# anilkeshwani/speech-integration

Measured on AMD Instinct MI355X. Metric: train_tokens_per_sec, higher is better.
Workload: dtype bf16; 1 GPU; Llama-3.2-1B +5000 DSUs (V=133258), SFT step fwd+bwd+AdamW, seq_len=2048, batch=8/GPU, grad_accum=1, 16 layers, random-init weights, MLS-shaped synthetic DSU sequences; global_batch=8, seq_len=2048, parallelism=dp1

## Files before the change

### include/ssi_hip.h

```cpp
#ifndef SSI_HIP_H
#define SSI_HIP_H

#include <stdint.h>

#ifdef __cplusplus
extern "C" {
#endif

#define SSI_ABI_VERSION 9

enum { SSI_F32 = 0, SSI_BF16 = 1 };
enum { SSI_OK = 0, SSI_ERR_ARG = 1, SSI_ERR_UNSUPPORTED = 2, SSI_ERR_WORKSPACE = 3, SSI_ERR_HIP = 1000  };
enum { SSI_GEMM_NT = 0, SSI_GEMM_NN = 1, SSI_GEMM_TN = 2 };
enum { SSI_TILES_STATIC = 0, SSI_TILES_DYNAMIC = 1 };
int ssi_set_gemm_tile_order(int mode);

enum { SSI_IMPL_AUTO = 0, SSI_IMPL_GENERIC = 1, SSI_IMPL_MFMA = 2,
       SSI_IMPL_MFMA_WG8 = 3  };

int ssi_abi_version(void);
const char* ssi_last_error(void);
int ssi_set_impl(int impl);

int ssi_embed_fwd(const int64_t* tokens, const void* table, void* out, int64_t n_tok, int64_t dim, int64_t vocab,
                  int dtype, void* stream);
int64_t ssi_embed_bwd_workspace_bytes(int64_t vocab);
int ssi_embed_bwd(const int64_t* tokens, const void* dout, void* dtable, int64_t n_tok, int64_t dim, int64_t vocab,
                  int dtype, void* workspace, int64_t workspace_bytes, void* stream);

int ssi_rmsnorm_fwd(const void* x, const void* scale, void* y, float* rstd, int64_t rows, int64_t dim, float eps,
                    int dtype, void* stream);
int64_t ssi_rmsnorm_bwd_workspace_bytes(int64_t rows, int64_t dim);
int ssi_rmsnorm_bwd(const void* dy, const void* x, const void* scale, const float* rstd, const void* dres, void* dx,
                    void* dscale, int accumulate_dscale, int64_t rows, int64_t dim, int dtype, void* workspace,
                    int64_t workspace_bytes, void* stream);

int ssi_rope_inplace(void* x, int64_t ld, int64_t rows, int64_t seq_len, int n_heads_rot, int head_dim,
                     const float* table, int64_t table_len, const int32_t* positions, int inverse, int dtype,
                     void* stream);

int ssi_gemm_rope(int64_t M, int64_t N, int64_t K, const void* A, int64_t lda, const void* B, int64_t ldb, void* C, int64_t ldc,
                  int64_t seq_len, int n_heads_rot, int head_dim, const float* rope_table, int64_t table_len,
                  const int32_t* positions, int dtype, void* stream);

int ssi_attn_fwd(const void* qkv, int64_t ld, void* out, float* lse, int64_t batch, int64_t seq, int n_heads,
                 int n_kv, int head_dim, int dtype, void* stream);
int ssi_attn_bwd(const void* qkv, int64_t ld, const void* out, const void* dout, const float* lse, void* dqkv,
                 float* delta, int64_t batch, int64_t seq, int n_heads, int n_kv, int head_dim, int dtype,
                 void* stream);

int ssi_attn_varlen_fwd(const void* qkv, int64_t ld, void* out, float* lse, const int32_t* doc_start, const int32_t* doc_end,
                        int64_t batch, int64_t seq, int n_heads, int n_kv, int head_dim, int dtype, void* stream);
int ssi_attn_varlen_bwd(const void* qkv, int64_t ld, const void* out, const void* dout, const float* lse, void* dqkv,
                        float* delta, const int32_t* doc_start, const int32_t* doc_end, int64_t batch, int64_t seq,
                        int n_heads, int n_kv, int head_dim, int dtype, void* stream);

int ssi_doc_ranges(const int64_t* input_pos, int64_t batch, int64_t seq, int64_t max_pos, int32_t* positions, int32_t* doc_start,
                   int32_t* doc_end, int32_t* n_clamped, void* stream);

int ssi_attn_varlen_bwd_rope(const void* qkv, int64_t ld, const void* out, const void* dout, const float* lse, void* dqkv,
                             float* delta, const int32_t* doc_start, const int32_t* doc_end, const float* rope_table,
                             int64_t table_len, const int32_t* positions, int64_t batch, int64_t seq, int n_heads, int n_kv,
                             int head_dim, int dtype, void* stream);

int64_t ssi_attn_bwd_workspace_bytes(int64_t batch, int64_t seq, int n_heads, int n_kv, int head_dim, int dtype);
int ssi_attn_varlen_bwd_ws(const void* qkv, int64_t ld, const void* out, const void* dout, const float* lse, void* dqkv,
                           float* delta, const int32_t* doc_start, const int32_t* doc_end, const float* rope_table,
                           int64_t table_len, const int32_t* positions, int64_t batch, int64_t seq, int n_heads, int n_kv,
                           int head_dim, int dtype, void* workspace, int64_t workspace_bytes, void* stream);

enum { SSI_ATTN_KERNEL_DQ = 0, SSI_ATTN_KERNEL_DKV = 1 };
enum { SSI_ATTN_MODE_AUTO = 0, SSI_ATTN_MODE_OLD = 1, SSI_ATTN_MODE_NEW = 2, SSI_ATTN_MODE_NO_HEAD_SPLIT = 3 };
int ssi_set_attn_impl(int which, int mode);
enum { SSI_ATTN_USED_DQ2 = 1, SSI_ATTN_USED_DKV2 = 2, SSI_ATTN_USED_HEAD_SPLIT = 4, SSI_ATTN_USED_PLAN = 8 };
int ssi_attn_last_dispatch(void);

enum { SSI_ATTN_PLAN_HEADER = 16, SSI_ATTN_PLAN_FORCE = 1, SSI_ATTN_PLAN_SPLIT_ALL = 2  };
int64_t ssi_attn_plan_words(int64_t batch, int64_t seq, int64_t n_docs);
int64_t ssi_attn_plan_workspace_bytes(const int32_t* host_plan_header);
int64_t ssi_attn_plan_build(const int32_t* host_doc_row, const int32_t* host_doc_start, const int32_t* host_doc_end, int64_t n_docs,
                            int64_t batch, int64_t seq, int n_heads, int n_kv, int flags, int32_t* host_plan, int64_t plan_words);
int ssi_attn_varlen_bwd_plan(const void* qkv, int64_t ld, const void* out, const void* dout, const float* lse, void* dqkv,
                             float* delta, const int32_t* doc_start, const int32_t* doc_end, const float* rope_table,
                             int64_t table_len, const int32_t* positions, int64_t batch, int64_t seq, int n_heads, int n_kv,
                             int head_dim, int dtype, void* workspace, int64_t workspace_bytes, const int32_t* plan,
                             const int32_t* host_plan_header, void* stream);

int ssi_swiglu_fwd(const void* gu, void* act, int64_t rows, int64_t inter, int dtype, void* stream);
int ssi_swiglu_bwd(const void* dact, const void* gu, void* dgu, int64_t rows, int64_t inter, int dtype, void* stream);

int ssi_gemm(int layout, int64_t M, int64_t N, int64_t K, const void* A, int64_t lda, const void* B, int64_t ldb,
             void* C, int64_t ldc, const void* R, float alpha, const float* alpha_dev, int accumulate, int dtype,
             void* stream);

int64_t ssi_gemm_splitk_workspace_bytes(int64_t M, int64_t N, int splits);
int ssi_gemm_splitk(int layout, int64_t M, int64_t N, int64_t K, const void* A, int64_t lda, const void* B, int64_t ldb,
                    void* C, int64_t ldc, const void* R, float alpha, const float* alpha_dev, int accumulate, int dtype,
                    int splits, void* workspace, int64_t workspace_bytes, void* stream);

int ssi_gemm_batched(int layout, int batch, int64_t M, int64_t N, int64_t K, const void* A, int64_t lda, int64_t strideA, const void* B,
                     int64_t ldb, int64_t strideB, void* C, int64_t ldc, int64_t strideC, float alpha, const float* alpha_dev,
                     int accumulate, int dtype, void* stream);

int ssi_gemm_swiglu_fwd(int64_t M, int64_t inter, int64_t K, const void* X, int64_t ldx, const void* W13, int64_t ldw, void* GU,
                        int64_t ldgu, void* ACT, int64_t ldact, int dtype, void* stream);
int ssi_gemm_swiglu_bwd(int layout, int64_t M, int64_t inter, int64_t K, const void* DY, int64_t lddy, const void* W2, int64_t ldw,
                        const void* GU, int64_t ldgu, void* DGU, int64_t lddgu, void* dact_ws, int dtype, void* stream);

int ssi_transpose(const void* src, int64_t ld_src, void* dst, int64_t ld_dst, int64_t rows, int64_t cols, int dtype,
                  void* stream);

int ssi_ce_fwd(void* logits, int64_t ld, const int64_t* labels, int64_t rows, int64_t vocab, int64_t ignore_index,
               float* row_loss, float* row_lse, int write_grad, int dtype, void* stream);
int ssi_ce_reduce(const float* row_loss, const int64_t* labels, int64_t rows, int64_t vocab, int64_t ignore_index, float* out,
                  void* stream);
int ssi_ce_fwd_weighted(void* logits, int64_t ld, const int64_t* labels, const float* row_weight, int64_t rows, int64_t vocab,
                        int64_t ignore_index, float* row_loss, float* row_lse, int write_grad, int dtype, void* stream);

int ssi_lmhead_ce_fwd(const void* hidden, int64_t ldh, const void* table, int64_t ldt, const int64_t* labels, int64_t rows,
                      int64_t dim, int64_t vocab, int64_t vocab_pad, int64_t ignore_index, void* logits_ws, int64_t ldl,
                      float* row_loss, float* stats, int write_grad, int dtype, void* stream);
int ssi_lmhead_ce_bwd(const void* dlogits, int64_t ldl, const void* hidden, int64_t ldh, const void* table, int64_t ldt,
                      const float* alpha_dev, int64_t rows, int64_t dim, int64_t vocab_pad, void* d_hidden, int64_t lddh,
                      void* d_table, int64_t lddt, int accumulate_d_table, int dtype, void* stream);

int ssi_count_tokens(const int64_t* tokens, const int64_t* labels, int64_t n, const int64_t* ranges, int n_ranges,
                     int64_t pad_id, int64_t ignore_index, int64_t* out, void* stream);

int ssi_scale_inplace(void* x, int64_t n, float scale, const float* scale_dev, int dtype, void* stream);
int64_t ssi_sumsq_workspace_bytes(int64_t n);
int ssi_sumsq(const void* x, int64_t n, int dtype, float* out, void* workspace, int64_t workspace_bytes, void* stream);
int ssi_adamw_step(void* param, void* grad, void* exp_avg, void* exp_avg_sq, int64_t n, double lr, double beta1,
                   double beta2, double eps, double weight_decay, int64_t step, const float* grad_scale_dev, int zero_grad,
                   int dtype, void* stream);

#ifdef __cplusplus
}
#endif
#endif
```

### speech-integration_amd/csrc/common_hip.h

```cpp
#pragma once
#include <hip/hip_runtime.h>
#include <stdint.h>
#include <stdio.h>
#include "../../include/ssi_hip.h"

typedef __bf16 bf16_t;
typedef __attribute__((ext_vector_type(2))) float f32x2;
typedef __attribute__((ext_vector_type(4))) float f32x4;
typedef __attribute__((ext_vector_type(16))) float f32x16;
typedef __attribute__((ext_vector_type(4))) __bf16 bf16x4;
typedef __attribute__((ext_vector_type(8))) __bf16 bf16x8;
typedef __attribute__((ext_vector_type(4))) short s16x4;
typedef __attribute__((ext_vector_type(4))) unsigned int u32x4;
typedef __attribute__((ext_vector_type(2))) unsigned int u32x2;

#define SSI_WAVE 64

void ssi_set_error(const char* fmt, ...);

#define SSI_CHECK_ARG(cond)                                                                  \
    do {                                                                                     \
        if (!(cond)) {                                                                       \
            ssi_set_error("%s:%d: argument check failed: %s", __FILE__, __LINE__, #cond);    \
            return SSI_ERR_ARG;                                                              \
// ... 48 lines not shown
    f32x4 v;
    __device__ __forceinline__ float get(int i) const { return v[i]; }
    __device__ __forceinline__ void set(int i, float x) { v[i] = x; }
};
template <> struct Vec16<bf16_t> {
    static constexpr int N = 8;
    bf16x8 v;
    __device__ __forceinline__ float get(int i) const { return (float)v[i]; }
    __device__ __forceinline__ void set(int i, float x) { v[i] = (bf16_t)x; }
};
template <typename T> __device__ __forceinline__ Vec16<T> load16(const T* p) {
    Vec16<T> r;
    r.v = *reinterpret_cast<const decltype(r.v)*>(p);
    return r;
}
template <typename T> __device__ __forceinline__ void store16(T* p, const Vec16<T>& r) {
    *reinterpret_cast<decltype(r.v)*>(p) = r.v;
}

template <typename T> __device__ __forceinline__ Vec16<T> load16_nt(const T* p) {
    Vec16<T> r;
    r.v = __builtin_nontemporal_load(reinterpret_cast<const decltype(r.v)*>(p));
    return r;
}
template <typename T> __device__ __forceinline__ void store16_nt(T* p, const Vec16<T>& r) {
    __builtin_nontemporal_store(r.v, reinterpret_cast<decltype(r.v)*>(p));
}

__device__ __forceinline__ float wave_sum(float v) {
#pragma unroll
    for (int o = 32; o > 0; o >>= 1) v += __shfl_xor(v, o, 64);
    return v;
}
__device__ __forceinline__ float wave_max(float v) {
#pragma unroll
    for (int o = 32; o > 0; o >>= 1) v = fmaxf(v, __shfl_xor(v, o, 64));
    return v;
}
__device__ __forceinline__ float block_sum(float v, float* red) {
    v = wave_sum(v);
    const int w = threadIdx.x >> 6, l = threadIdx.x & 63, nw = (blockDim.x + 63) >> 6;
    __syncthreads();
    if (l == 0) red[w] = v;
    __syncthreads();
    float t = (l < nw) ? red[l] : 0.f;
    t = wave_sum(t);
    return t;
}
__device__ __forceinline__ float block_max(float v, float* red) {
    v = wave_max(v);
    const int w = threadIdx.x >> 6, l = threadIdx.x & 63, nw = (blockDim.x + 63) >> 6;
    __syncthreads();
    if (l == 0) red[w] = v;
    __syncthreads();
    float t = (l < nw) ? red[l] : -INFINITY;
    t = wave_max(t);
    return t;
}

template <bool ENABLED, int N, bool FENCED = false> struct PhaseStamps {
    unsigned long long begin = __builtin_readcyclecounter(), last = begin, total[N] = {};
    __device__ __forceinline__ void reset() {
        if (FENCED) __builtin_amdgcn_sched_barrier(0);
        last = __builtin_readcyclecounter();
        if (FENCED) __builtin_amdgcn_sched_barrier(0);
    }
    __device__ __forceinline__ void tick(int i) {
        const unsigned long long prev = last;
        reset();
        total[i] += last - prev;
    }
};
template <int N, bool FENCED> struct PhaseStamps<false, N, FENCED> {
    __device__ __forceinline__ void reset() {}
    __device__ __forceinline__ void tick(int) {}
};

int ssi_get_impl();

bool ssi_gemm_mfma_supported(int layout, int64_t M, int64_t N, int64_t K, const void* A, int64_t lda, const void* B,
                             int64_t ldb, const void* C, int64_t ldc, const void* R);
int ssi_gemm_mfma_bf16(int layout, int64_t M, int64_t N, int64_t K, const void* A, int64_t lda, const void* B,
                       int64_t ldb, void* C, int64_t ldc, const void* R, float alpha, const float* alpha_dev,
                       int accumulate, void* stream);
int ssi_gemm_mfma_bf16_splitk(int layout, int64_t M, int64_t N, int64_t K, const void* A, int64_t lda, const void* B,
                              int64_t ldb, void* C, int64_t ldc, const void* R, float alpha, const float* alpha_dev,
                              int accumulate, int splits, float* slabs, void* stream);
bool ssi_gemm_mfma_bf16_batched(int layout, int batch, int64_t M, int64_t N, int64_t K, const void* A, int64_t lda, int64_t bsA, const void* B,
                                int64_t ldb, int64_t bsB, void* C, int64_t ldc, int64_t bsC, float alpha, const float* alpha_dev, int accumulate,
                                void* stream, int* rc);
void ssi_gemm_mfma_set_dynamic_tiles(int on);
bool ssi_gemm_rope_mfma(int64_t M, int64_t N, int64_t K, const void* A, int64_t lda, const void* B, int64_t ldb, void* C, int64_t ldc,
                        const float* rope, const int32_t* positions, int64_t seq, int64_t rot_cols, void* stream, int* rc);
bool ssi_gemm_swiglu_supported(int64_t M, int64_t inter, int64_t K, const void* p0, const void* p1, const void* p2, const void* p3,
                               int64_t ld0, int64_t ld1, int64_t ld2, int64_t ld3);
int ssi_gemm_swiglu_fwd_mfma(int64_t M, int64_t inter, int64_t K, const void* X, int64_t ldx, const void* W13, int64_t ldw,
                             void* GU, int64_t ldgu, void* ACT, int64_t ldact, void* stream);
int ssi_gemm_swiglu_bwd_mfma(int layout, int64_t M, int64_t inter, int64_t K, const void* DY, int64_t lddy, const void* W2, int64_t ldw,
                             const void* GU, int64_t ldgu, void* DGU, int64_t lddgu, void* stream);
bool ssi_gemm_swiglu_bwd_nn_supported(int64_t K, int64_t lddy, int64_t ldw);

bool ssi_gemm_f32_mfma_supported(int layout, int64_t M, int64_t N, int64_t K, const void* A, int64_t lda, const void* B,
                                 int64_t ldb, const void* C, int64_t ldc, const void* R);
int ssi_gemm_f32_mfma(int layout, int64_t M, int64_t N, int64_t K, const void* A, int64_t lda, const void* B, int64_t ldb,
                      void* C, int64_t ldc, const void* R, float alpha, const float* alpha_dev, int accumulate,
                      void* stream);

bool ssi_attn_mfma_supported(int64_t ld, int64_t batch, int64_t seq, int n_heads, int n_kv, int head_dim, int dtype);
void ssi_attn_note_dispatch(int v);
int ssi_attn_bwd_mfma(const void* qkv, int64_t ld, const void* out, const void* dout, const float* lse, void* dqkv,
                      float* delta, const int32_t* doc_start, const int32_t* doc_end, const float* rope, int64_t table_len,
                      const int32_t* positions, int64_t batch, int64_t seq, int n_heads, int n_kv, void* workspace, int64_t workspace_bytes,
                      const int32_t* plan_dev, const int32_t* host_plan_header, void* stream);
int ssi_attn_fwd_mfma(const void* qkv, int64_t ld, void* out, float* lse, const int32_t* doc_start, int64_t batch, int64_t seq,
                      int n_heads, int n_kv, void* stream);
int64_t ssi_attn_mfma_bwd_workspace_bytes(int64_t batch, int64_t seq, int n_heads, int n_kv);

#define SSI_DISPATCH_DTYPE(dtype, ...)                           \
    do {                                                         \
        if ((dtype) == SSI_F32) {                                \
            using T = float;                                     \
            __VA_ARGS__;                                         \
        } else if ((dtype) == SSI_BF16) {                        \
            using T = bf16_t;                                    \
            __VA_ARGS__;                                         \
        } else {                                                 \
            ssi_set_error("unsupported dtype %d", (int)(dtype)); \
            return SSI_ERR_ARG;                                  \
        }                                                        \
    } while (0)
```

### speech-integration_amd/csrc/gemm_generic.hip

```cpp
#include "common_hip.h"
#include <atomic>

static std::atomic<int> g_impl{SSI_IMPL_AUTO};
extern "C" int ssi_set_impl(int impl) {
    if (impl >= SSI_IMPL_AUTO && impl <= SSI_IMPL_MFMA_WG8) return g_impl.exchange(impl, std::memory_order_relaxed);
    return g_impl.load(std::memory_order_relaxed);
}
int ssi_get_impl() { return g_impl.load(std::memory_order_relaxed); }

extern "C" int ssi_set_gemm_tile_order(int mode) {
    if (mode != SSI_TILES_STATIC && mode != SSI_TILES_DYNAMIC) { ssi_set_error("ssi_set_gemm_tile_order: mode %d", mode); return SSI_ERR_ARG; }
    ssi_gemm_mfma_set_dynamic_tiles(mode == SSI_TILES_DYNAMIC);
    return SSI_OK;
}

template <typename T>
__global__ __launch_bounds__(256) void gemm_generic_kernel(int64_t M, int64_t N, int64_t K, const T* __restrict__ A,
                                                           int64_t sam, int64_t sak, const T* __restrict__ B, int64_t sbk,
                                                           int64_t sbn, T* __restrict__ C, int64_t ldc,
                                                           const T* __restrict__ R, float alpha,
                                                           const float* __restrict__ alpha_dev, int accumulate) {
    constexpr int BM = 64, BN = 64, BK = 16;
    __shared__ float As[BK][BM + 4];
    __shared__ float Bs[BK][BN + 4];
    const int tid = threadIdx.x;
    const int tx = tid & 15, ty = tid >> 4;
    const int64_t m0 = (int64_t)blockIdx.y * BM, n0 = (int64_t)blockIdx.x * BN;
    float acc[4][4];
#pragma unroll
    for (int i = 0; i < 4; ++i)
#pragma unroll
        for (int j = 0; j < 4; ++j) acc[i][j] = 0.f;

    const bool a_k_contig = (sak == 1);
    const bool b_n_contig = (sbn == 1);
    for (int64_t k0 = 0; k0 < K; k0 += BK) {
#pragma unroll
        for (int it = 0; it < 4; ++it) {
            const int e = tid + it * 256;
            int mm, kk;
            if (a_k_contig) { kk = e & 15; mm = e >> 4; } else { mm = e & 63; kk = e >> 6; }
            const int64_t gm = m0 + mm, gk = k0 + kk;
            As[kk][mm] = (gm < M && gk < K) ? to_f32<T>(A[gm * sam + gk * sak]) : 0.f;
            int nn, kb;
            if (b_n_contig) { nn = e & 63; kb = e >> 6; } else { kb = e & 15; nn = e >> 4; }
            const int64_t gn = n0 + nn, gkb = k0 + kb;
            Bs[kb][nn] = (gn < N && gkb < K) ? to_f32<T>(B[gkb * sbk + gn * sbn]) : 0.f;
        }
        __syncthreads();
#pragma unroll
        for (int kk = 0; kk < BK; ++kk) {
            float a[4], b[4];
#pragma unroll
            for (int i = 0; i < 4; ++i) a[i] = As[kk][ty * 4 + i];
#pragma unroll
            for (int j = 0; j < 4; ++j) b[j] = Bs[kk][tx * 4 + j];
#pragma unroll
            for (int i = 0; i < 4; ++i)
#pragma unroll
                for (int j = 0; j < 4; ++j) acc[i][j] = fmaf(a[i], b[j], acc[i][j]);
        }
        __syncthreads();
    }
    const float al = alpha * (alpha_dev ? *alpha_dev : 1.f);
#pragma unroll
    for (int i = 0; i < 4; ++i) {
        const int64_t gm = m0 + ty * 4 + i;
        if (gm >= M) continue;
#pragma unroll
        for (int j = 0; j < 4; ++j) {
            const int64_t gn = n0 + tx * 4 + j;
            if (gn >= N) continue;
            float v = al * acc[i][j];
            if (accumulate) v += to_f32<T>(C[gm * ldc + gn]);
            if (R) v += to_f32<T>(R[gm * ldc + gn]);
            C[gm * ldc + gn] = from_f32<T>(v);
        }
    }
}

extern "C" int ssi_gemm(int layout, int64_t M, int64_t N, int64_t K, const void* A, int64_t lda, const void* B,
                        int64_t ldb, void* C, int64_t ldc, const void* R, float alpha, const float* alpha_dev,
                        int accumulate, int dtype, void* stream) {
    SSI_CHECK_ARG(A && B && C && M >= 0 && N >= 0 && K >= 0 && ldc >= N);
    SSI_CHECK_ARG(layout == SSI_GEMM_NT || layout == SSI_GEMM_NN || layout == SSI_GEMM_TN);
    if (M == 0 || N == 0) return SSI_OK;
    int64_t sam, sak, sbk, sbn;
    if (layout == SSI_GEMM_NT)      { SSI_CHECK_ARG(lda >= K && ldb >= K); sam = lda; sak = 1;   sbk = 1;   sbn = ldb; }
    else if (layout == SSI_GEMM_NN) { SSI_CHECK_ARG(lda >= K && ldb >= N); sam = lda; sak = 1;   sbk = ldb; sbn = 1; }
    else                            { SSI_CHECK_ARG(lda >= M && ldb >= N); sam = 1;   sak = lda; sbk = ldb; sbn = 1; }

    const bool f32_ok = dtype == SSI_F32 && ssi_gemm_f32_mfma_supported(layout, M, N, K, A, lda, B, ldb, C, ldc, R);
    const bool mfma_ok = f32_ok || (dtype == SSI_BF16 && ssi_gemm_mfma_supported(layout, M, N, K, A, lda, B, ldb, C, ldc, R));
    if ((g_impl == SSI_IMPL_MFMA || g_impl == SSI_IMPL_MFMA_WG8) && !mfma_ok) {
        ssi_set_error("ssi_gemm: MFMA path forced but shape/dtype unsupported (M=%lld N=%lld K=%lld dtype=%d)",
                      (long long)M, (long long)N, (long long)K, dtype);
        return SSI_ERR_UNSUPPORTED;
    }
    if (f32_ok && g_impl != SSI_IMPL_GENERIC)
        return ssi_gemm_f32_mfma(layout, M, N, K, A, lda, B, ldb, C, ldc, R, alpha, alpha_dev, accumulate, stream);
    if (mfma_ok && g_impl != SSI_IMPL_GENERIC)
        return ssi_gemm_mfma_bf16(layout, M, N, K, A, lda, B, ldb, C, ldc, R, alpha, alpha_dev, accumulate, stream);

    SSI_CHECK_ARG(ssi_cdiv(M, 64) <= 65535);
    dim3 grid((unsigned)ssi_cdiv(N, 64), (unsigned)ssi_cdiv(M, 64));
    SSI_DISPATCH_DTYPE(dtype, hipLaunchKernelGGL(gemm_generic_kernel<T>, grid, dim3(256), 0, (hipStream_t)stream, M, N, K,
                                                 (const T*)A, sam, sak, (const T*)B, sbk, sbn, (T*)C, ldc, (const T*)R,
                                                 alpha, alpha_dev, accumulate));
    SSI_LAUNCH_CHECK();
    return SSI_OK;
}

extern "C" int ssi_gemm_batched(int layout, int batch, int64_t M, int64_t N, int64_t K, const void* A, int64_t lda, int64_t strideA,
                                const void* B, int64_t ldb, int64_t strideB, void* C, int64_t ldc, int64_t strideC, float alpha,
                                const float* alpha_dev, int accumulate, int dtype, void* stream) {
    SSI_CHECK_ARG(batch >= 0 && strideA >= 0 && strideB >= 0 && strideC >= 0);
    SSI_CHECK_ARG(dtype == SSI_BF16 || dtype == SSI_F32);
    if (batch == 0) return SSI_OK;
    SSI_CHECK_ARG(A && B && C);
    const int64_t es = dtype == SSI_BF16 ? 2 : 4;
    auto off = [&](const void* p, int64_t b, int64_t stride) { return (const void*)((const char*)p + b * stride * es); };
    bool mfma_ok = dtype == SSI_BF16 && batch > 1 && g_impl != SSI_IMPL_GENERIC && g_impl != SSI_IMPL_MFMA_WG8;
    for (int b = 0; b < batch && mfma_ok; ++b)
        mfma_ok = ssi_gemm_mfma_supported(layout, M, N, K, off(A, b, strideA), lda, off(B, b, strideB), ldb, off(C, b, strideC), ldc, nullptr);
    if (mfma_ok) {
        SSI_CHECK_ARG(layout == SSI_GEMM_NT || layout == SSI_GEMM_NN || layout == SSI_GEMM_TN);
        int rc = SSI_OK;
        if (ssi_gemm_mfma_bf16_batched(layout, batch, M, N, K, A, lda, strideA, B, ldb, strideB, C, ldc, strideC, alpha, alpha_dev, accumulate,
                                       stream, &rc))
            return rc;
    }
    for (int b = 0; b < batch; ++b)
        if (int rc = ssi_gemm(layout, M, N, K, off(A, b, strideA), lda, off(B, b, strideB), ldb, (void*)off(C, b, strideC), ldc, nullptr, alpha,
                              alpha_dev, accumulate, dtype, stream))
            return rc;
    return SSI_OK;
}

extern "C" int64_t ssi_gemm_splitk_workspace_bytes(int64_t M, int64_t N, int splits) {
    return splits <= 1 ? 0 : (int64_t)splits * M * N * (int64_t)sizeof(float);
}

extern "C" int ssi_gemm_splitk(int layout, int64_t M, int64_t N, int64_t K, const void* A, int64_t lda, const void* B,
                               int64_t ldb, void* C, int64_t ldc, const void* R, float alpha, const float* alpha_dev,
                               int accumulate, int dtype, int splits, void* workspace, int64_t workspace_bytes, void* stream) {
    const bool mfma_ok = dtype == SSI_BF16 && ssi_gemm_mfma_supported(layout, M, N, K, A, lda, B, ldb, C, ldc, R);
    if (splits <= 1 || !mfma_ok || g_impl == SSI_IMPL_GENERIC || K / 64 < splits)
        return ssi_gemm(layout, M, N, K, A, lda, B, ldb, C, ldc, R, alpha, alpha_dev, accumulate, dtype, stream);
    SSI_CHECK_ARG(layout == SSI_GEMM_NT || layout == SSI_GEMM_NN || layout == SSI_GEMM_TN);
    SSI_CHECK_ARG(splits <= 64 && ((uintptr_t)workspace % 16) == 0);
    if (!workspace || workspace_bytes < ssi_gemm_splitk_workspace_bytes(M, N, splits)) { ssi_set_error("ssi_gemm_splitk: workspace too small"); return SSI_ERR_WORKSPACE; }
    return ssi_gemm_mfma_bf16_splitk(layout, M, N, K, A, lda, B, ldb, C, ldc, R, alpha, alpha_dev, accumulate, splits,
                                     (float*)workspace, stream);
}

extern "C" int ssi_gemm_rope(int64_t M, int64_t N, int64_t K, const void* A, int64_t lda, const void* B, int64_t ldb, void* C, int64_t ldc,
                             int64_t seq_len, int n_heads_rot, int head_dim, const float* rope_table, int64_t table_len,
                             const int32_t* positions, int dtype, void* stream) {
    SSI_CHECK_ARG(A && B && C && rope_table && M >= 0 && N > 0 && K > 0 && seq_len > 0 && n_heads_rot > 0 && head_dim > 0);
    SSI_CHECK_ARG((int64_t)n_heads_rot * head_dim <= N && (positions != nullptr || table_len >= seq_len));
    if (M == 0) return SSI_OK;
    int rc = SSI_OK;
    if (dtype == SSI_BF16 && head_dim == 64 && g_impl != SSI_IMPL_GENERIC &&
        ssi_gemm_rope_mfma(M, N, K, A, lda, B, ldb, C, ldc, rope_table, positions, seq_len, (int64_t)n_heads_rot * head_dim, stream, &rc))
        return rc;
    if ((rc = ssi_gemm(SSI_GEMM_NT, M, N, K, A, lda, B, ldb, C, ldc, nullptr, 1.f, nullptr, 0, dtype, stream))) return rc;
    return ssi_rope_inplace(C, ldc, M, seq_len, n_heads_rot, head_dim, rope_table, table_len, positions, 0, dtype, stream);
}

extern "C" int ssi_gemm_swiglu_fwd(int64_t M, int64_t inter, int64_t K, const void* X, int64_t ldx, const void* W13, int64_t ldw,
                                   void* GU, int64_t ldgu, void* ACT, int64_t ldact, int dtype, void* stream) {
    SSI_CHECK_ARG(X && W13 && GU && ACT && M >= 0 && inter > 0 && K > 0 && ldgu >= 2 * inter && ldact >= inter);
    if (dtype == SSI_BF16 && g_impl != SSI_IMPL_GENERIC && ssi_gemm_swiglu_supported(M, inter, K, X, W13, GU, ACT, ldx, ldw, ldgu, ldact))
        return ssi_gemm_swiglu_fwd_mfma(M, inter, K, X, ldx, W13, ldw, GU, ldgu, ACT, ldact, stream);
    if (int rc = ssi_gemm(SSI_GEMM_NT, M, 2 * inter, K, X, ldx, W13, ldw, GU, ldgu, nullptr, 1.f, nullptr, 0, dtype, stream)) return rc;
    SSI_CHECK_ARG(ldgu == 2 * inter && ldact == inter);
    return ssi_swiglu_fwd(GU, ACT, M, inter, dtype, stream);
}

extern "C" int ssi_gemm_swiglu_bwd(int layout, int64_t M, int64_t inter, int64_t K, const void* DY, int64_t lddy, const void* W2,
                                   int64_t ldw, const void* GU, int64_t ldgu, void* DGU, int64_t lddgu, void* dact_ws, int dtype,
                                   void* stream) {
    SSI_CHECK_ARG(DY && W2 && GU && DGU && M >= 0 && inter > 0 && K > 0 && ldgu >= 2 * inter && lddgu >= 2 * inter);
    SSI_CHECK_ARG(layout == SSI_GEMM_NT || layout == SSI_GEMM_NN);
    if (dtype == SSI_BF16 && g_impl != SSI_IMPL_GENERIC && ssi_gemm_swiglu_supported(M, inter, K, DY, W2, GU, DGU, lddy, ldw, ldgu, lddgu) &&
        (layout == SSI_GEMM_NT || ssi_gemm_swiglu_bwd_nn_supported(K, lddy, ldw)))
        return ssi_gemm_swiglu_bwd_mfma(layout, M, inter, K, DY, lddy, W2, ldw, GU, ldgu, DGU, lddgu, stream);
    SSI_CHECK_ARG(dact_ws != nullptr && ldgu == 2 * inter && lddgu == 2 * inter);
    if (int rc = ssi_gemm(layout, M, inter, K, DY, lddy, W2, ldw, dact_ws, inter, nullptr, 1.f, nullptr, 0, dtype, stream)) return rc;
    return ssi_swiglu_bwd(dact_ws, GU, DGU, M, inter, dtype, stream);
}
```

### speech-integration_amd/csrc/gemm_mfma.hip

```cpp
#include "common_hip.h"
#include <atomic>
#include <type_traits>

namespace {

constexpr int BM = 256, BN = 256, BK = 64;
constexpr int NTHREADS = 512;
constexpr int WAVES_N = 4;
constexpr int WM = 128, WN = 64;
constexpr int MT = WM / 16, NT = WN / 16;
constexpr int TILE_BYTES = BM * BK * 2;
constexpr int PIPE_BYTES = 2 * 2 * TILE_BYTES;
constexpr int EPI_ROW_BYTES = WN * 2 + 16;
constexpr int EPI_WAVE_BYTES = WM * EPI_ROW_BYTES;
constexpr int LDS_BYTES = 8 * EPI_WAVE_BYTES > PIPE_BYTES ? 8 * EPI_WAVE_BYTES : PIPE_BYTES;

typedef __attribute__((address_space(3))) void lds_void;
typedef __attribute__((address_space(1))) const void gbl_void;

__device__ __forceinline__ int col_swz(int krow) { return ((krow & 3) | (((krow >> 3) & 1) << 2)) << 1; }

__device__ __forceinline__ void stage_col_load(const bf16_t* __restrict__ g, int64_t ld, int64_t r0, int64_t k0, int tid,
                                               u32x4 (&regs)[4]) {
#pragma unroll
    for (int p = 0; p < 4; ++p) {
        const int krow = p * 16 + (tid >> 5);
        const int chunk = (tid & 31) ^ col_swz(krow);
        regs[p] = *reinterpret_cast<const u32x4*>(g + (k0 + krow) * ld + r0 + chunk * 8);
    }
}
__device__ __forceinline__ void stage_col_write(char* lds_tile, int tid, const u32x4 (&regs)[4]) {
#pragma unroll
    for (int p = 0; p < 4; ++p) *reinterpret_cast<u32x4*>(lds_tile + p * 8192 + tid * 16) = regs[p];
}

template <bool COL>
__device__ __forceinline__ void stage_tile(const bf16_t* __restrict__ g, int64_t ld, int64_t r0, int64_t k0, char* lds_tile,
                                           int tid, int64_t split_rows = 0) {
#pragma unroll
    for (int p = 0; p < 4; ++p) {
        const bf16_t* src;
        if (!COL) {
            const int row = p * 64 + (tid >> 3);
            const int chunk = (tid & 7) ^ ((row >> 1) & 7);
            const int64_t grow = split_rows ? (row < 128 ? (r0 >> 1) + row : split_rows + (r0 >> 1) + row - 128) : r0 + row;
            src = g + grow * ld + k0 + chunk * 8;
        } else {
            const int krow = p * 16 + (tid >> 5);
            const int chunk = (tid & 31) ^ col_swz(krow);
            src = g + (k0 + krow) * ld + r0 + chunk * 8;
        }
        const int wave_base = __builtin_amdgcn_readfirstlane(p * 8192 + (tid >> 6) * 1024);
        __builtin_amdgcn_global_load_lds((gbl_void*)src, (lds_void*)(lds_tile + wave_base), 16, 0, 0);
    }
}

template <bool COL>
__device__ __forceinline__ bf16x8 read_frag(const char* lds_tile, int outer_base, int kh, int lane) {
    if (!COL) {
        const int row = outer_base + (lane & 15);
        const int chunk = (kh * 4 + (lane >> 4)) ^ ((row >> 1) & 7);
        return *reinterpret_cast<const bf16x8*>(lds_tile + row * 128 + chunk * 16);
    } else {
        const int i = lane & 15, q = i >> 2, p = i & 3;
        const int kbase = kh * 32 + 8 * (lane >> 4);
        const int chunk = (outer_base >> 3) + (p >> 1);
        const int k0 = kbase + q, k1 = kbase + 4 + q;
        const char* a0 = lds_tile + k0 * 512 + ((chunk ^ col_swz(k0)) * 16) + 8 * (p & 1);
        const char* a1 = lds_tile + k1 * 512 + ((chunk ^ col_swz(k1)) * 16) + 8 * (p & 1);
        s16x4 lo = __builtin_amdgcn_ds_read_tr16_b64_v4i16((__attribute__((address_space(3))) s16x4*)a0);
        s16x4 hi = __builtin_amdgcn_ds_read_tr16_b64_v4i16((__attribute__((address_space(3))) s16x4*)a1);
        typedef __attribute__((ext_vector_type(8))) short s16x8;
        s16x8 r = __builtin_shufflevector(lo, hi, 0, 1, 2, 3, 4, 5, 6, 7);
        return __builtin_bit_cast(bf16x8, r);
    }
}

__device__ __forceinline__ void tile_coords(int bid, int tiles_m, int tiles_n, int& tm, int& tn) {
    const int nwg = tiles_m * tiles_n;
    const int xcd = bid & 7, q = nwg >> 3, r = nwg & 7;
    const int t = (xcd < r ? xcd * (q + 1) : r * (q + 1) + (xcd - r) * q) + (bid >> 3);
    constexpr int GM = 4;
    const int per_group = GM * tiles_n;
    const int group = t / per_group, in_group = t % per_group;
    const int gm = (tiles_m - group * GM) < GM ? (tiles_m - group * GM) : GM;
    tm = group * GM + in_group % gm;
    tn = in_group / gm;
}

__device__ __forceinline__ void tile_from_t(int t, int tiles_m, int tiles_n, int& tm, int& tn) {
    constexpr int GM = 4;
    const int per_group = GM * tiles_n;
    const int group = t / per_group, in_group = t % per_group;
    const int gm = (tiles_m - group * GM) < GM ? (tiles_m - group * GM) : GM;
    tm = group * GM + in_group % gm;
    tn = in_group / gm;
}

__device__ int g_nt4_sched[16][16];

enum { EPI_PLAIN = 0, EPI_SWIGLU_FWD = 1, EPI_SWIGLU_BWD = 2, EPI_ROPE = 3 };
struct EpiArgs {
    bf16_t* out2;
    int64_t ld_out2;
    const bf16_t* in2;
    int64_t ld_in2;
    int64_t inter;
    const float* rope = nullptr;
    const int32_t* pos = nullptr;
    int64_t seq = 1;
    int64_t rot_cols = 0;
    int batch = 1;
    int64_t bsA = 0, bsB = 0, bsC = 0;
};

template <bool A_COL, bool B_COL, bool SPLITK, int EPI = EPI_PLAIN>
__global__ __launch_bounds__(NTHREADS, 2) void gemm_mfma_kernel(int tiles_m, int tiles_n, int64_t K,
                                                               const bf16_t* __restrict__ A, int64_t lda,
                                                               const bf16_t* __restrict__ B, int64_t ldb,
                                                               bf16_t* __restrict__ C, int64_t ldc,
                                                               const bf16_t* __restrict__ R, float alpha,
                                                               const float* __restrict__ alpha_dev, int accumulate,
                                                               float* __restrict__ slabs, EpiArgs ea) {
    extern __shared__ __attribute__((aligned(16))) char smem[];
    const int tid = threadIdx.x, lane = tid & 63;
    const int wave = __builtin_amdgcn_readfirstlane(tid >> 6);
    const int wm = wave / WAVES_N, wn = wave % WAVES_N;
    int tm, tn;
    tile_coords(blockIdx.x, tiles_m, tiles_n, tm, tn);
    const int64_t m0 = (int64_t)tm * BM, n0 = (int64_t)tn * BN;

    f32x4 acc[NT][MT];
#pragma unroll
    for (int i = 0; i < NT; ++i)
#pragma unroll
        for (int j = 0; j < MT; ++j) acc[i][j] = f32x4{0.f, 0.f, 0.f, 0.f};

    const int nk_total = (int)(K / BK);
    const int kt_begin = SPLITK ? (int)((int64_t)blockIdx.y * nk_total / gridDim.y) : 0;
    const int kt_end = SPLITK ? (int)((int64_t)(blockIdx.y + 1) * nk_total / gridDim.y) : nk_total;
    const int nk = kt_end - kt_begin;
    const int64_t kofs = (int64_t)kt_begin * BK;
    auto tileA = [&](int buf) { return smem + buf * 2 * TILE_BYTES; };
    auto tileB = [&](int buf) { return smem + buf * 2 * TILE_BYTES + TILE_BYTES; };
    auto stage = [&](int kt, int buf) {
        stage_tile<A_COL>(A, lda, m0, kofs + (int64_t)kt * BK, tileA(buf), tid);
        stage_tile<B_COL>(B, ldb, n0, kofs + (int64_t)kt * BK, tileB(buf), tid, EPI == EPI_SWIGLU_FWD ? ea.inter : 0);
    };
    if constexpr (A_COL && B_COL) {
        u32x4 ra[4], rb[4];
        stage_col_load(A, lda, m0, kofs, tid, ra);
        stage_col_load(B, ldb, n0, kofs, tid, rb);
        stage_col_write(tileA(0), tid, ra);
        stage_col_write(tileB(0), tid, rb);
        for (int kt = 0; kt < nk; ++kt) {
            const int cur = kt & 1;
            __syncthreads();
            if (kt + 1 < nk) {
                stage_col_load(A, lda, m0, kofs + (int64_t)(kt + 1) * BK, tid, ra);
                stage_col_load(B, ldb, n0, kofs + (int64_t)(kt + 1) * BK, tid, rb);
            }
            const char* la = tileA(cur);
            const char* lb = tileB(cur);
#pragma unroll
            for (int kh = 0; kh < 2; ++kh) {
                bf16x8 bfr[NT], afr[MT];
#pragma unroll
                for (int j = 0; j < NT; ++j) bfr[j] = read_frag<true>(lb, wn * WN + j * 16, kh, lane);
#pragma unroll
                for (int i = 0; i < MT; ++i) afr[i] = read_frag<true>(la, wm * WM + i * 16, kh, lane);
                __builtin_amdgcn_s_setprio(1);
#pragma unroll
                for (int i = 0; i < MT; ++i)
#pragma unroll
                    for (int j = 0; j < NT; ++j)
                        acc[j][i] = __builtin_amdgcn_mfma_f32_16x16x32_bf16(bfr[j], afr[i], acc[j][i], 0, 0, 0);
                __builtin_amdgcn_s_setprio(0);
            }
            if (kt + 1 < nk) {
// ... 180 lines not shown
#pragma unroll
    for (int e = 0; e < 8; ++e) f[e] = 0.f;
    for (int s = 0; s < splits; ++s) {
        const float* p = slabs + (int64_t)s * M * N + row * N + col;
        const f32x4 a = *reinterpret_cast<const f32x4*>(p), b = *reinterpret_cast<const f32x4*>(p + 4);
#pragma unroll
        for (int e = 0; e < 4; ++e) { f[e] += a[e]; f[4 + e] += b[e]; }
    }
    bf16x8 o;
#pragma unroll
    for (int e = 0; e < 8; ++e) o[e] = (bf16_t)(f[e] * al);
    const int64_t off = row * ldc + col;
    if (accumulate || R) {
#pragma unroll
        for (int e = 0; e < 8; ++e) f[e] = (float)o[e];
        if (accumulate) {
            const bf16x8 c = *reinterpret_cast<const bf16x8*>(C + off);
#pragma unroll
            for (int e = 0; e < 8; ++e) f[e] += (float)c[e];
        }
        if (R) {
            const bf16x8 c = *reinterpret_cast<const bf16x8*>(R + off);
#pragma unroll
            for (int e = 0; e < 8; ++e) f[e] += (float)c[e];
        }
#pragma unroll
        for (int e = 0; e < 8; ++e) o[e] = (bf16_t)f[e];
    }
    *reinterpret_cast<bf16x8*>(C + off) = o;
}

template <bool A_COL, bool B_COL, bool SPLITK, int EPI = EPI_PLAIN>
int launch(int tiles_m, int tiles_n, int64_t K, const void* A, int64_t lda, const void* B, int64_t ldb, void* C,
           int64_t ldc, const void* R, float alpha, const float* alpha_dev, int accumulate, hipStream_t st,
           int splits = 1, float* slabs = nullptr, EpiArgs ea = EpiArgs{nullptr, 0, nullptr, 0, 0}) {
    auto kern = gemm_mfma_kernel<A_COL, B_COL, SPLITK, EPI>;
    static const hipError_t attr_rc = hipFuncSetAttribute((const void*)kern, hipFuncAttributeMaxDynamicSharedMemorySize, LDS_BYTES);
    if (attr_rc != hipSuccess) { ssi_set_error("gemm_mfma: cannot reserve %d B of LDS: %s", LDS_BYTES, hipGetErrorString(attr_rc)); return SSI_ERR_HIP + (int)attr_rc; }
    hipLaunchKernelGGL(kern, dim3((unsigned)(tiles_m * tiles_n), (unsigned)splits), dim3(NTHREADS), LDS_BYTES, st, tiles_m,
                       tiles_n, K, (const bf16_t*)A, lda, (const bf16_t*)B, ldb, (bf16_t*)C, ldc, (const bf16_t*)R, alpha,
                       alpha_dev, accumulate, slabs, ea);
    SSI_LAUNCH_CHECK();
    if (SPLITK) {
        const int64_t M = (int64_t)tiles_m * BM, N = (int64_t)tiles_n * BN;
        hipLaunchKernelGGL(splitk_reduce_kernel, dim3((unsigned)ssi_cdiv(M * N / 8, 256)), dim3(256), 0, st, slabs, splits, M, N,
                           (bf16_t*)C, ldc, (const bf16_t*)R, alpha, alpha_dev, accumulate);
        SSI_LAUNCH_CHECK();
    }
    return SSI_OK;
}

#ifndef NT4_ST_AUX
#define NT4_ST_AUX 0
#endif
#ifndef NT4_ST_AUX_BIG
#define NT4_ST_AUX_BIG 2
#endif
#ifndef NT4_RS
#define NT4_RS 2
#define NT4_BAR 40
#define NT4_A0 44
#define NT4_SA 6
#define NT4_NA 4
#endif
constexpr int NT4_THREADS = 256;
constexpr int NT4_LDS_BYTES = PIPE_BYTES + 16;
std::atomic<int> g_nt4_dynamic{0};
inline unsigned nt4_next_slot() {
    static std::atomic<unsigned> n{0};
    return n.fetch_add(1, std::memory_order_relaxed);
}
constexpr int NT4_WM = 128, NT4_WN = 128;
constexpr unsigned BUF_RSRC_DW3 = 0x00020000u;

__device__ __forceinline__ __amdgpu_buffer_rsrc_t make_rsrc(const void* p) {
    return __builtin_amdgcn_make_buffer_rsrc(const_cast<void*>(p), 0, 0x7fffffff, BUF_RSRC_DW3);
}

template <bool A_COL, bool B_COL, int EPI, int PREV, bool SPLITK, bool BATCHED>
__device__ __forceinline__ void nt4_body(char* smem, int tiles_m, int tiles_n, int64_t K, const bf16_t* __restrict__ A,
                                         int64_t lda, const bf16_t* __restrict__ B, int64_t ldb,
                                         bf16_t* __restrict__ C, int64_t ldc, const bf16_t* __restrict__ R,
                                         float alpha, const float* __restrict__ alpha_dev, EpiArgs ea, int slot,
                                         int splits, float* __restrict__ slabs) {
    const int tid = threadIdx.x, lane = tid & 63;
    const int wave = __builtin_amdgcn_readfirstlane(tid >> 6);
    const int wm = wave >> 1, wn = wave & 1;
    const int per_prob = tiles_m * tiles_n;
    const int ntiles_out = BATCHED ? per_prob * ea.batch : per_prob;
    const int ntiles = SPLITK ? ntiles_out * splits : ntiles_out;
    auto locate = [&](int t, int& tm, int& tn) {
        int tt = SPLITK ? t % ntiles_out : t, pb = 0;
        if constexpr (BATCHED) { pb = tt / per_prob; tt -= pb * per_prob; }
        tile_from_t(tt, tiles_m, tiles_n, tm, tn);
        return pb;
    };
    const int G = (int)gridDim.x;
    const int nk_total = (int)(K / BK);
    auto k_lo = [&](int t) { return SPLITK ? (int)(((int64_t)nk_total * (t / ntiles_out) / splits) & ~1LL) : 0; };
    auto k_hi = [&](int t) { return SPLITK ? ((t / ntiles_out) + 1 == splits ? nk_total : (int)(((int64_t)nk_total * (t / ntiles_out + 1) / splits) & ~1LL)) : nk_total; };

    int* sched = g_nt4_sched[slot < 0 ? 0 : slot];
    volatile int* lds_next = reinterpret_cast<volatile int*>(smem + PIPE_BYTES);
    const int xcd = (int)blockIdx.x & 7, span_q = ntiles >> 3, span_r = ntiles & 7;
    auto span_len = [&](int x) { return span_q + (x < span_r ? 1 : 0); };
    auto span_lo = [&](int x) { return x < span_r ? x * (span_q + 1) : span_r * (span_q + 1) + (x - span_r) * span_q; };
    auto span_wgs = [&](int x) { return (G - x + 7) >> 3; };
    auto span_fixed = [&](int x) { const int n = 2 * span_wgs(x); return n < span_len(x) ? n : span_len(x); };
    const bool dynamic = slot >= 0;
    int my_idx = (int)blockIdx.x >> 3;
    int pending = 0;
    auto request_tile = [&]() {
        if (dynamic && tid == 0) pending = atomicAdd(&sched[xcd], 1);
    };
    auto receive_tile = [&]() -> int {
        if (!dynamic) {
            my_idx += G >> 3;
            return ((G & 7) == 0 && my_idx < span_len(xcd)) ? span_lo(xcd) + my_idx : -1;
        }
        asm volatile("s_waitcnt lgkmcnt(0)\n\ts_barrier" ::: "memory");
        if (tid == 0) {
            int t = -1;
            const int i = pending + span_fixed(xcd);
            if (i < span_len(xcd)) t = span_lo(xcd) + i;
            if (t < 0) {
                int seen[8];
#pragma unroll
                for (int x = 0; x < 8; ++x) seen[x] = __hip_atomic_load(&sched[x], __ATOMIC_RELAXED, __HIP_MEMORY_SCOPE_AGENT);
                for (int k = 1; k < 8 && t < 0; ++k) {
                    const int x = (xcd + k) & 7;
                    if (seen[x] + span_fixed(x) >= span_len(x)) continue;
                    const int j = atomicAdd(&sched[x], 1) + span_fixed(x);
                    if (j < span_len(x)) t = span_lo(x) + j;
                }
            }
            *lds_next = t;
        }
        asm volatile("s_waitcnt lgkmcnt(0)\n\ts_barrier" ::: "memory");
        return __builtin_amdgcn_readfirstlane(*lds_next);
    };
    int cur = ((int)blockIdx.x >> 3) < span_len(xcd) ? span_lo(xcd) + ((int)blockIdx.x >> 3) : -1;
    int nxt = -1;
    if (dynamic) {
        const int second = ((int)blockIdx.x >> 3) + span_wgs(xcd);
        nxt = (cur >= 0 && second < span_len(xcd)) ? span_lo(xcd) + second : -1;
    }

    f32x4 acc[8][8];
    auto tileA = [&](int buf) { return smem + buf * TILE_BYTES; };
    auto tileB = [&](int buf) { return smem + 2 * TILE_BYTES + buf * TILE_BYTES; };

    int lkt = 0, lnk = nk_total;
    const bf16_t* baseA = A;
    const bf16_t* baseB = B;
    const int64_t kstepA_ = A_COL ? BK * lda : BK, kstepB_ = B_COL ? BK * ldb : BK;
    auto set_load_tile = [&](int t) {
        int tm, tn;
        const int pb = locate(t, tm, tn);
        const bf16_t* Ap = BATCHED ? A + pb * ea.bsA : A;
        const bf16_t* Bp = BATCHED ? B + pb * ea.bsB : B;
        baseA = (A_COL ? Ap + (int64_t)tm * BM : Ap + (int64_t)tm * BM * lda) + k_lo(t) * kstepA_;
        baseB = (B_COL ? Bp + (int64_t)tn * BN : Bp + (int64_t)tn * (EPI == EPI_SWIGLU_FWD ? BN / 2 : BN) * ldb) + k_lo(t) * kstepB_;
        lnk = k_hi(t) - k_lo(t);
    };
    auto advance = [&]() {
        if (++lkt == lnk) {
            lkt = 0;
            if (nxt >= 0) set_load_tile(nxt);
        }
    };
    auto lane_off = [&](bool col, int64_t ld, int odd) {
        if (col) return (int)(((tid >> 5) * ld + (((tid & 31) ^ col_swz(odd * 8 + (tid >> 5))) * 8)) * 2);
        return (int)(((tid >> 3) * ld + (tid & 7) * 8) * 2);
    };
    const int offA0 = lane_off(A_COL, lda, 0), offA1 = A_COL ? lane_off(true, lda, 1) : offA0;
    const int offB0 = lane_off(B_COL, ldb, 0), offB1 = B_COL ? lane_off(true, ldb, 1) : offB0;
    const int64_t kstepA = kstepA_, kstepB = kstepB_;
    auto pieceA = [&](int p) { return A_COL ? (int)(p * 8 * lda * 2) : (int)(p * 32 * lda * 2); };
    auto pieceB = [&](int p) {
        if (B_COL) return (int)(p * 8 * ldb * 2);
        if (EPI == EPI_SWIGLU_FWD) {
            const int blk64 = p >> 1;
            return (int)((((blk64 & 1) ? ea.inter : 0) + (blk64 >> 1) * 64 + (p & 1) * 32) * ldb * 2);
        }
        return (int)(p * 32 * ldb * 2);
    };
    int trA = 0, trB = 0;
    if (A_COL || B_COL) {
        const int i16 = lane & 15, q = i16 >> 2, pp = i16 & 3, k0l = 8 * (lane >> 4) + q;
        const int common = k0l * 512 + (pp >> 1) * 16 + 8 * (pp & 1) + (col_swz(k0l) << 4);
        trA = common + wm * 256;
        trB = common + wn * 256;
    }
    auto rd_tr = [&](const char* tile, int base, int t8, int kh) {
        typedef __attribute__((address_space(3))) s16x4 lds_s16x4;
        const char* a0 = tile + (base ^ (t8 << 5)) + kh * 16384;
        const s16x4 lo = __builtin_amdgcn_ds_read_tr16_b64_v4i16((lds_s16x4*)a0);
        const s16x4 hi = __builtin_amdgcn_ds_read_tr16_b64_v4i16((lds_s16x4*)(a0 + 2048));
        typedef __attribute__((ext_vector_type(8))) short s16x8;
        const s16x8 r = __builtin_shufflevector(lo, hi, 0, 1, 2, 3, 4, 5, 6, 7);
        return __builtin_bit_cast(bf16x8, r);
    };
    using F_ = std::false_type;
    bf16x8 F0A[8], F0B[8], F1A[8], F1B[8];
    const int dofA = (int)(((tid >> 3) * lda + (((tid & 7) ^ ((tid >> 4) & 7)) * 8)) * 2);
    const int dofB = (int)(((tid >> 3) * ldb + (((tid & 7) ^ ((tid >> 4) & 7)) * 8)) * 2);
    typedef __attribute__((address_space(3))) char lds_c;
    const unsigned lds_wave = __builtin_amdgcn_readfirstlane((unsigned)(uintptr_t)(lds_c*)smem + (unsigned)wave * 1024u);
    auto rsrc_words = [&](const bf16_t* base) {
        const uint64_t a = (uint64_t)(uintptr_t)base;
        u32x4 r;
        r[0] = __builtin_amdgcn_readfirstlane((unsigned)a);
        r[1] = __builtin_amdgcn_readfirstlane((unsigned)(a >> 32) & 0xffffu);
        r[2] = 0x7fffffffu;
        r[3] = BUF_RSRC_DW3;
        return r;
    };
    auto dma_m0 = [&](int buf, int d) {
        const unsigned dst = lds_wave + (unsigned)((d < 8 ? buf * TILE_BYTES : 2 * TILE_BYTES + buf * TILE_BYTES) + (d & 7) * 4096);
        asm volatile("s_mov_b32 m0, %0" ::"s"(dst) : "memory");
    };
    u32x4 rsA, rsB;
    auto dma_src = [&]() { rsA = rsrc_words(baseA + lkt * kstepA); rsB = rsrc_words(baseB + lkt * kstepB); };
    auto dma_go = [&](int d) {
        if (d < 8) asm volatile("buffer_load_dwordx4 %0, %1, %2 offen lds" ::"v"(A_COL ? ((d & 1) ? offA1 : offA0) : dofA), "s"(rsA), "s"(pieceA(d)) : "memory");
        else asm volatile("buffer_load_dwordx4 %0, %1, %2 offen lds" ::"v"(B_COL ? ((d & 1) ? offB1 : offB0) : dofB), "s"(rsB), "s"(pieceB(d - 8)) : "memory");
    };
    auto dma = [&](int buf, int d) {
        dma_m0(buf, d);
        asm volatile("s_nop 1" ::: "memory");
        dma_go(d);
    };
    auto fragA = [&](const char* t, int i, int kh) {
        if constexpr (A_COL) return rd_tr(t, trA, i, kh);
        else return read_frag<false>(t, wm * NT4_WM + i * 16, kh, lane);
    };
    auto fragB = [&](const char* t, int j, int kh) {
        if constexpr (B_COL) return rd_tr(t, trB, j, kh);
        else return read_frag<false>(t, wn * NT4_WN + j * 16, kh, lane);
    };
    auto phase = [&](const bf16x8 (&fa)[8], const bf16x8 (&fb)[8], auto zero_c, auto extra) {
#pragma unroll
        for (int m = 0; m < 64; ++m) {
            const int i = m >> 3, j = m & 7;
            if (decltype(zero_c)::value)
                asm volatile("v_mfma_f32_16x16x32_bf16 %0, %1, %2, 0" : "=a"(acc[j][i]) : "v"(fb[j]), "v"(fa[i]));
            else
                asm volatile("v_mfma_f32_16x16x32_bf16 %0, %1, %2, %0" : "+a"(acc[j][i]) : "v"(fb[j]), "v"(fa[i]));
            extra(m);
            __builtin_amdgcn_sched_barrier(0);
        }
    };
    auto dma_body = [&](auto cur_c, auto first) {
        constexpr int cur = decltype(cur_c)::value;
        if (A_COL) asm volatile("" : "+v"(trA));
        if (B_COL) asm volatile("" : "+v"(trB));
        const char* la = tileA(cur);
        const char* lb = tileB(cur);
        const char* na = tileA(cur ^ 1);
        const char* nb = tileB(cur ^ 1);
        constexpr int RS = NT4_RS, BAR = NT4_BAR, A0 = NT4_A0, SA = NT4_SA, NA = NT4_NA;
        static_assert(15 * RS + 4 <= BAR && BAR + 2 <= A0 - 1 && A0 + (NA - 1) * SA <= 63 && 3 + 5 * (15 - NA) <= 58, "DMA schedule");
        phase(F0A, F0B, first, [&](int m) {
            if (m < 16 * RS && m % RS == 0) {
                const int r = m / RS;
                if (r < 8) F1B[r] = fragB(lb, r, 1); else F1A[r - 8] = fragA(la, r - 8, 1);
            }
            if (m == BAR) {
                asm volatile("s_waitcnt lgkmcnt(0)\n\ts_barrier" ::: "memory");
                dma_src();
            }
            if (m >= A0 - 1 && m < A0 - 1 + NA * SA && (m - (A0 - 1)) % SA == 0) dma_m0(cur, (m - (A0 - 1)) / SA);
            if (m >= A0 && m < A0 + NA * SA && (m - A0) % SA == 0) dma_go((m - A0) / SA);
        });
        advance();
        phase(F1A, F1B, F_{}, [&](int m) {
            if (m >= 2 && m < 2 + 5 * (16 - NA) && (m - 2) % 5 == 0) dma_m0(cur, NA + (m - 2) / 5);
            if (m >= 3 && m < 3 + 5 * (16 - NA) && (m - 3) % 5 == 0) dma_go(NA + (m - 3) / 5);
            if (m == 11) {
                if constexpr (NA == 4) asm volatile("s_waitcnt vmcnt(6)\n\ts_barrier" ::: "memory");
                else if constexpr (NA == 6) asm volatile("s_waitcnt vmcnt(8)\n\ts_barrier" ::: "memory");
                else if constexpr (NA == 7) asm volatile("s_waitcnt vmcnt(9)\n\ts_barrier" ::: "memory");
                else asm volatile("s_waitcnt vmcnt(0)\n\ts_barrier" ::: "memory");
            }
            if (m >= 12 && m <= 50 && !(m & 1) && m % 10 != 8) {
                const int r = (m - 12) / 2 - (m - 8) / 10;
                if (r < 8) F0B[r] = fragB(nb, r, 0); else F0A[r - 8] = fragA(na, r - 8, 0);
            }
        });
    };
    set_load_tile(cur >= 0 ? cur : 0);
    if (nk_total == 0) return;
    dma_src();
#pragma unroll
    for (int d = 0; d < 16; ++d) dma(0, d);
    advance();
    dma_src();
#pragma unroll
    for (int d = 0; d < 16; ++d) dma(1, d);
    advance();
    asm volatile("s_waitcnt vmcnt(16)\n\ts_barrier" ::: "memory");
#pragma unroll
    for (int r = 0; r < 8; ++r) F0B[r] = fragB(tileB(0), r, 0);
#pragma unroll
    for (int r = 0; r < 8; ++r) F0A[r] = fragA(tileA(0), r, 0);
    if (cur >= 0 && !dynamic) nxt = receive_tile();
    const float al = alpha * (alpha_dev ? *alpha_dev : 1.f);
    const int g = lane >> 4;
    while (cur >= 0) {
        int tm, tn;
        const int pb = locate(cur, tm, tn);
        const int nk = k_hi(cur) - k_lo(cur);
        using B0_ = std::integral_constant<int, 0>;
        using B1_ = std::integral_constant<int, 1>;
        if (nxt >= 0) request_tile();
        dma_body(B0_{}, std::true_type{});
        dma_body(B1_{}, F_{});
        for (int kt = 2; kt < nk; kt += 2) {
            dma_body(B0_{}, F_{});
            dma_body(B1_{}, F_{});
        }
        asm volatile("s_nop 15\n\ts_nop 15" ::: "memory");
        auto pair = [&](int i, int ja, int jb, auto scale_c) {
            bf16x4 x, y;
#pragma unroll
            for (int r = 0; r < 4; ++r) {
                float fx, fy;
                asm volatile("v_accvgpr_read_b32 %0, %1" : "=v"(fx) : "a"(acc[ja][i][r]));
                asm volatile("v_accvgpr_read_b32 %0, %1" : "=v"(fy) : "a"(acc[jb][i][r]));
                x[r] = (bf16_t)(decltype(scale_c)::value ? fx * al : fx);
                y[r] = (bf16_t)(decltype(scale_c)::value ? fy * al : fy);
            }
            const u32x2 xu = __builtin_bit_cast(u32x2, x), yu = __builtin_bit_cast(u32x2, y);
            const auto s0 = __builtin_amdgcn_permlane16_swap(xu[0], yu[0], false, false);
            const auto s1 = __builtin_amdgcn_permlane16_swap(xu[1], yu[1], false, false);
            u32x4 o;
            o[0] = s0[0]; o[1] = s1[0]; o[2] = s0[1]; o[3] = s1[1];
            return o;
        };
        auto duo = [&](int i, int j0, auto scale_c, u32x4& lo, u32x4& hi) {
            const u32x4 oa = pair(i, j0, j0 + 1, scale_c), ob = pair(i, j0 + 2, j0 + 3, scale_c);
#pragma unroll
            for (int d = 0; d < 4; ++d) {
                lo[d] = (unsigned)__builtin_amdgcn_update_dpp((int)oa[d], (int)ob[d], 0x118 , 0xF, 0xC, false);
                hi[d] = (unsigned)__builtin_amdgcn_update_dpp((int)ob[d], (int)oa[d], 0x108 , 0xF, 0x3, false);
            }
        };
        if constexpr (SPLITK) {
            const __amdgpu_buffer_rsrc_t rsS = make_rsrc(slabs + ((int64_t)cur * 4 + wave) * (64 * 64 * 4));
#pragma unroll
            for (int i = 0; i < 8; ++i)
#pragma unroll
                for (int j = 0; j < 8; ++j) {
                    u32x4 v;
#pragma unroll
                    for (int r = 0; r < 4; ++r) {
                        float f;
                        asm volatile("v_accvgpr_read_b32 %0, %1" : "=v"(f) : "a"(acc[j][i][r]));
                        v[r] = __builtin_bit_cast(unsigned, f);
                    }
                    __builtin_amdgcn_raw_buffer_store_b128(v, rsS, lane * 16, (i * 8 + j) * 1024, 0);
                    __builtin_amdgcn_sched_barrier(0);
                }
        } else {
        const int64_t row0 = (int64_t)tm * BM + wm * NT4_WM;
        const int lane_row = lane & 7, lane_col = ((lane >> 3) & 1) * 32 + (g & 1) * 16 + (g >> 1) * 8;
        auto epilogue = [&](auto scale_c) {
        if constexpr (EPI == EPI_PLAIN) {
            const int64_t tile_off = (BATCHED ? pb * ea.bsC : 0) + row0 * ldc + (int64_t)tn * BN + wn * NT4_WN;
            const __amdgpu_buffer_rsrc_t rsC = make_rsrc(C + tile_off);
            const __amdgpu_buffer_rsrc_t rsP = make_rsrc(PREV == 2 ? R + tile_off : C + tile_off);
            const int voff = (int)((lane_row * ldc + lane_col) * 2);
            auto soff = [&](int i, int h, int jd) { return (int)(((i * 16 + h * 8) * ldc + jd * 64) * 2); };
            u32x4 pv[2][4];
            auto ldprev = [&](int i) {
#pragma unroll
                for (int q = 0; q < 4; ++q) pv[i & 1][q] = __builtin_amdgcn_raw_buffer_load_b128(rsP, voff, soff(i, q & 1, q >> 1), 0);
            };
            auto add_prev = [&](u32x4& o, const u32x4& p) {
                bf16x8 ob = __builtin_bit_cast(bf16x8, o);
                const bf16x8 c = __builtin_bit_cast(bf16x8, p);
#pragma unroll
                for (int e = 0; e < 8; ++e) ob[e] = (bf16_t)((float)ob[e] + (float)c[e]);
                o = __builtin_bit_cast(u32x4, ob);
            };
            if (PREV) ldprev(0);
#pragma unroll
            for (int i = 0; i < 8; ++i) {
                if (PREV && i + 1 < 8) ldprev(i + 1);
#pragma unroll
                for (int jd = 0; jd < 2; ++jd) {
                    u32x4 lo, hi;
                    duo(i, jd * 4, scale_c, lo, hi);
                    if (PREV) { add_prev(lo, pv[i & 1][jd * 2]); add_prev(hi, pv[i & 1][jd * 2 + 1]); }
                    __builtin_amdgcn_raw_buffer_store_b128(lo, rsC, voff, soff(i, 0, jd), NT4_ST_AUX);
                    __builtin_amdgcn_raw_buffer_store_b128(hi, rsC, voff, soff(i, 1, jd), NT4_ST_AUX);
                    __builtin_amdgcn_sched_barrier(0);
                }
            }
        } else if constexpr (EPI == EPI_ROPE) {
            const int64_t tile_off = row0 * ldc + (int64_t)tn * BN + wn * NT4_WN;
            const __amdgpu_buffer_rsrc_t rsC = make_rsrc(C + tile_off);
            const int voff = (int)((lane_row * ldc + lane_col) * 2);
            auto soff = [&](int i, int hh, int jd) { return (int)(((i * 16 + hh * 8) * ldc + jd * 64) * 2); };
            const bool rot = (int64_t)tn * BN < ea.rot_cols;
            int prow[8][2];
            f32x4 cs[2][2][2];
            if (rot) {
#pragma unroll
                for (int i = 0; i < 8; ++i)
#pragma unroll
                    for (int hh = 0; hh < 2; ++hh) {
                        const int64_t r = row0 + i * 16 + hh * 8 + lane_row;
                        prow[i][hh] = ea.pos ? ea.pos[r] : (int)(r % ea.seq);
                    }
            }
            auto ldcs = [&](int i) {
#pragma unroll
                for (int hh = 0; hh < 2; ++hh) {
                    const float* tb = ea.rope + (int64_t)prow[i][hh] * 64 + (lane_col & 63);
                    cs[i & 1][hh][0] = *reinterpret_cast<const f32x4*>(tb);
                    cs[i & 1][hh][1] = *reinterpret_cast<const f32x4*>(tb + 4);
                }
            };
            auto rotate = [&](u32x4& o, const f32x4& c01, const f32x4& c23) {
                bf16x8 v = __builtin_bit_cast(bf16x8, o);
#pragma unroll
                for (int p = 0; p < 4; ++p) {
                    const f32x4& c = p < 2 ? c01 : c23;
                    float o0, o1;
                    ssi_rope_pair((float)v[2 * p], (float)v[2 * p + 1], c[(p & 1) * 2], c[(p & 1) * 2 + 1], o0, o1);
                    v[2 * p] = (bf16_t)o0;
                    v[2 * p + 1] = (bf16_t)o1;
                }
                o = __builtin_bit_cast(u32x4, v);
            };
            if (rot) ldcs(0);
#pragma unroll
            for (int i = 0; i < 8; ++i) {
                if (rot && i + 1 < 8) ldcs(i + 1);
#pragma unroll
                for (int jd = 0; jd < 2; ++jd) {
                    u32x4 lo, hi;
                    duo(i, jd * 4, scale_c, lo, hi);
                    if (rot) { rotate(lo, cs[i & 1][0][0], cs[i & 1][0][1]); rotate(hi, cs[i & 1][1][0], cs[i & 1][1][1]); }
                    __builtin_amdgcn_raw_buffer_store_b128(lo, rsC, voff, soff(i, 0, jd), NT4_ST_AUX);
                    __builtin_amdgcn_raw_buffer_store_b128(hi, rsC, voff, soff(i, 1, jd), NT4_ST_AUX);
// ... 18 lines not shown
            };
#pragma unroll
            for (int i = 0; i < 8; ++i) {
                u32x4 glo, ghi, ulo, uhi;
                duo(i, 0, scale_c, glo, ghi);
                duo(i, 4, scale_c, ulo, uhi);
#pragma unroll
                for (int h = 0; h < 2; ++h) {
                    const u32x4& gq = h ? ghi : glo;
                    const u32x4& uq = h ? uhi : ulo;
                    const int so = (int)(((i * 16 + h * 8) * ldc) * 2), so2 = (int)(((i * 16 + h * 8) * ea.ld_out2) * 2);
                    __builtin_amdgcn_raw_buffer_store_b128(gq, rsGU, voff, so, NT4_ST_AUX_BIG);
                    __builtin_amdgcn_raw_buffer_store_b128(uq, rsGU, voff, so + up_off, NT4_ST_AUX_BIG);
                    __builtin_amdgcn_raw_buffer_store_b128(act_of(gq, uq), rsACT, voff2, so2, NT4_ST_AUX_BIG);
                }
                __builtin_amdgcn_sched_barrier(0);
            }
        } else {
            const int64_t c0 = (int64_t)tn * BN + wn * NT4_WN;
            const __amdgpu_buffer_rsrc_t rsGU = make_rsrc(ea.in2 + row0 * ea.ld_in2 + c0);
            const __amdgpu_buffer_rsrc_t rsDGU = make_rsrc(ea.out2 + row0 * ea.ld_out2 + c0);
            const int voff = (int)((lane_row * ea.ld_in2 + lane_col) * 2), voff2 = (int)((lane_row * ea.ld_out2 + lane_col) * 2);
            const int up_off = (int)(ea.inter * 2);
            u32x4 pg[2][2], pu[2][2];
            auto ldprev = [&](int u) {
#pragma unroll
                for (int h = 0; h < 2; ++h) {
                    const int so = (int)((((u >> 1) * 16 + h * 8) * ea.ld_in2 + (u & 1) * 64) * 2);
                    pg[u & 1][h] = __builtin_amdgcn_raw_buffer_load_b128(rsGU, voff, so, 0);
                    pu[u & 1][h] = __builtin_amdgcn_raw_buffer_load_b128(rsGU, voff, so + up_off, 0);
                }
            };
            auto grads = [&](const u32x4& dq, const u32x4& gq, const u32x4& uq, u32x4& og_out, u32x4& ou_out) {
                const bf16x8 dv = __builtin_bit_cast(bf16x8, dq), gv = __builtin_bit_cast(bf16x8, gq), uv = __builtin_bit_cast(bf16x8, uq);
                bf16x8 og, ou;
#pragma unroll
                for (int e = 0; e < 8; ++e) {
                    float dg, du;
                    ssi_swiglu_bwd_elem<bf16_t>((float)gv[e], (float)uv[e], (float)dv[e], dg, du);
                    ou[e] = (bf16_t)du;
                    og[e] = (bf16_t)dg;
                }
                og_out = __builtin_bit_cast(u32x4, og);
                ou_out = __builtin_bit_cast(u32x4, ou);
            };
            ldprev(0);
#pragma unroll
            for (int u = 0; u < 16; ++u) {
                if (u + 1 < 16) ldprev(u + 1);
                const int i = u >> 1, jd = u & 1;
                u32x4 lo, hi;
                duo(i, jd * 4, scale_c, lo, hi);
#pragma unroll
                for (int h = 0; h < 2; ++h) {
                    u32x4 og, ou;
                    grads(h ? hi : lo, pg[u & 1][h], pu[u & 1][h], og, ou);
                    const int so2 = (int)(((i * 16 + h * 8) * ea.ld_out2 + jd * 64) * 2);
                    __builtin_amdgcn_raw_buffer_store_b128(og, rsDGU, voff2, so2, NT4_ST_AUX);
                    __builtin_amdgcn_raw_buffer_store_b128(ou, rsDGU, voff2, so2 + up_off, NT4_ST_AUX);
                }
                __builtin_amdgcn_sched_barrier(0);
            }
        }
        };
        if (al == 1.f) epilogue(std::false_type{});
        else epilogue(std::true_type{});
        }
        cur = nxt;
        if (cur >= 0) nxt = receive_tile();
    }
    asm volatile("s_waitcnt vmcnt(0)" ::: "memory");
    if (dynamic && tid == 0 && atomicAdd(&sched[8], 1) == G - 1) {
        volatile int* vs = sched;
#pragma unroll
        for (int i = 0; i < 9; ++i) vs[i] = 0;
    }
}

template <bool A_COL, bool B_COL, int EPI, int PREV, bool SPLITK = false, bool BATCHED = false>
__global__ __launch_bounds__(NT4_THREADS, 1) void gemm_nt4dma_kernel(int tiles_m, int tiles_n, int64_t K, const bf16_t* __restrict__ A,
                                                                     int64_t lda, const bf16_t* __restrict__ B, int64_t ldb,
                                                                     bf16_t* __restrict__ C, int64_t ldc, const bf16_t* __restrict__ R,
                                                                     float alpha, const float* __restrict__ alpha_dev, EpiArgs ea, int slot,
                                                                     int splits, float* __restrict__ slabs) {
    extern __shared__ __attribute__((aligned(16))) char smem[];
    nt4_body<A_COL, B_COL, EPI, PREV, SPLITK, BATCHED>(smem, tiles_m, tiles_n, K, A, lda, B, ldb, C, ldc, R, alpha, alpha_dev, ea, slot, splits, slabs);
}

__global__ __launch_bounds__(256) void nt4_splitk_reduce_kernel(const float* __restrict__ slabs, int splits, int tiles_m, int tiles_n,
                                                                bf16_t* __restrict__ C, int64_t ldc, const bf16_t* __restrict__ R, float alpha,
                                                                const float* __restrict__ alpha_dev, int accumulate) {
    const int lane = threadIdx.x & 63;
    const int64_t u = (int64_t)blockIdx.x * 4 + (threadIdx.x >> 6);
    const int ntiles = tiles_m * tiles_n;
    if (u >= (int64_t)ntiles * 64) return;
    const int jd = (int)(u & 1), i = (int)((u >> 1) & 7), wave = (int)((u >> 4) & 3), t = (int)(u >> 6);
    const int wm = wave >> 1, wn = wave & 1, g = lane >> 4;
    int tm, tn;
    tile_from_t(t, tiles_m, tiles_n, tm, tn);
    const float al = alpha * (alpha_dev ? *alpha_dev : 1.f);
    f32x4 sum[4];
#pragma unroll
    for (int j = 0; j < 4; ++j) sum[j] = f32x4{0.f, 0.f, 0.f, 0.f};
    for (int s = 0; s < splits; ++s) {
        const float* p = slabs + (((int64_t)s * ntiles + t) * 4 + wave) * (64 * 64 * 4) + (int64_t)(i * 8 + jd * 4) * 256 + lane * 4;
#pragma unroll
        for (int j = 0; j < 4; ++j) {
            const f32x4 v = *reinterpret_cast<const f32x4*>(p + j * 256);
#pragma unroll
            for (int r = 0; r < 4; ++r) sum[j][r] += v[r];
        }
    }
    auto pair = [&](const f32x4& a, const f32x4& b) {
        bf16x4 x, y;
#pragma unroll
        for (int r = 0; r < 4; ++r) { x[r] = (bf16_t)(a[r] * al); y[r] = (bf16_t)(b[r] * al); }
        const u32x2 xu = __builtin_bit_cast(u32x2, x), yu = __builtin_bit_cast(u32x2, y);
        const auto s0 = __builtin_amdgcn_permlane16_swap(xu[0], yu[0], false, false);
        const auto s1 = __builtin_amdgcn_permlane16_swap(xu[1], yu[1], false, false);
        u32x4 o;
        o[0] = s0[0]; o[1] = s1[0]; o[2] = s0[1]; o[3] = s1[1];
        return o;
    };
    const u32x4 oa = pair(sum[0], sum[1]), ob = pair(sum[2], sum[3]);
    u32x4 lo, hi;
#pragma unroll
    for (int d = 0; d < 4; ++d) {
        lo[d] = (unsigned)__builtin_amdgcn_update_dpp((int)oa[d], (int)ob[d], 0x118 , 0xF, 0xC, false);
        hi[d] = (unsigned)__builtin_amdgcn_update_dpp((int)ob[d], (int)oa[d], 0x108 , 0xF, 0x3, false);
    }
    const int lane_row = lane & 7, lane_col = ((lane >> 3) & 1) * 32 + (g & 1) * 16 + (g >> 1) * 8;
    bf16_t* base = C + ((int64_t)tm * BM + wm * NT4_WM + i * 16 + lane_row) * ldc + (int64_t)tn * BN + wn * NT4_WN + jd * 64 + lane_col;
    const int64_t r_off = R ? (R - C) : 0;
    auto finish = [&](u32x4 o, bf16_t* dst) {
        if (accumulate || R) {
            bf16x8 ob8 = __builtin_bit_cast(bf16x8, o);
            const bf16x8 c = *reinterpret_cast<const bf16x8*>(dst + r_off);
#pragma unroll
            for (int e = 0; e < 8; ++e) ob8[e] = (bf16_t)((float)ob8[e] + (float)c[e]);
            o = __builtin_bit_cast(u32x4, ob8);
        }
        *reinterpret_cast<u32x4*>(dst) = o;
    };
    finish(lo, base);
    finish(hi, base + 8 * ldc);
}

template <bool A_COL, bool B_COL, int EPI, int PREV, bool SPLITK = false, bool BATCHED = false>
int launch_nt4(int tiles_m, int tiles_n, int64_t K, const void* A, int64_t lda, const void* B, int64_t ldb, void* C, int64_t ldc,
               const void* R, float alpha, const float* alpha_dev, hipStream_t st, EpiArgs ea = EpiArgs{nullptr, 0, nullptr, 0, 0},
               int splits = 1, float* slabs = nullptr) {
    static_assert(!BATCHED || (!SPLITK && EPI == EPI_PLAIN), "batched form: plain epilogue, no split-K");
    auto kern = gemm_nt4dma_kernel<A_COL, B_COL, EPI, PREV, SPLITK, BATCHED>;
    static const hipError_t attr_rc = hipFuncSetAttribute((const void*)kern, hipFuncAttributeMaxDynamicSharedMemorySize, NT4_LDS_BYTES);
    if (attr_rc != hipSuccess) { ssi_set_error("gemm_nt4: cannot reserve %d B of LDS: %s", NT4_LDS_BYTES, hipGetErrorString(attr_rc)); return SSI_ERR_HIP + (int)attr_rc; }
    static const int num_cu = [] {
        int dev = 0, cus = 0;
        if (hipGetDevice(&dev) != hipSuccess || hipDeviceGetAttribute(&cus, hipDeviceAttributeMultiprocessorCount, dev) != hipSuccess || cus <= 0) cus = 256;
        return cus;
    }();
    const int ntiles = tiles_m * tiles_n * (SPLITK ? splits : 1) * (BATCHED ? ea.batch : 1);
    int grid = ntiles < num_cu ? ntiles : num_cu;
    const int slot = g_nt4_dynamic.load(std::memory_order_relaxed) ? (int)(nt4_next_slot() & 15) : -1;
    hipLaunchKernelGGL(kern, dim3((unsigned)grid), dim3(NT4_THREADS), NT4_LDS_BYTES, st, tiles_m, tiles_n, K, (const bf16_t*)A, lda,
                       (const bf16_t*)B, ldb, (bf16_t*)C, ldc, (const bf16_t*)R, alpha, alpha_dev, ea, slot, splits, slabs);
    SSI_LAUNCH_CHECK();
    return SSI_OK;
}

bool nt4_ok(int64_t K) { return K % (2 * BK) == 0 && K >= 4 * BK && ssi_get_impl() != SSI_IMPL_MFMA_WG8; }
bool nt4_ld_ok(int64_t lda, int64_t ldb) { return 256 * lda * 2 < (1LL << 31) && 256 * ldb * 2 < (1LL << 31); }

template <bool A_COL, bool B_COL>
int gemm_form(int tm, int tn, int64_t K, const void* A, int64_t lda, const void* B, int64_t ldb, void* C, int64_t ldc, const void* R,
              float alpha, const float* alpha_dev, int accumulate, hipStream_t st) {
    if (nt4_ok(K) && nt4_ld_ok(lda, ldb) && !(accumulate && R)) {
        if (accumulate) return launch_nt4<A_COL, B_COL, EPI_PLAIN, 1>(tm, tn, K, A, lda, B, ldb, C, ldc, R, alpha, alpha_dev, st);
        if (R) return launch_nt4<A_COL, B_COL, EPI_PLAIN, 2>(tm, tn, K, A, lda, B, ldb, C, ldc, R, alpha, alpha_dev, st);
        return launch_nt4<A_COL, B_COL, EPI_PLAIN, 0>(tm, tn, K, A, lda, B, ldb, C, ldc, R, alpha, alpha_dev, st);
    }
    return launch<A_COL, B_COL, false>(tm, tn, K, A, lda, B, ldb, C, ldc, R, alpha, alpha_dev, accumulate, st);
}

}

void ssi_gemm_mfma_set_dynamic_tiles(int on) { g_nt4_dynamic.store(on ? 1 : 0, std::memory_order_relaxed); }

bool ssi_gemm_mfma_supported(int layout, int64_t M, int64_t N, int64_t K, const void* A, int64_t lda, const void* B,
                             int64_t ldb, const void* C, int64_t ldc, const void* R) {
    if (M <= 0 || N <= 0 || K <= 0) return false;
    if (M % BM || N % BN || K % BK) return false;
    if (lda % 8 || ldb % 8 || ldc % 8) return false;
    if (((uintptr_t)A | (uintptr_t)B | (uintptr_t)C | (uintptr_t)R) & 15) return false;
    if ((M / BM) * (N / BN) > (1LL << 30)) return false;
    (void)layout;
    return true;
}

int ssi_gemm_mfma_bf16(int layout, int64_t M, int64_t N, int64_t K, const void* A, int64_t lda, const void* B,
                       int64_t ldb, void* C, int64_t ldc, const void* R, float alpha, const float* alpha_dev,
                       int accumulate, void* stream) {
    const int tm = (int)(M / BM), tn = (int)(N / BN);
    auto st = (hipStream_t)stream;
#define GO(AC, BC) return gemm_form<AC, BC>(tm, tn, K, A, lda, B, ldb, C, ldc, R, alpha, alpha_dev, accumulate, st)
    switch (layout) {
        case SSI_GEMM_NT: GO(false, false);
        case SSI_GEMM_NN: GO(false, true);
        case SSI_GEMM_TN: GO(true, true);
    }
#undef GO
    return SSI_ERR_ARG;
}

bool ssi_gemm_mfma_bf16_batched(int layout, int batch, int64_t M, int64_t N, int64_t K, const void* A, int64_t lda, int64_t bsA, const void* B,
                                int64_t ldb, int64_t bsB, void* C, int64_t ldc, int64_t bsC, float alpha, const float* alpha_dev, int accumulate,
                                void* stream, int* rc) {
    if (layout != SSI_GEMM_TN || !nt4_ok(K) || !nt4_ld_ok(lda, ldb) || (bsA | bsB | bsC) % 8 || (M / BM) * (N / BN) * batch > (1LL << 30))
        return false;
    const int tm = (int)(M / BM), tn = (int)(N / BN);
    auto st = (hipStream_t)stream;
    EpiArgs ea{nullptr, 0, nullptr, 0, 0};
    ea.batch = batch; ea.bsA = bsA; ea.bsB = bsB; ea.bsC = bsC;
    *rc = accumulate ? launch_nt4<true, true, EPI_PLAIN, 1, false, true>(tm, tn, K, A, lda, B, ldb, C, ldc, nullptr, alpha, alpha_dev, st, ea)
                     : launch_nt4<true, true, EPI_PLAIN, 0, false, true>(tm, tn, K, A, lda, B, ldb, C, ldc, nullptr, alpha, alpha_dev, st, ea);
    return true;
}

int ssi_gemm_mfma_bf16_splitk(int layout, int64_t M, int64_t N, int64_t K, const void* A, int64_t lda, const void* B,
                              int64_t ldb, void* C, int64_t ldc, const void* R, float alpha, const float* alpha_dev,
                              int accumulate, int splits, float* slabs, void* stream) {
    const int tm = (int)(M / BM), tn = (int)(N / BN);
    auto st = (hipStream_t)stream;
    if (nt4_ok(K) && nt4_ld_ok(lda, ldb) && !(R && accumulate) && K / BK / splits >= 6 && ldc % 8 == 0) {
        const EpiArgs none{nullptr, 0, nullptr, 0, 0};
        int rc = SSI_ERR_ARG;
        if (layout == SSI_GEMM_TN) rc = launch_nt4<true, true, EPI_PLAIN, 0, true>(tm, tn, K, A, lda, B, ldb, C, ldc, nullptr, 1.f, nullptr, st, none, splits, slabs);
        else if (layout == SSI_GEMM_NT) rc = launch_nt4<false, false, EPI_PLAIN, 0, true>(tm, tn, K, A, lda, B, ldb, C, ldc, nullptr, 1.f, nullptr, st, none, splits, slabs);
        else if (layout == SSI_GEMM_NN) rc = launch_nt4<false, true, EPI_PLAIN, 0, true>(tm, tn, K, A, lda, B, ldb, C, ldc, nullptr, 1.f, nullptr, st, none, splits, slabs);
        if (rc) return rc;
        hipLaunchKernelGGL(nt4_splitk_reduce_kernel, dim3((unsigned)ssi_cdiv((int64_t)tm * tn * 64, 4)), dim3(256), 0, st, slabs, splits, tm, tn,
                           (bf16_t*)C, ldc, (const bf16_t*)R, alpha, alpha_dev, accumulate);
        SSI_LAUNCH_CHECK();
        return SSI_OK;
    }
#define GO(AC, BC) return launch<AC, BC, true>(tm, tn, K, A, lda, B, ldb, C, ldc, R, alpha, alpha_dev, accumulate, st, splits, slabs)
    switch (layout) {
        case SSI_GEMM_NT: GO(false, false);
        case SSI_GEMM_NN: GO(false, true);
        case SSI_GEMM_TN: GO(true, true);
    }
#undef GO
    return SSI_ERR_ARG;
}

bool ssi_gemm_rope_mfma(int64_t M, int64_t N, int64_t K, const void* A, int64_t lda, const void* B, int64_t ldb, void* C, int64_t ldc,
                        const float* rope, const int32_t* positions, int64_t seq, int64_t rot_cols, void* stream, int* rc) {
    if (!nt4_ok(K) || !nt4_ld_ok(lda, ldb) || M % BM || N % BN || rot_cols % BN || rot_cols > N || lda % 8 || ldb % 8 || ldc % 8) return false;
    if (((uintptr_t)A | (uintptr_t)B | (uintptr_t)C) & 15) return false;
    EpiArgs ea{nullptr, 0, nullptr, 0, 0};
    ea.rope = rope; ea.pos = positions; ea.seq = seq; ea.rot_cols = rot_cols;
    *rc = launch_nt4<false, false, EPI_ROPE, 0, false>((int)(M / BM), (int)(N / BN), K, A, lda, B, ldb, C, ldc, nullptr, 1.f, nullptr,
                                                (hipStream_t)stream, ea);
    return true;
}

bool ssi_gemm_swiglu_supported(int64_t M, int64_t inter, int64_t K, const void* p0, const void* p1, const void* p2, const void* p3,
                               int64_t ld0, int64_t ld1, int64_t ld2, int64_t ld3) {
    if (M <= 0 || M % BM || inter % BN || K % BK) return false;
    if ((ld0 | ld1 | ld2 | ld3) % 8) return false;
    if (((uintptr_t)p0 | (uintptr_t)p1 | (uintptr_t)p2 | (uintptr_t)p3) & 15) return false;
    return true;
}

int ssi_gemm_swiglu_fwd_mfma(int64_t M, int64_t inter, int64_t K, const void* X, int64_t ldx, const void* W13, int64_t ldw,
                             void* GU, int64_t ldgu, void* ACT, int64_t ldact, void* stream) {
    EpiArgs ea{(bf16_t*)ACT, ldact, nullptr, 0, inter};
    if (nt4_ok(K))
        return launch_nt4<false, false, EPI_SWIGLU_FWD, 0, false>((int)(M / BM), (int)(2 * inter / BN), K, X, ldx, W13, ldw, GU, ldgu, nullptr, 1.f, nullptr,
                                             (hipStream_t)stream, ea);
    return launch<false, false, false, EPI_SWIGLU_FWD>((int)(M / BM), (int)(2 * inter / BN), K, X, ldx, W13, ldw, GU, ldgu, nullptr, 1.f,
                                                       nullptr, 0, (hipStream_t)stream, 1, nullptr, ea);
}

int ssi_gemm_swiglu_bwd_mfma(int layout, int64_t M, int64_t inter, int64_t K, const void* DY, int64_t lddy, const void* W2, int64_t ldw,
                             const void* GU, int64_t ldgu, void* DGU, int64_t lddgu, void* stream) {
    EpiArgs ea{(bf16_t*)DGU, lddgu, (const bf16_t*)GU, ldgu, inter};
    const int tm = (int)(M / BM), tn = (int)(inter / BN);
    if (layout == SSI_GEMM_NN) {
        if (nt4_ok(K) && nt4_ld_ok(lddy, ldw))
            return launch_nt4<false, true, EPI_SWIGLU_BWD, 0, false>(tm, tn, K, DY, lddy, W2, ldw, DGU, lddgu, nullptr, 1.f, nullptr, (hipStream_t)stream, ea);
        return SSI_ERR_UNSUPPORTED;
    }
    if (nt4_ok(K) && nt4_ld_ok(lddy, ldw))
        return launch_nt4<false, false, EPI_SWIGLU_BWD, 0, false>(tm, tn, K, DY, lddy, W2, ldw, DGU, lddgu, nullptr, 1.f, nullptr, (hipStream_t)stream, ea);
    return launch<false, false, false, EPI_SWIGLU_BWD>(tm, tn, K, DY, lddy, W2, ldw, DGU, lddgu, nullptr, 1.f, nullptr, 0, (hipStream_t)stream, 1,
                                                       nullptr, ea);
}

bool ssi_gemm_swiglu_bwd_nn_supported(int64_t K, int64_t lddy, int64_t ldw) { return nt4_ok(K) && nt4_ld_ok(lddy, ldw); }
```

### speech-integration_amd/ssi/_lib.py

```python

from __future__ import annotations

import ctypes
import os
from ctypes import POINTER, c_char_p, c_double, c_float, c_int, c_int32, c_int64, c_void_p

import torch

_HERE = os.path.dirname(os.path.abspath(__file__))
LIB_PATH = os.environ.get("SSI_HIP_LIB") or os.path.join(os.path.dirname(_HERE), "libssi_hip.so")

SSI_F32, SSI_BF16 = 0, 1
GEMM_NT, GEMM_NN, GEMM_TN = 0, 1, 2
IMPL_AUTO, IMPL_GENERIC, IMPL_MFMA, IMPL_MFMA_WG8 = 0, 1, 2, 3
TILES_STATIC, TILES_DYNAMIC = 0, 1
ABI_VERSION = 9
ATTN_KERNEL_DQ, ATTN_KERNEL_DKV = 0, 1
ATTN_MODE_AUTO, ATTN_MODE_OLD, ATTN_MODE_NEW, ATTN_MODE_NO_HEAD_SPLIT = 0, 1, 2, 3
ATTN_USED_DQ2, ATTN_USED_DKV2, ATTN_USED_HEAD_SPLIT, ATTN_USED_PLAN = 1, 2, 4, 8
ATTN_PLAN_HEADER, ATTN_PLAN_FORCE, ATTN_PLAN_SPLIT_ALL = 16, 1, 2

_P = c_void_p
PROTOTYPES = {
    "ssi_abi_version": (c_int, []),
    "ssi_last_error": (c_char_p, []),
    "ssi_set_impl": (c_int, [c_int]),
    "ssi_set_attn_impl": (c_int, [c_int, c_int]),
    "ssi_attn_last_dispatch": (c_int, []),
    "ssi_embed_fwd": (c_int, [_P, _P, _P, c_int64, c_int64, c_int64, c_int, _P]),
    "ssi_embed_bwd_workspace_bytes": (c_int64, [c_int64]),
    "ssi_embed_bwd": (c_int, [_P, _P, _P, c_int64, c_int64, c_int64, c_int, _P, c_int64, _P]),
    "ssi_rmsnorm_fwd": (c_int, [_P, _P, _P, _P, c_int64, c_int64, c_float, c_int, _P]),
    "ssi_rmsnorm_bwd_workspace_bytes": (c_int64, [c_int64, c_int64]),
    "ssi_rmsnorm_bwd": (c_int, [_P, _P, _P, _P, _P, _P, _P, c_int, c_int64, c_int64, c_int, _P, c_int64, _P]),
    "ssi_rope_inplace": (c_int, [_P, c_int64, c_int64, c_int64, c_int, c_int, _P, c_int64, _P, c_int, c_int, _P]),
    "ssi_gemm_rope": (c_int, [c_int64, c_int64, c_int64, _P, c_int64, _P, c_int64, _P, c_int64, c_int64, c_int, c_int, _P, c_int64, _P,
                              c_int, _P]),
    "ssi_attn_fwd": (c_int, [_P, c_int64, _P, _P, c_int64, c_int64, c_int, c_int, c_int, c_int, _P]),
    "ssi_attn_bwd": (c_int, [_P, c_int64, _P, _P, _P, _P, _P, c_int64, c_int64, c_int, c_int, c_int, c_int, _P]),
    "ssi_set_gemm_tile_order": (c_int, [c_int]),
    "ssi_attn_varlen_fwd": (c_int, [_P, c_int64, _P, _P, _P, _P, c_int64, c_int64, c_int, c_int, c_int, c_int, _P]),
    "ssi_attn_varlen_bwd": (c_int, [_P, c_int64, _P, _P, _P, _P, _P, _P, _P, c_int64, c_int64, c_int, c_int, c_int, c_int, _P]),
    "ssi_attn_varlen_bwd_rope": (c_int, [_P, c_int64, _P, _P, _P, _P, _P, _P, _P, _P, c_int64, _P, c_int64, c_int64, c_int, c_int, c_int,
                                         c_int, _P]),
    "ssi_attn_bwd_workspace_bytes": (c_int64, [c_int64, c_int64, c_int, c_int, c_int, c_int]),
    "ssi_attn_varlen_bwd_ws": (c_int, [_P, c_int64, _P, _P, _P, _P, _P, _P, _P, _P, c_int64, _P, c_int64, c_int64, c_int, c_int, c_int,
                                       c_int, _P, c_int64, _P]),
    "ssi_attn_plan_words": (c_int64, [c_int64, c_int64, c_int64]),
    "ssi_attn_plan_workspace_bytes": (c_int64, [_P]),
    "ssi_attn_plan_build": (c_int64, [_P, _P, _P, c_int64, c_int64, c_int64, c_int, c_int, c_int, _P, c_int64]),
    "ssi_attn_varlen_bwd_plan": (c_int, [_P, c_int64, _P, _P, _P, _P, _P, _P, _P, _P, c_int64, _P, c_int64, c_int64, c_int, c_int, c_int,
                                         c_int, _P, c_int64, _P, _P, _P]),
    "ssi_doc_ranges": (c_int, [_P, c_int64, c_int64, c_int64, _P, _P, _P, _P, _P]),
    "ssi_swiglu_fwd": (c_int, [_P, _P, c_int64, c_int64, c_int, _P]),
    "ssi_swiglu_bwd": (c_int, [_P, _P, _P, c_int64, c_int64, c_int, _P]),
    "ssi_gemm": (c_int, [c_int, c_int64, c_int64, c_int64, _P, c_int64, _P, c_int64, _P, c_int64, _P, c_float, _P,
                         c_int, c_int, _P]),
    "ssi_gemm_splitk_workspace_bytes": (c_int64, [c_int64, c_int64, c_int]),
    "ssi_gemm_splitk": (c_int, [c_int, c_int64, c_int64, c_int64, _P, c_int64, _P, c_int64, _P, c_int64, _P, c_float, _P,
                                c_int, c_int, c_int, _P, c_int64, _P]),
    "ssi_gemm_batched": (c_int, [c_int, c_int, c_int64, c_int64, c_int64, _P, c_int64, c_int64, _P, c_int64, c_int64, _P, c_int64, c_int64,
                                 c_float, _P, c_int, c_int, _P]),
    "ssi_gemm_swiglu_fwd": (c_int, [c_int64, c_int64, c_int64, _P, c_int64, _P, c_int64, _P, c_int64, _P, c_int64, c_int, _P]),
    "ssi_gemm_swiglu_bwd": (c_int, [c_int, c_int64, c_int64, c_int64, _P, c_int64, _P, c_int64, _P, c_int64, _P, c_int64, _P, c_int,
                                    _P]),
    "ssi_transpose": (c_int, [_P, c_int64, _P, c_int64, c_int64, c_int64, c_int, _P]),
    "ssi_ce_fwd": (c_int, [_P, c_int64, _P, c_int64, c_int64, c_int64, _P, _P, c_int, c_int, _P]),
    "ssi_ce_fwd_weighted": (c_int, [_P, c_int64, _P, _P, c_int64, c_int64, c_int64, _P, _P, c_int, c_int, _P]),
    "ssi_ce_reduce": (c_int, [_P, _P, c_int64, c_int64, c_int64, _P, _P]),
    "ssi_lmhead_ce_fwd": (c_int, [_P, c_int64, _P, c_int64, _P, c_int64, c_int64, c_int64, c_int64, c_int64, _P, c_int64, _P, _P, c_int, c_int, _P]),
    "ssi_lmhead_ce_bwd": (c_int, [_P, c_int64, _P, c_int64, _P, c_int64, _P, c_int64, c_int64, c_int64, _P, c_int64, _P, c_int64, c_int, c_int, _P]),
    "ssi_count_tokens": (c_int, [_P, _P, c_int64, _P, c_int, c_int64, c_int64, _P, _P]),
    "ssi_scale_inplace": (c_int, [_P, c_int64, c_float, _P, c_int, _P]),
    "ssi_sumsq_workspace_bytes": (c_int64, [c_int64]),
    "ssi_sumsq": (c_int, [_P, c_int64, c_int, _P, _P, c_int64, _P]),
    "ssi_adamw_step": (c_int, [_P, _P, _P, _P, c_int64, c_double, c_double, c_double, c_double, c_double, c_int64, _P, c_int,
                               c_int, _P]),
}

_lib = None


class HipLibraryError(RuntimeError):
    pass


def load() -> ctypes.CDLL:
    global _lib
    if _lib is not None:
        return _lib
    if not os.path.exists(LIB_PATH):
        raise HipLibraryError(
            f"{LIB_PATH} not found: the HIP extension is required (no CPU fallback). Build it with "
            f"`make -C {os.path.join(os.path.dirname(_HERE), 'csrc')}` or `__graft_entry__.build()`.")
    lib = ctypes.CDLL(LIB_PATH)
    for name, (res, args) in PROTOTYPES.items():
        try:
            fn = getattr(lib, name)
        except AttributeError as e:
            raise HipLibraryError(f"{LIB_PATH} does not export {name}") from e
        fn.restype, fn.argtypes = res, args
    v = lib.ssi_abi_version()
    if v != ABI_VERSION:
        raise HipLibraryError(f"libssi_hip ABI version {v} != expected {ABI_VERSION}")
    _lib = lib
    return lib


def check(rc: int, what: str) -> None:
    if rc != 0:
        msg = load().ssi_last_error()
        raise RuntimeError(f"{what} failed with code {rc}: {msg.decode() if msg else ''}")


def dtype_code(dtype: torch.dtype) -> int:
    if dtype == torch.float32:
        return SSI_F32
    if dtype == torch.bfloat16:
        return SSI_BF16
    raise TypeError(f"unsupported dtype {dtype}; supported: torch.float32, torch.bfloat16")


def ptr(t: torch.Tensor | None) -> int | None:
    if t is None:
        return None
    if not t.is_cuda:
        raise HipLibraryError("libssi_hip kernels need GPU tensors (there is no CPU fallback in the product path)")
    return t.data_ptr()


_RAW_STREAM = getattr(torch._C, "_cuda_getCurrentRawStream", None)
_CURRENT_DEVICE = getattr(torch._C, "_cuda_getDevice", None)


def stream_ptr() -> int:
    if _RAW_STREAM is not None and _CURRENT_DEVICE is not None:
        return _RAW_STREAM(_CURRENT_DEVICE())
    return torch.cuda.current_stream().cuda_stream
```

### speech-integration_amd/ssi/model.py

```python

from __future__ import annotations

import os

import logging
import math
from typing import Any, Optional

import torch
from torch import Tensor, nn

from . import _lib, ops
from .constants import CROSS_ENTROPY_IGNORE_IDX, PRECISION_STR_TO_DTYPE
from .llama_configs import ConfigLlama3_2
from .ops import GEMM_NN, GEMM_NT, GEMM_TN

LOGGER = logging.getLogger(__name__)

VOCAB_ALIGN = 256


def _align(n: int, a: int) -> int:
    return (n + a - 1) // a * a

# ... 208 lines not shown

    def zero_grad(self, set_to_none: bool = True) -> None:
        if set_to_none:
            self._grads_stale = self._grads_stale or self._grads_dirty
            for p, _, _ in self._param_src:
                p.grad = None
        elif self._grads_dirty or self._grads_stale:
            self._flat_grad.zero_()
            self._grads_stale = False
        self._grads_dirty = False
        self._emb_grad_written = False
        self.pending_grad_scale = None

    def _window_accumulates(self) -> bool:
        if not self._grads_dirty:
            return False
        dropped = [(p, name, rows) for p, name, rows in self._param_src if p.grad is None]
        if not dropped:
            return True
        if len(dropped) == len(self._param_src):
            self._grads_dirty, self._grads_stale, self._emb_grad_written = False, True, False
            self.pending_grad_scale = None
            return False
        for p, name, rows in dropped:
            p.grad = self._view(name, rows, self._flat_grad).zero_()
        return True

    def _finish_pending_exchange(self) -> None:
        sync = self.grad_sync
        if sync is not None and hasattr(sync, "finish_deferred"):
            sync.finish_deferred()

    def activation_bytes(self) -> int:
        return self._arena.bytes()

    def _mfma_shapes(self) -> bool:
        D, I = self.embed_dim, self.intermediate_dim
        return (self.dtype == torch.bfloat16 and D % 256 == 0 and self.qkv_dim % 256 == 0 and (2 * I) % 256 == 0
                and I % 64 == 0 and (self.num_heads * self.head_dim) % 64 == 0)

    def padded_seq_len(self, batch: int, seq: int) -> int:
        if not self._mfma_shapes():
            return seq
        g = 256 // math.gcd(batch, 256)
        g = max(g, 128)
        return _align(seq, g)

    @staticmethod
    def _document_ranges(input_pos: Tensor, max_pos: Optional[int] = None) -> tuple[Tensor, Tensor, Tensor]:
        B, S = input_pos.shape
        idx = torch.arange(S, device=input_pos.device, dtype=torch.int64).expand(B, S)
        is_start = input_pos == 0
        is_start[:, 0] = True
        doc_start = torch.where(is_start, idx, torch.zeros_like(idx)).cummax(dim=1).values
        nxt = torch.where(is_start, idx, torch.full_like(idx, S))
        nxt = torch.cat([nxt[:, 1:], torch.full_like(nxt[:, :1], S)], dim=1)
        doc_end = nxt.flip(1).cummin(dim=1).values.flip(1)
        as32 = lambda t: t.to(torch.int32).reshape(-1).contiguous()
        return as32(input_pos if max_pos is None else input_pos.clamp(max=max_pos)), as32(doc_start), as32(doc_end)

    split_small_grids = os.environ.get("SSI_SPLITK_NT", "1") != "0"

    split_tail_only = os.environ.get("SSI_TAIL_SPLIT", "1") != "0"

    def _gemm(self, layout: int, a: Tensor, b: Tensor, c: Tensor, residual: Optional[Tensor] = None) -> None:
        M, N = c.shape
        K = a.shape[1]
        mfma = self.split_small_grids and self.dtype == torch.bfloat16 and self._mfma_shapes() and M % 256 == 0 and N % 256 == 0
        if mfma and self.split_tail_only and layout in (GEMM_NT, GEMM_NN):
            tm, tn = M // 256, N // 256
            rounds = (tm * tn) // 256
            m_main = (rounds * 256) // tn
            if rounds >= 1 and 0 < m_main < tm and (tm - m_main) * tn <= 192:
                rows = m_main * 256
                ops.gemm(layout, a[:rows], b, c[:rows], residual=None if residual is None else residual[:rows])
                self._gemm(layout, a[rows:], b, c[rows:], None if residual is None else residual[rows:])
                return
        splits = ops.splitk_choice(M, N, K) if mfma else 1
        if splits > 1:
            wsk = self._arena.get("ws.splitk.nt", (splits * M * N,), torch.float32)
            ops.gemm_splitk(layout, a, b, c, splits, wsk, residual=residual)
        else:
            ops.gemm(layout, a, b, c, residual=residual)

    def build_attn_plan(self, input_pos: Tensor, force: bool = False):
        from . import attn_plan
        if input_pos is None or input_pos.is_cuda or input_pos.dim() != 2 or not self._mfma_shapes() or self.head_dim != 64:
            return None
        B, S = input_pos.shape
        if self.num_heads != 4 * self.num_kv_heads or self.padded_seq_len(B, S) != S or S % 128:
            return None
        return attn_plan.plan_from_input_pos(input_pos, self.num_heads, self.num_kv_heads, force=force)

    def _forward_hidden(self, tokens: Tensor, save: bool, input_pos: Optional[Tensor] = None, attn_plan=None) -> Tensor:
        B, S = tokens.shape
        pos = ds = de = None
        self.position_errors = None
        plan = None
        if input_pos is not None and save:
            if attn_plan is None and not input_pos.is_cuda:
                attn_plan = self.build_attn_plan(input_pos)
            if attn_plan is not None and attn_plan.matches(B, S, self.num_heads, self.num_kv_heads) and self._mfma_shapes():
                plan = attn_plan.to_device(tokens.device)
        if input_pos is not None:
            if input_pos.shape != tokens.shape:
                raise ValueError("input_pos must have the shape of tokens")
            if not input_pos.is_cuda and int(input_pos.max()) >= self._rope.shape[0]:
                raise ValueError("input_pos exceeds the RoPE cache")
            self.position_errors = torch.zeros(1, dtype=torch.int32, device=tokens.device)
            pos, ds, de = ops.doc_ranges(input_pos.to(tokens.device), self._rope.shape[0] - 1, self.position_errors)
        T, D, I = B * S, self.embed_dim, self.intermediate_dim
        H, KV, hd, dt, A = self.num_heads, self.num_kv_heads, self.head_dim, self.dtype, self._arena
        if pos is None and S > self._rope.shape[0]:
            raise ValueError(f"sequence length {S} exceeds the RoPE cache ({self._rope.shape[0]})")
        tok = tokens.reshape(-1).contiguous()
        L = self.num_layers
        h = A.get("h0" if save else "h0.x", (T, D), dt)
        ops.embed_fwd(tok, self._view("emb"), h, self.vocab_size)
        for l in range(L):
            sfx = f"{l}" if save else "x"
            xn1 = A.get("xn1.all", (L, T, D), dt)[l] if save else A.get("xn1.x", (T, D), dt)
            rstd1 = A.get(f"rstd1.{sfx}", (T,), torch.float32)
            ops.rmsnorm_fwd(h, self._view(f"L{l}.sa_norm"), xn1, rstd1, self.norm_eps)
            qkv = A.get(f"qkv.{sfx}", (T, self.qkv_dim), dt)
            ops.gemm_rope(xn1, self._view(f"L{l}.wqkv"), qkv, S, H + KV, hd, self._rope, positions=pos)
            att = A.get("att.all", (L, T, H * hd), dt)[l] if save else A.get("att.x", (T, H * hd), dt)
            lse = A.get(f"lse.{sfx}", (B * H * S,), torch.float32)
            ops.attn_fwd(qkv, att, lse, B, S, H, KV, hd, ds, de)
            hmid = A.get(f"hmid.{sfx}", (T, D), dt)
            self._gemm(GEMM_NT, att, self._view(f"L{l}.wo"), hmid, residual=h)
            xn2 = A.get(f"xn2.{sfx}", (T, D), dt)
            rstd2 = A.get(f"rstd2.{sfx}", (T,), torch.float32)
            ops.rmsnorm_fwd(hmid, self._view(f"L{l}.mlp_norm"), xn2, rstd2, self.norm_eps)
            gu = A.get(f"gu.{sfx}", (T, 2 * I), dt)
            act = A.get(f"act.{sfx}", (T, I), dt)
            ops.gemm_swiglu_fwd(xn2, self._view(f"L{l}.w13"), gu, act)
            hn_name = f"h{l + 1}" if save else f"hx{l & 1}"
            hnext = A.get(hn_name, (T, D), dt)
            self._gemm(GEMM_NT, act, self._view(f"L{l}.w2"), hnext, residual=hmid)
            h = hnext
        hn = A.get("hn" if save else "hn.x", (T, D), dt)
        rstdf = A.get("rstdf" if save else "rstdf.x", (T,), torch.float32)
        ops.rmsnorm_fwd(h, self.norm.scale, hn, rstdf, self.norm_eps)
        if save:
            self._fwd_generation += 1
            self._saved = {"tok": tok, "B": B, "S": S, "gen": self._fwd_generation, "pos": pos, "ds": ds, "de": de, "plan": plan}
        return hn

    def _backward_hidden(self, d_hn: Tensor, gen: int) -> None:
        sv = self._saved
        if sv is None or sv["gen"] != gen:
            raise RuntimeError("HipLlamaDecoder: backward called for a forward whose activations were overwritten; "
                               "run backward before the next training forward")
        B, S, tok = sv["B"], sv["S"], sv["tok"]
        pos, ds, de, plan = sv["pos"], sv["ds"], sv["de"], sv.get("plan")
        T, D, I = B * S, self.embed_dim, self.intermediate_dim
        H, KV, hd, dt, A = self.num_heads, self.num_kv_heads, self.head_dim, self.dtype, self._arena
        L = self.num_layers
        G = self._flat_grad
        self._finish_pending_exchange()
        acc = self._window_accumulates()
        gv = lambda name: self._view(name, None, G)
        ws = A.get("ws.rms", (max(ops.rmsnorm_bwd_workspace_bytes(T, D), 16),), torch.uint8)

        def wgrad(dy: Tensor, x: Tensor, name: str) -> None:
            g = gv(name)
            splits = ops.splitk_choice(g.shape[0], g.shape[1], T) if (dt == torch.bfloat16 and T % 64 == 0) else 1
            if splits > 1:
                wsk = A.get("ws.splitk", (splits * g.shape[0] * g.shape[1],), torch.float32)
                ops.gemm_splitk(GEMM_TN, dy, x, g, splits, wsk, accumulate=acc)
            else:
                ops.gemm(GEMM_TN, dy, x, g, accumulate=acc)

        sync = self.grad_sync if (self.grad_sync is not None and self.sync_this_backward) else None
        listener, self.bucket_listener = (self.bucket_listener if self.sync_this_backward else None), None

        def announce(name: str) -> None:
            if sync:
                sync.bucket_ready(*self._bucket_by_name[name])
            if listener is not None:
                listener(*self._bucket_by_name[name])

        Gp = self.wgrad_group
        if sync and Gp != self._bucket_group:
            raise RuntimeError("wgrad_group was changed after construction: the data-parallel buckets were laid out for the old grouping")
        defer = (Gp > 1 and dt == torch.bfloat16 and self._mfma_shapes() and T % 128 == 0 and T >= 256
                 and ops.splitk_choice(D, H * hd, T) > 1 and ops.splitk_choice(self.qkv_dim, D, T) > 1)
        xn1_all, att_all = A.get("xn1.all", (L, T, D), dt), A.get("att.all", (L, T, H * hd), dt)
        if defer:
            dhmid_all, dqkv_all = A.get("dh.b.all", (Gp, T, D), dt), A.get("dqkv.all", (Gp, T, self.qkv_dim), dt)
            lstride = (self._slices["L1.wqkv"][0] - self._slices["L0.wqkv"][0]) if L > 1 else 0

        def flush_attention_wgrads(l_lo: int) -> None:
            n = min(Gp, L - l_lo)
            g_o = torch.as_strided(G, (n, D, H * hd), (lstride, H * hd, 1), self._slices[f"L{l_lo}.wo"][0])
            g_qkv = torch.as_strided(G, (n, self.qkv_dim, D), (lstride, D, 1), self._slices[f"L{l_lo}.wqkv"][0])
            ops.gemm_batched(GEMM_TN, dhmid_all[:n], att_all[l_lo:l_lo + n], g_o, accumulate=acc)
            ops.gemm_batched(GEMM_TN, dqkv_all[:n], xn1_all[l_lo:l_lo + n], g_qkv, accumulate=acc)

        def dgrad(dy: Tensor, name: str, dx: Tensor) -> None:
            self._gemm(GEMM_NN, dy, self._view(name), dx)

        ws_bytes = ops.attn_bwd_workspace_bytes(B, S, H, KV, hd, dt) if T > 0 else 0
        if plan is not None:
            ws_bytes = max(ws_bytes, plan.workspace_bytes)
        attn_ws = A.get("ws.attn", (ws_bytes,), torch.uint8) if ws_bytes else None
        dh = A.get("dh.a", (T, D), dt)
        ops.rmsnorm_bwd(d_hn, A.get(f"h{L}", (T, D), dt), self.norm.scale, A.get("rstdf", (T,), torch.float32), None, dh,
                        gv("norm"), ws, accumulate=acc)
        announce("norm")
        for l in reversed(range(L)):
            xn1, xn2 = xn1_all[l], A.get(f"xn2.{l}", (T, D), dt)
            qkv, att = A.get(f"qkv.{l}", (T, self.qkv_dim), dt), att_all[l]
            hmid, gu, act = A.get(f"hmid.{l}", (T, D), dt), A.get(f"gu.{l}", (T, 2 * I), dt), A.get(f"act.{l}", (T, I), dt)
            h_in = A.get(f"h{l}", (T, D), dt)
            wgrad(dh, act, f"L{l}.w2")
            dgu = A.get("dgu", (T, 2 * I), dt)
            ops.gemm_swiglu_bwd(GEMM_NN, dh, self._view(f"L{l}.w2"), gu, dgu, A.get("dact", (T, I), dt))
            dxn = A.get("dxn", (T, D), dt)
            dgrad(dgu, f"L{l}.w13", dxn)
            wgrad(dgu, xn2, f"L{l}.w13")
            dhmid = dhmid_all[l % Gp] if defer else A.get("dh.b", (T, D), dt)
            ops.rmsnorm_bwd(dxn, hmid, self._view(f"L{l}.mlp_norm"), A.get(f"rstd2.{l}", (T,), torch.float32), dh, dhmid,
                            gv(f"L{l}.mlp_norm"), ws, accumulate=acc)
            datt = A.get("datt", (T, H * hd), dt)
            dgrad(dhmid, f"L{l}.wo", datt)
            if not defer:
                wgrad(dhmid, att, f"L{l}.wo")
            dqkv = dqkv_all[l % Gp] if defer else A.get("dqkv", (T, self.qkv_dim), dt)
            delta = A.get("delta", (B * H * S,), torch.float32)
            ops.attn_bwd(qkv, att, datt, A.get(f"lse.{l}", (B * H * S,), torch.float32), dqkv, delta, B, S, H, KV, hd, ds, de,
                         rope_table=self._rope, positions=pos, workspace=attn_ws, plan=plan)
            dgrad(dqkv, f"L{l}.wqkv", dxn)
            if not defer:
                wgrad(dqkv, xn1, f"L{l}.wqkv")
            ops.rmsnorm_bwd(dxn, h_in, self._view(f"L{l}.sa_norm"), A.get(f"rstd1.{l}", (T,), torch.float32), dhmid, dh,
                            gv(f"L{l}.sa_norm"), ws, accumulate=acc)
            announce(f"L{l}.mlp")
            if defer and l % Gp == 0:
                flush_attention_wgrads(l)
            if l % self._bucket_group == 0:
                announce(f"attn.{l}")
        ws_e = A.get("ws.emb", (max(_lib.load().ssi_embed_bwd_workspace_bytes(self.vocab_size), 16),), torch.uint8)
        if not acc and not self._emb_grad_written:
            gv("emb").zero_()
        ops.embed_bwd(tok, dh, gv("emb"), self.vocab_size, ws_e)
        self._grads_dirty, self._grads_stale, self._emb_grad_written = True, False, False
        announce("emb")
        self._saved = None
        self.attach_grads()

    def _head_logits(self, hn: Tensor, arena_name: Optional[str] = None) -> Tensor:
        T = hn.shape[0]
        if arena_name is None:
            logits = torch.empty((T, self.vocab_pad), dtype=self.dtype, device=self.device)
        else:
            logits = self._arena.get(arena_name, (T, self.vocab_pad), self.dtype)
        ops.gemm(GEMM_NT, hn, self._view("emb"), logits)
        return logits

    def _head_backward(self, dlogits: Tensor, hn: Tensor, alpha_dev: Optional[Tensor]) -> Tensor:
        T, D = hn.shape
        self._finish_pending_exchange()
        acc = self._window_accumulates()
        d_hn = self._arena.get("d_hn", (T, D), self.dtype)
        ops.gemm(GEMM_NN, dlogits, self._view("emb"), d_hn, alpha_dev=alpha_dev)
        g_emb = self._view("emb", None, self._flat_grad)
        rows_main = self._head_wgrad_main_rows(T)
        if rows_main:
            Vp = self.vocab_pad
            ops.gemm(GEMM_TN, dlogits[:, :rows_main], hn, g_emb[:rows_main], alpha_dev=alpha_dev, accumulate=acc)
            tail, splits = Vp - rows_main, self._head_wgrad_tail_splits
            wsk = self._arena.get("ws.splitk.head", (splits * tail * D,), torch.float32)
            ops.gemm_splitk(GEMM_TN, dlogits[:, rows_main:], hn, g_emb[rows_main:], splits, wsk, alpha_dev=alpha_dev, accumulate=acc)
        else:
            ops.gemm(GEMM_TN, dlogits, hn, g_emb, alpha_dev=alpha_dev, accumulate=acc)
        self._emb_grad_written = True
        return d_hn

    _head_wgrad_tail_splits = 3

    def _head_wgrad_main_rows(self, T: int, n_cu: int = 256) -> int:
        if os.environ.get("SSI_HEAD_WGRAD_TAIL", "1") == "0" or self.dtype != torch.bfloat16 or not self._mfma_shapes() or T % 128 or T < 64 * 6 * self._head_wgrad_tail_splits:
            return 0
        tm, tn = self.vocab_pad // 256, self.embed_dim // 256
        full_rounds = (tm * tn) // n_cu
        if full_rounds == 0 or (full_rounds * n_cu) % tn:
            return 0
        tail_tiles = tm * tn - full_rounds * n_cu
        if tail_tiles == 0 or 2 * tail_tiles >= n_cu or tail_tiles * self._head_wgrad_tail_splits > n_cu:
            return 0
        return full_rounds * n_cu // tn * 256

    def _check_inputs(self, tokens: Tensor, mask, encoder_input, encoder_mask, input_pos) -> Tensor:
        if encoder_input is not None or encoder_mask is not None:
            raise NotImplementedError("no encoder inputs: the reference's model is decoder-only (ssi/model.py:34)")
        if mask is not None and input_pos is None:
            raise NotImplementedError("a dense attention mask is never materialised: packed batches pass input_pos, from which "
                                      "the block-causal mask follows (ssi/data/packed.py)")
        if tokens.dim() != 2 or tokens.dtype != torch.int64:
            raise ValueError("tokens must be an int64 tensor of shape [batch, seq]")
# ... 172 lines not shown
```

### speech-integration_amd/ssi/ops.py

```python

from __future__ import annotations

import torch
from typing import Optional
from torch import Tensor

from . import _lib
from ._lib import GEMM_NN, GEMM_NT, GEMM_TN, check, dtype_code, ptr, stream_ptr

__all__ = ["lmhead_ce_fwd", "lmhead_ce_bwd", "doc_ranges", "embed_fwd", "embed_bwd", "rmsnorm_fwd", "rmsnorm_bwd", "rope_", "attn_fwd", "attn_bwd", "attn_bwd_workspace_bytes", "swiglu_fwd",
           "swiglu_bwd", "gemm", "gemm_splitk", "splitk_choice", "gemm_swiglu_fwd", "gemm_swiglu_bwd", "transpose", "ce_fwd", "ce_reduce", "count_tokens", "scale_", "sumsq", "adamw_step", "set_impl", "set_attn_impl", "attn_last_dispatch",
           "GEMM_NT", "GEMM_NN", "GEMM_TN"]


def set_impl(impl: int) -> int:
    return _lib.load().ssi_set_impl(impl)


def set_attn_impl(which: int, mode: int) -> int:
    return _lib.load().ssi_set_attn_impl(which, mode)


def attn_last_dispatch() -> int:
    return _lib.load().ssi_attn_last_dispatch()


def _byte_ws(nbytes: int, like: Tensor) -> Tensor:
    return torch.empty(max(int(nbytes), 16), dtype=torch.uint8, device=like.device)


def embed_fwd(tokens: Tensor, table: Tensor, out: Tensor, vocab: int) -> None:
    n, dim = tokens.numel(), table.shape[1]
    assert tokens.dtype == torch.int64 and tokens.is_contiguous() and out.is_contiguous() and table.stride(1) == 1
    assert table.stride(0) == dim and out.shape[-1] == dim and out.numel() == n * dim and out.dtype == table.dtype
    check(_lib.load().ssi_embed_fwd(ptr(tokens), ptr(table), ptr(out), n, dim, vocab, dtype_code(table.dtype),
                                    stream_ptr()), "ssi_embed_fwd")


def embed_bwd(tokens: Tensor, dout: Tensor, dtable: Tensor, vocab: int, workspace: Tensor | None = None) -> None:
    lib = _lib.load()
    n, dim = tokens.numel(), dtable.shape[1]
    assert tokens.dtype == torch.int64 and tokens.is_contiguous() and dout.is_contiguous() and dtable.stride(0) == dim
    need = lib.ssi_embed_bwd_workspace_bytes(vocab)
    if workspace is None or workspace.numel() * workspace.element_size() < need:
        workspace = _byte_ws(need, dout)
    check(lib.ssi_embed_bwd(ptr(tokens), ptr(dout), ptr(dtable), n, dim, vocab, dtype_code(dtable.dtype), ptr(workspace),
                            workspace.numel() * workspace.element_size(), stream_ptr()), "ssi_embed_bwd")


def rmsnorm_fwd(x: Tensor, scale: Tensor, y: Tensor, rstd: Tensor | None, eps: float) -> None:
    dim = x.shape[-1]
    rows = x.numel() // dim
    assert x.is_contiguous() and y.is_contiguous() and scale.is_contiguous() and scale.numel() == dim
    assert rstd is None or (rstd.dtype == torch.float32 and rstd.numel() >= rows)
    check(_lib.load().ssi_rmsnorm_fwd(ptr(x), ptr(scale), ptr(y), ptr(rstd), rows, dim, eps, dtype_code(x.dtype),
                                      stream_ptr()), "ssi_rmsnorm_fwd")


def rmsnorm_bwd_workspace_bytes(rows: int, dim: int) -> int:
    return _lib.load().ssi_rmsnorm_bwd_workspace_bytes(rows, dim)


def rmsnorm_bwd(dy: Tensor, x: Tensor, scale: Tensor, rstd: Tensor, dres: Tensor | None, dx: Tensor, dscale: Tensor,
                workspace: Tensor | None = None, accumulate: bool = True) -> None:
    lib = _lib.load()
    dim = x.shape[-1]
    rows = x.numel() // dim
    assert dy.is_contiguous() and x.is_contiguous() and dx.is_contiguous() and dscale.is_contiguous()
    assert dres is None or dres.is_contiguous()
    need = lib.ssi_rmsnorm_bwd_workspace_bytes(rows, dim)
    if workspace is None or workspace.numel() * workspace.element_size() < need:
        workspace = _byte_ws(need, dy)
    check(lib.ssi_rmsnorm_bwd(ptr(dy), ptr(x), ptr(scale), ptr(rstd), ptr(dres), ptr(dx), ptr(dscale), int(accumulate), rows, dim,
                              dtype_code(x.dtype), ptr(workspace), workspace.numel() * workspace.element_size(),
                              stream_ptr()), "ssi_rmsnorm_bwd")


def rope_(x: Tensor, seq_len: int, n_heads_rot: int, head_dim: int, table: Tensor, inverse: bool = False,
          positions: Tensor | None = None) -> None:
    assert x.dim() == 2 and x.stride(1) == 1 and table.dtype == torch.float32 and table.is_contiguous()
    assert positions is None or (positions.dtype == torch.int32 and positions.numel() == x.shape[0])
    check(_lib.load().ssi_rope_inplace(ptr(x), x.stride(0), x.shape[0], seq_len, n_heads_rot, head_dim, ptr(table),
                                       table.shape[0], ptr(positions), int(inverse), dtype_code(x.dtype), stream_ptr()),
          "ssi_rope_inplace")


def gemm_rope(a: Tensor, b: Tensor, c: Tensor, seq_len: int, n_heads_rot: int, head_dim: int, table: Tensor,
              positions: Tensor | None = None) -> None:
    assert a.dim() == 2 and b.dim() == 2 and c.dim() == 2 and a.stride(1) == 1 and b.stride(1) == 1 and c.stride(1) == 1
    M, K = a.shape
    N = b.shape[0]
    assert b.shape[1] == K and c.shape == (M, N) and a.dtype == b.dtype == c.dtype
    assert table.dtype == torch.float32 and table.is_contiguous() and table.shape[1] * 2 == head_dim
    assert positions is None or (positions.dtype == torch.int32 and positions.numel() == M)
    check(_lib.load().ssi_gemm_rope(M, N, K, ptr(a), a.stride(0), ptr(b), b.stride(0), ptr(c), c.stride(0), seq_len, n_heads_rot, head_dim,
                                    ptr(table), table.shape[0], ptr(positions), dtype_code(a.dtype), stream_ptr()), "ssi_gemm_rope")


def _doc_ptrs(doc_start: Optional[Tensor], doc_end: Optional[Tensor], rows: int):
    if doc_start is None and doc_end is None:
        return None, None
    assert doc_start is not None and doc_end is not None, "doc_start and doc_end go together"
    for t in (doc_start, doc_end):
        assert t.dtype == torch.int32 and t.is_contiguous() and t.numel() == rows
    return ptr(doc_start), ptr(doc_end)


def doc_ranges(input_pos: Tensor, max_pos: int, n_clamped: Tensor | None = None) -> tuple[Tensor, Tensor, Tensor]:
    assert input_pos.dim() == 2 and input_pos.dtype == torch.int64
    assert n_clamped is None or (n_clamped.dtype == torch.int32 and n_clamped.numel() == 1)
    ip = input_pos.contiguous()
    B, S = ip.shape
    out = torch.empty(3, B * S, dtype=torch.int32, device=ip.device)
    check(_lib.load().ssi_doc_ranges(ptr(ip), B, S, int(max_pos), ptr(out[0]), ptr(out[1]), ptr(out[2]), ptr(n_clamped), stream_ptr()),
          "ssi_doc_ranges")
    return out[0], out[1], out[2]


def set_gemm_tile_order(dynamic: bool) -> None:
    check(_lib.load().ssi_set_gemm_tile_order(_lib.TILES_DYNAMIC if dynamic else _lib.TILES_STATIC), "ssi_set_gemm_tile_order")


def attn_fwd(qkv: Tensor, out: Tensor, lse: Tensor, batch: int, seq: int, n_heads: int, n_kv: int, head_dim: int,
             doc_start: Optional[Tensor] = None, doc_end: Optional[Tensor] = None) -> None:
    assert qkv.dim() == 2 and qkv.stride(1) == 1 and out.is_contiguous() and lse.dtype == torch.float32
    assert qkv.shape[0] == batch * seq and out.numel() == batch * seq * n_heads * head_dim
    assert lse.numel() >= batch * n_heads * seq
    ds, de = _doc_ptrs(doc_start, doc_end, batch * seq)
    check(_lib.load().ssi_attn_varlen_fwd(ptr(qkv), qkv.stride(0), ptr(out), ptr(lse), ds, de, batch, seq, n_heads, n_kv, head_dim,
                                          dtype_code(qkv.dtype), stream_ptr()), "ssi_attn_varlen_fwd")


def attn_bwd_workspace_bytes(batch: int, seq: int, n_heads: int, n_kv: int, head_dim: int, dtype: torch.dtype) -> int:
    return int(_lib.load().ssi_attn_bwd_workspace_bytes(batch, seq, n_heads, n_kv, head_dim, dtype_code(dtype)))


def attn_bwd(qkv: Tensor, out: Tensor, dout: Tensor, lse: Tensor, dqkv: Tensor, delta: Tensor, batch: int, seq: int,
             n_heads: int, n_kv: int, head_dim: int, doc_start: Optional[Tensor] = None, doc_end: Optional[Tensor] = None,
             rope_table: Optional[Tensor] = None, positions: Optional[Tensor] = None, workspace: Optional[Tensor] = None, plan=None) -> None:
    assert qkv.stride(1) == 1 and dqkv.stride() == qkv.stride() and out.is_contiguous() and dout.is_contiguous()
    assert delta.dtype == torch.float32 and delta.numel() >= batch * n_heads * seq
    assert workspace is None or (workspace.is_contiguous() and workspace.dtype == torch.uint8)
    assert rope_table is None or (rope_table.dtype == torch.float32 and rope_table.is_contiguous() and rope_table.shape[1] * 2 == head_dim)
    assert positions is None or (positions.dtype == torch.int32 and positions.numel() == batch * seq)
    ds, de = _doc_ptrs(doc_start, doc_end, batch * seq)
    ws_bytes = workspace.numel() if workspace is not None else 0
    table_len = rope_table.shape[0] if rope_table is not None else 0
    plan_dev = plan_header = None
    if plan is not None:
        assert plan.dev is not None and plan.dev.device == qkv.device and plan.matches(batch, seq, n_heads, n_kv)
        assert ds is not None or (positions is None and plan.n_docs == batch), "a plan for plain rows has one document per row"
        if ws_bytes < plan.workspace_bytes:
            workspace = _byte_ws(plan.workspace_bytes, qkv)
            ws_bytes = workspace.numel()
        plan_dev, plan_header = ptr(plan.dev), plan.host.data_ptr()
    check(_lib.load().ssi_attn_varlen_bwd_plan(ptr(qkv), qkv.stride(0), ptr(out), ptr(dout), ptr(lse), ptr(dqkv), ptr(delta), ds, de,
                                               ptr(rope_table), table_len, ptr(positions), batch, seq, n_heads, n_kv, head_dim,
                                               dtype_code(qkv.dtype), ptr(workspace), ws_bytes, plan_dev, plan_header, stream_ptr()),
          "ssi_attn_varlen_bwd_plan")


def swiglu_fwd(gu: Tensor, act: Tensor) -> None:
    inter = act.shape[-1]
    rows = act.numel() // inter
    assert gu.is_contiguous() and act.is_contiguous() and gu.shape[-1] == 2 * inter
    check(_lib.load().ssi_swiglu_fwd(ptr(gu), ptr(act), rows, inter, dtype_code(gu.dtype), stream_ptr()), "ssi_swiglu_fwd")


def swiglu_bwd(dact: Tensor, gu: Tensor, dgu: Tensor) -> None:
    inter = dact.shape[-1]
    rows = dact.numel() // inter
    assert gu.is_contiguous() and dact.is_contiguous() and dgu.is_contiguous() and gu.shape[-1] == 2 * inter
    check(_lib.load().ssi_swiglu_bwd(ptr(dact), ptr(gu), ptr(dgu), rows, inter, dtype_code(gu.dtype), stream_ptr()),
          "ssi_swiglu_bwd")


def gemm(layout: int, a: Tensor, b: Tensor, c: Tensor, *, residual: Tensor | None = None, alpha: float = 1.0,
         alpha_dev: Tensor | None = None, accumulate: bool = False) -> None:
    assert a.dim() == 2 and b.dim() == 2 and c.dim() == 2 and a.stride(1) == 1 and b.stride(1) == 1 and c.stride(1) == 1
    assert a.dtype == b.dtype == c.dtype
    M, N = c.shape
    if layout == GEMM_NT:
        K = a.shape[1]
        assert a.shape[0] == M and b.shape == (N, K)
    elif layout == GEMM_NN:
        K = a.shape[1]
        assert a.shape[0] == M and b.shape == (K, N)
    else:
        K = a.shape[0]
        assert a.shape[1] == M and b.shape == (K, N)
    if residual is not None:
        assert residual.shape == c.shape and residual.stride() == c.stride() and residual.dtype == c.dtype
    if alpha_dev is not None:
        assert alpha_dev.dtype == torch.float32 and alpha_dev.numel() == 1
    check(_lib.load().ssi_gemm(layout, M, N, K, ptr(a), a.stride(0), ptr(b), b.stride(0), ptr(c), c.stride(0),
                               ptr(residual), alpha, ptr(alpha_dev), int(accumulate), dtype_code(c.dtype), stream_ptr()),
          "ssi_gemm")


def splitk_choice(M: int, N: int, K: int, n_cu: int = 256) -> int:
    if M % 256 or N % 256 or K % 64:
        return 1
    tiles, nk = (M // 256) * (N // 256), K // 64
    if tiles >= 4 * n_cu or tiles % n_cu == 0:
        return 1
    best, best_t = 1, None
    for s in (1, 2, 3, 4, 6, 8, 12, 16):
        if s > nk:
            break
        waves = -(-tiles * s // n_cu)
        t = waves * -(-nk // s) * 1.8e-6 + ((s + 1) * M * N * 4 / 4.0e12 if s > 1 else 0.0)
        if best_t is None or t < best_t * 0.97:
            best, best_t = s, t
    return best


def gemm_splitk(layout: int, a: Tensor, b: Tensor, c: Tensor, splits: int, workspace: Tensor, *, alpha: float = 1.0,
                alpha_dev: Tensor | None = None, accumulate: bool = False, residual: Tensor | None = None) -> None:
    if splits <= 1:
        return gemm(layout, a, b, c, alpha=alpha, alpha_dev=alpha_dev, accumulate=accumulate, residual=residual)
    M, N = c.shape
    K = a.shape[1] if layout in (GEMM_NT, GEMM_NN) else a.shape[0]
    assert a.stride(1) == 1 and b.stride(1) == 1 and c.stride(1) == 1 and a.dtype == b.dtype == c.dtype
    if residual is not None:
        assert residual.shape == c.shape and residual.stride() == c.stride() and residual.dtype == c.dtype and not accumulate
    check(_lib.load().ssi_gemm_splitk(layout, M, N, K, ptr(a), a.stride(0), ptr(b), b.stride(0), ptr(c), c.stride(0), ptr(residual),
                                      alpha, ptr(alpha_dev), int(accumulate), dtype_code(c.dtype), splits, ptr(workspace),
                                      workspace.numel() * workspace.element_size(), stream_ptr()), "ssi_gemm_splitk")


def gemm_batched(layout: int, a: Tensor, b: Tensor, c: Tensor, *, alpha: float = 1.0, alpha_dev: Tensor | None = None,
                 accumulate: bool = False) -> None:
    assert a.dim() == 3 and b.dim() == 3 and c.dim() == 3 and a.shape[0] == b.shape[0] == c.shape[0]
    assert a.stride(2) == 1 and b.stride(2) == 1 and c.stride(2) == 1 and a.dtype == b.dtype == c.dtype
    n, M, N = c.shape
    if layout == GEMM_NT:
        K = a.shape[2]
        assert a.shape[1] == M and b.shape[1:] == (N, K)
    elif layout == GEMM_NN:
        K = a.shape[2]
        assert a.shape[1] == M and b.shape[1:] == (K, N)
    else:
        K = a.shape[1]
        assert a.shape[2] == M and b.shape[1:] == (K, N)
    if alpha_dev is not None:
        assert alpha_dev.dtype == torch.float32 and alpha_dev.numel() == 1
    check(_lib.load().ssi_gemm_batched(layout, n, M, N, K, ptr(a), a.stride(1), a.stride(0), ptr(b), b.stride(1), b.stride(0), ptr(c),
                                       c.stride(1), c.stride(0), alpha, ptr(alpha_dev), int(accumulate), dtype_code(c.dtype), stream_ptr()),
          "ssi_gemm_batched")


def gemm_swiglu_fwd(x: Tensor, w13: Tensor, gu: Tensor, act: Tensor) -> None:
    M, K = x.shape
    inter = act.shape[1]
    assert w13.shape == (2 * inter, K) and gu.shape == (M, 2 * inter) and act.shape[0] == M
    assert x.stride(1) == 1 and w13.stride(1) == 1 and gu.is_contiguous() and act.is_contiguous()
    check(_lib.load().ssi_gemm_swiglu_fwd(M, inter, K, ptr(x), x.stride(0), ptr(w13), w13.stride(0), ptr(gu), gu.stride(0), ptr(act),
                                          act.stride(0), dtype_code(x.dtype), stream_ptr()), "ssi_gemm_swiglu_fwd")


def gemm_swiglu_bwd(layout: int, dy: Tensor, w2: Tensor, gu: Tensor, dgu: Tensor, dact_ws: Tensor | None) -> None:
    M, K = dy.shape
    inter = gu.shape[1] // 2
    assert w2.shape == ((inter, K) if layout == GEMM_NT else (K, inter)) and dgu.shape == gu.shape and gu.shape[0] == M
    assert dy.stride(1) == 1 and w2.stride(1) == 1 and gu.is_contiguous() and dgu.is_contiguous()
    check(_lib.load().ssi_gemm_swiglu_bwd(layout, M, inter, K, ptr(dy), dy.stride(0), ptr(w2), w2.stride(0), ptr(gu), gu.stride(0),
                                          ptr(dgu), dgu.stride(0), ptr(dact_ws), dtype_code(dy.dtype), stream_ptr()),
          "ssi_gemm_swiglu_bwd")


def transpose(src: Tensor, dst: Tensor) -> None:
    assert src.dim() == 2 and dst.dim() == 2 and src.stride(1) == 1 and dst.stride(1) == 1 and src.dtype == dst.dtype
    assert dst.shape == (src.shape[1], src.shape[0])
    check(_lib.load().ssi_transpose(ptr(src), src.stride(0), ptr(dst), dst.stride(0), src.shape[0], src.shape[1],
                                    dtype_code(src.dtype), stream_ptr()), "ssi_transpose")


def ce_fwd(logits: Tensor, labels: Tensor, vocab: int, ignore_index: int, row_loss: Tensor, row_lse: Tensor | None,
           write_grad: bool, row_weight: Tensor | None = None) -> None:
    assert logits.dim() == 2 and logits.stride(1) == 1 and labels.dtype == torch.int64 and labels.is_contiguous()
    rows = logits.shape[0]
    assert labels.numel() == rows and row_loss.dtype == torch.float32 and row_loss.numel() >= rows
    if row_weight is None:
        check(_lib.load().ssi_ce_fwd(ptr(logits), logits.stride(0), ptr(labels), rows, vocab, ignore_index, ptr(row_loss),
                                     ptr(row_lse), int(write_grad), dtype_code(logits.dtype), stream_ptr()), "ssi_ce_fwd")
        return
    assert row_weight.dtype == torch.float32 and row_weight.is_contiguous() and row_weight.numel() == rows and row_weight.device == logits.device
    check(_lib.load().ssi_ce_fwd_weighted(ptr(logits), logits.stride(0), ptr(labels), ptr(row_weight), rows, vocab, ignore_index, ptr(row_loss),
                                          ptr(row_lse), int(write_grad), dtype_code(logits.dtype), stream_ptr()), "ssi_ce_fwd_weighted")


def ce_reduce(row_loss: Tensor, labels: Tensor, vocab: int, ignore_index: int, out: Tensor) -> None:
    assert out.dtype == torch.float32 and out.numel() >= 4 and labels.is_contiguous()
    check(_lib.load().ssi_ce_reduce(ptr(row_loss), ptr(labels), labels.numel(), vocab, ignore_index, ptr(out), stream_ptr()),
          "ssi_ce_reduce")


def lmhead_ce_fwd(hidden: Tensor, table: Tensor, labels: Tensor, vocab: int, ignore_index: int, logits_ws: Tensor, row_loss: Tensor,
                  stats: Tensor, write_grad: bool) -> None:
    rows, dim = hidden.shape
    vocab_pad = table.shape[0]
    assert table.shape[1] == dim and logits_ws.shape == (rows, vocab_pad) and hidden.stride(1) == 1 and table.stride(1) == 1
    assert labels.dtype == torch.int64 and labels.is_contiguous() and labels.numel() == rows and stats.dtype == torch.float32 and stats.numel() >= 4
    assert row_loss.dtype == torch.float32 and row_loss.numel() >= rows and hidden.dtype == table.dtype == logits_ws.dtype
    check(_lib.load().ssi_lmhead_ce_fwd(ptr(hidden), hidden.stride(0), ptr(table), table.stride(0), ptr(labels), rows, dim, vocab, vocab_pad,
                                        ignore_index, ptr(logits_ws), logits_ws.stride(0), ptr(row_loss), ptr(stats), int(write_grad),
                                        dtype_code(hidden.dtype), stream_ptr()), "ssi_lmhead_ce_fwd")


def lmhead_ce_bwd(dlogits: Tensor, hidden: Tensor, table: Tensor, alpha_dev: Tensor | None, d_hidden: Tensor, d_table: Tensor,
                  accumulate_d_table: bool) -> None:
    rows, dim = hidden.shape
    vocab_pad = table.shape[0]
    assert dlogits.shape == (rows, vocab_pad) and d_hidden.shape == hidden.shape and d_table.shape == table.shape
    assert alpha_dev is None or (alpha_dev.dtype == torch.float32 and alpha_dev.numel() == 1)
    check(_lib.load().ssi_lmhead_ce_bwd(ptr(dlogits), dlogits.stride(0), ptr(hidden), hidden.stride(0), ptr(table), table.stride(0),
                                        ptr(alpha_dev), rows, dim, vocab_pad, ptr(d_hidden), d_hidden.stride(0), ptr(d_table),
                                        d_table.stride(0), int(accumulate_d_table), dtype_code(hidden.dtype), stream_ptr()), "ssi_lmhead_ce_bwd")


def count_tokens(tokens: Tensor, labels: Tensor | None, ranges: Tensor, pad_id: int, ignore_index: int, out: Tensor) -> None:
    n_ranges = ranges.numel() // 2
    assert tokens.dtype == torch.int64 and tokens.is_contiguous() and ranges.dtype == torch.int64 and out.dtype == torch.int64
    assert out.numel() >= n_ranges + 2 and (labels is None or (labels.is_contiguous() and labels.numel() == tokens.numel()))
    check(_lib.load().ssi_count_tokens(ptr(tokens), ptr(labels), tokens.numel(), ptr(ranges), n_ranges, pad_id,
                                       ignore_index, ptr(out), stream_ptr()), "ssi_count_tokens")


def scale_(x: Tensor, scale: float = 1.0, scale_dev: Tensor | None = None) -> None:
    assert x.is_contiguous()
    check(_lib.load().ssi_scale_inplace(ptr(x), x.numel(), scale, ptr(scale_dev), dtype_code(x.dtype), stream_ptr()),
          "ssi_scale_inplace")


def sumsq(x: Tensor, out: Tensor, workspace: Tensor | None = None) -> None:
    lib = _lib.load()
    assert x.is_contiguous() and out.dtype == torch.float32
    need = lib.ssi_sumsq_workspace_bytes(x.numel())
    if workspace is None or workspace.numel() * workspace.element_size() < need:
        workspace = _byte_ws(need, x)
    check(lib.ssi_sumsq(ptr(x), x.numel(), dtype_code(x.dtype), ptr(out), ptr(workspace),
                        workspace.numel() * workspace.element_size(), stream_ptr()), "ssi_sumsq")


def adamw_step(param: Tensor, grad: Tensor, exp_avg: Tensor, exp_avg_sq: Tensor, *, lr: float, beta1: float, beta2: float,
               eps: float, weight_decay: float, step: int, grad_scale_dev: Tensor | None = None,
               zero_grad: bool = False, skip_nonfinite_scale: bool = False) -> None:
    assert param.is_contiguous() and grad.is_contiguous() and exp_avg.is_contiguous() and exp_avg_sq.is_contiguous()
    assert param.numel() == grad.numel() == exp_avg.numel() == exp_avg_sq.numel()
    assert param.dtype == grad.dtype == exp_avg.dtype == exp_avg_sq.dtype
    check(_lib.load().ssi_adamw_step(ptr(param), ptr(grad), ptr(exp_avg), ptr(exp_avg_sq), param.numel(), lr, beta1, beta2,
# ... 3 lines not shown
```

Measured before the change: 156,900 tokens/s.

## Split-K the wave-quantization tail of persistent MFMA GEMMs into K-slice units

```diff
diff --git a/include/ssi_hip.h b/include/ssi_hip.h
--- a/include/ssi_hip.h
+++ b/include/ssi_hip.h
@@ -7,7 +7,7 @@
 extern "C" {
 #endif
 
-#define SSI_ABI_VERSION 9
+#define SSI_ABI_VERSION 10
 
 enum { SSI_F32 = 0, SSI_BF16 = 1 };
 enum { SSI_OK = 0, SSI_ERR_ARG = 1, SSI_ERR_UNSUPPORTED = 2, SSI_ERR_WORKSPACE = 3, SSI_ERR_HIP = 1000  };
@@ -93,6 +93,21 @@
              void* C, int64_t ldc, const void* R, float alpha, const float* alpha_dev, int accumulate, int dtype,
              void* stream);
 
+int ssi_gemm_tail_plan(int64_t M, int64_t N, int64_t K, int cus, int* n_main, int* splits);
+int64_t ssi_gemm_tail_workspace_bytes(int64_t M, int64_t N, int64_t K, int cus);
+int64_t ssi_gemm_tail_units(int64_t M, int64_t N, int64_t K, int cus, int32_t* units, int64_t capacity);
+int ssi_gemm_tail(int layout, int64_t M, int64_t N, int64_t K, const void* A, int64_t lda, const void* B, int64_t ldb,
+                  void* C, int64_t ldc, const void* R, float alpha, const float* alpha_dev, int accumulate, int dtype,
+                  void* workspace, int64_t workspace_bytes, void* stream);
+int ssi_gemm_rope_tail(int64_t M, int64_t N, int64_t K, const void* A, int64_t lda, const void* B, int64_t ldb, void* C, int64_t ldc,
+                       int64_t seq_len, int n_heads_rot, int head_dim, const float* rope_table, int64_t table_len,
+                       const int32_t* positions, int dtype, void* workspace, int64_t workspace_bytes, void* stream);
+int ssi_gemm_swiglu_fwd_tail(int64_t M, int64_t inter, int64_t K, const void* X, int64_t ldx, const void* W13, int64_t ldw, void* GU,
+                             int64_t ldgu, void* ACT, int64_t ldact, int dtype, void* workspace, int64_t workspace_bytes, void* stream);
+int ssi_gemm_swiglu_bwd_tail(int layout, int64_t M, int64_t inter, int64_t K, const void* DY, int64_t lddy, const void* W2, int64_t ldw,
+                             const void* GU, int64_t ldgu, void* DGU, int64_t lddgu, void* dact_ws, int dtype, void* workspace,
+                             int64_t workspace_bytes, void* stream);
+
 int64_t ssi_gemm_splitk_workspace_bytes(int64_t M, int64_t N, int splits);
 int ssi_gemm_splitk(int layout, int64_t M, int64_t N, int64_t K, const void* A, int64_t lda, const void* B, int64_t ldb,
                     void* C, int64_t ldc, const void* R, float alpha, const float* alpha_dev, int accumulate, int dtype,
diff --git a/speech-integration_amd/csrc/common_hip.h b/speech-integration_amd/csrc/common_hip.h
--- a/speech-integration_amd/csrc/common_hip.h
+++ b/speech-integration_amd/csrc/common_hip.h
@@ -154,7 +154,10 @@
                              int64_t ldb, const void* C, int64_t ldc, const void* R);
 int ssi_gemm_mfma_bf16(int layout, int64_t M, int64_t N, int64_t K, const void* A, int64_t lda, const void* B,
                        int64_t ldb, void* C, int64_t ldc, const void* R, float alpha, const float* alpha_dev,
-                       int accumulate, void* stream);
+                       int accumulate, void* stream, void* tail_ws = nullptr, int64_t tail_ws_bytes = 0);
+int ssi_gemm_mfma_tail_plan(int64_t M, int64_t N, int64_t K, int cus, int* n_main, int* splits);
+int64_t ssi_gemm_mfma_tail_units(int64_t M, int64_t N, int64_t K, int cus, int32_t* out, int64_t cap);
+int ssi_gemm_mfma_num_cu();
 int ssi_gemm_mfma_bf16_splitk(int layout, int64_t M, int64_t N, int64_t K, const void* A, int64_t lda, const void* B,
                               int64_t ldb, void* C, int64_t ldc, const void* R, float alpha, const float* alpha_dev,
                               int accumulate, int splits, float* slabs, void* stream);
@@ -163,13 +166,15 @@
                                 void* stream, int* rc);
 void ssi_gemm_mfma_set_dynamic_tiles(int on);
 bool ssi_gemm_rope_mfma(int64_t M, int64_t N, int64_t K, const void* A, int64_t lda, const void* B, int64_t ldb, void* C, int64_t ldc,
-                        const float* rope, const int32_t* positions, int64_t seq, int64_t rot_cols, void* stream, int* rc);
+                        const float* rope, const int32_t* positions, int64_t seq, int64_t rot_cols, void* stream, int* rc,
+                        void* tail_ws = nullptr, int64_t tail_ws_bytes = 0);
 bool ssi_gemm_swiglu_supported(int64_t M, int64_t inter, int64_t K, const void* p0, const void* p1, const void* p2, const void* p3,
                                int64_t ld0, int64_t ld1, int64_t ld2, int64_t ld3);
 int ssi_gemm_swiglu_fwd_mfma(int64_t M, int64_t inter, int64_t K, const void* X, int64_t ldx, const void* W13, int64_t ldw,
-                             void* GU, int64_t ldgu, void* ACT, int64_t ldact, void* stream);
+                             void* GU, int64_t ldgu, void* ACT, int64_t ldact, void* stream, void* tail_ws = nullptr, int64_t tail_ws_bytes = 0);
 int ssi_gemm_swiglu_bwd_mfma(int layout, int64_t M, int64_t inter, int64_t K, const void* DY, int64_t lddy, const void* W2, int64_t ldw,
-                             const void* GU, int64_t ldgu, void* DGU, int64_t lddgu, void* stream);
+                             const void* GU, int64_t ldgu, void* DGU, int64_t lddgu, void* stream, void* tail_ws = nullptr,
+                             int64_t tail_ws_bytes = 0);
 bool ssi_gemm_swiglu_bwd_nn_supported(int64_t K, int64_t lddy, int64_t ldw);
 
 bool ssi_gemm_f32_mfma_supported(int layout, int64_t M, int64_t N, int64_t K, const void* A, int64_t lda, const void* B,
diff --git a/speech-integration_amd/csrc/gemm_generic.hip b/speech-integration_amd/csrc/gemm_generic.hip
--- a/speech-integration_amd/csrc/gemm_generic.hip
+++ b/speech-integration_amd/csrc/gemm_generic.hip
@@ -82,6 +82,31 @@
 extern "C" int ssi_gemm(int layout, int64_t M, int64_t N, int64_t K, const void* A, int64_t lda, const void* B,
                         int64_t ldb, void* C, int64_t ldc, const void* R, float alpha, const float* alpha_dev,
                         int accumulate, int dtype, void* stream) {
+    return ssi_gemm_tail(layout, M, N, K, A, lda, B, ldb, C, ldc, R, alpha, alpha_dev, accumulate, dtype, nullptr, 0, stream);
+}
+
+extern "C" int ssi_gemm_tail_plan(int64_t M, int64_t N, int64_t K, int cus, int* n_main, int* splits) {
+    int nm = 0, sp = 1;
+    const int rc = ssi_gemm_mfma_tail_plan(M, N, K, cus, &nm, &sp);
+    if (n_main) *n_main = nm;
+    if (splits) *splits = sp;
+    return rc;
+}
+
+extern "C" int64_t ssi_gemm_tail_workspace_bytes(int64_t M, int64_t N, int64_t K, int cus) {
+    int nm = 0, sp = 1;
+    if (ssi_gemm_mfma_tail_plan(M, N, K, cus, &nm, &sp) <= 1) return 0;
+    return ((M / 256) * (N / 256) - nm) * sp * (int64_t)(256 * 256 * sizeof(float));
+}
+
+extern "C" int64_t ssi_gemm_tail_units(int64_t M, int64_t N, int64_t K, int cus, int32_t* units, int64_t capacity) {
+    if (!units || capacity < 0) return -1;
+    return ssi_gemm_mfma_tail_units(M, N, K, cus, units, capacity);
+}
+
+extern "C" int ssi_gemm_tail(int layout, int64_t M, int64_t N, int64_t K, const void* A, int64_t lda, const void* B,
+                             int64_t ldb, void* C, int64_t ldc, const void* R, float alpha, const float* alpha_dev,
+                             int accumulate, int dtype, void* workspace, int64_t workspace_bytes, void* stream) {
     SSI_CHECK_ARG(A && B && C && M >= 0 && N >= 0 && K >= 0 && ldc >= N);
     SSI_CHECK_ARG(layout == SSI_GEMM_NT || layout == SSI_GEMM_NN || layout == SSI_GEMM_TN);
     if (M == 0 || N == 0) return SSI_OK;
@@ -100,7 +125,7 @@
     if (f32_ok && g_impl != SSI_IMPL_GENERIC)
         return ssi_gemm_f32_mfma(layout, M, N, K, A, lda, B, ldb, C, ldc, R, alpha, alpha_dev, accumulate, stream);
     if (mfma_ok && g_impl != SSI_IMPL_GENERIC)
-        return ssi_gemm_mfma_bf16(layout, M, N, K, A, lda, B, ldb, C, ldc, R, alpha, alpha_dev, accumulate, stream);
+        return ssi_gemm_mfma_bf16(layout, M, N, K, A, lda, B, ldb, C, ldc, R, alpha, alpha_dev, accumulate, stream, workspace, workspace_bytes);
 
     SSI_CHECK_ARG(ssi_cdiv(M, 64) <= 65535);
     dim3 grid((unsigned)ssi_cdiv(N, 64), (unsigned)ssi_cdiv(M, 64));
@@ -157,12 +182,20 @@
 extern "C" int ssi_gemm_rope(int64_t M, int64_t N, int64_t K, const void* A, int64_t lda, const void* B, int64_t ldb, void* C, int64_t ldc,
                              int64_t seq_len, int n_heads_rot, int head_dim, const float* rope_table, int64_t table_len,
                              const int32_t* positions, int dtype, void* stream) {
+    return ssi_gemm_rope_tail(M, N, K, A, lda, B, ldb, C, ldc, seq_len, n_heads_rot, head_dim, rope_table, table_len, positions, dtype, nullptr, 0,
+                              stream);
+}
+
+extern "C" int ssi_gemm_rope_tail(int64_t M, int64_t N, int64_t K, const void* A, int64_t lda, const void* B, int64_t ldb, void* C, int64_t ldc,
+                                  int64_t seq_len, int n_heads_rot, int head_dim, const float* rope_table, int64_t table_len,
+                                  const int32_t* positions, int dtype, void* workspace, int64_t workspace_bytes, void* stream) {
     SSI_CHECK_ARG(A && B && C && rope_table && M >= 0 && N > 0 && K > 0 && seq_len > 0 && n_heads_rot > 0 && head_dim > 0);
     SSI_CHECK_ARG((int64_t)n_heads_rot * head_dim <= N && (positions != nullptr || table_len >= seq_len));
     if (M == 0) return SSI_OK;
     int rc = SSI_OK;
     if (dtype == SSI_BF16 && head_dim == 64 && g_impl != SSI_IMPL_GENERIC &&
-        ssi_gemm_rope_mfma(M, N, K, A, lda, B, ldb, C, ldc, rope_table, positions, seq_len, (int64_t)n_heads_rot * head_dim, stream, &rc))
+        ssi_gemm_rope_mfma(M, N, K, A, lda, B, ldb, C, ldc, rope_table, positions, seq_len, (int64_t)n_heads_rot * head_dim, stream, &rc,
+                           workspace, workspace_bytes))
         return rc;
     if ((rc = ssi_gemm(SSI_GEMM_NT, M, N, K, A, lda, B, ldb, C, ldc, nullptr, 1.f, nullptr, 0, dtype, stream))) return rc;
     return ssi_rope_inplace(C, ldc, M, seq_len, n_heads_rot, head_dim, rope_table, table_len, positions, 0, dtype, stream);
@@ -170,9 +203,15 @@
 
 extern "C" int ssi_gemm_swiglu_fwd(int64_t M, int64_t inter, int64_t K, const void* X, int64_t ldx, const void* W13, int64_t ldw,
                                    void* GU, int64_t ldgu, void* ACT, int64_t ldact, int dtype, void* stream) {
+    return ssi_gemm_swiglu_fwd_tail(M, inter, K, X, ldx, W13, ldw, GU, ldgu, ACT, ldact, dtype, nullptr, 0, stream);
+}
+
+extern "C" int ssi_gemm_swiglu_fwd_tail(int64_t M, int64_t inter, int64_t K, const void* X, int64_t ldx, const void* W13, int64_t ldw,
+                                        void* GU, int64_t ldgu, void* ACT, int64_t ldact, int dtype, void* workspace, int64_t workspace_bytes,
+                                        void* stream) {
     SSI_CHECK_ARG(X && W13 && GU && ACT && M >= 0 && inter > 0 && K > 0 && ldgu >= 2 * inter && ldact >= inter);
     if (dtype == SSI_BF16 && g_impl != SSI_IMPL_GENERIC && ssi_gemm_swiglu_supported(M, inter, K, X, W13, GU, ACT, ldx, ldw, ldgu, ldact))
-        return ssi_gemm_swiglu_fwd_mfma(M, inter, K, X, ldx, W13, ldw, GU, ldgu, ACT, ldact, stream);
+        return ssi_gemm_swiglu_fwd_mfma(M, inter, K, X, ldx, W13, ldw, GU, ldgu, ACT, ldact, stream, workspace, workspace_bytes);
     if (int rc = ssi_gemm(SSI_GEMM_NT, M, 2 * inter, K, X, ldx, W13, ldw, GU, ldgu, nullptr, 1.f, nullptr, 0, dtype, stream)) return rc;
     SSI_CHECK_ARG(ldgu == 2 * inter && ldact == inter);
     return ssi_swiglu_fwd(GU, ACT, M, inter, dtype, stream);
@@ -181,11 +220,17 @@
 extern "C" int ssi_gemm_swiglu_bwd(int layout, int64_t M, int64_t inter, int64_t K, const void* DY, int64_t lddy, const void* W2,
                                    int64_t ldw, const void* GU, int64_t ldgu, void* DGU, int64_t lddgu, void* dact_ws, int dtype,
                                    void* stream) {
+    return ssi_gemm_swiglu_bwd_tail(layout, M, inter, K, DY, lddy, W2, ldw, GU, ldgu, DGU, lddgu, dact_ws, dtype, nullptr, 0, stream);
+}
+
+extern "C" int ssi_gemm_swiglu_bwd_tail(int layout, int64_t M, int64_t inter, int64_t K, const void* DY, int64_t lddy, const void* W2,
+                                        int64_t ldw, const void* GU, int64_t ldgu, void* DGU, int64_t lddgu, void* dact_ws, int dtype,
+                                        void* workspace, int64_t workspace_bytes, void* stream) {
     SSI_CHECK_ARG(DY && W2 && GU && DGU && M >= 0 && inter > 0 && K > 0 && ldgu >= 2 * inter && lddgu >= 2 * inter);
     SSI_CHECK_ARG(layout == SSI_GEMM_NT || layout == SSI_GEMM_NN);
     if (dtype == SSI_BF16 && g_impl != SSI_IMPL_GENERIC && ssi_gemm_swiglu_supported(M, inter, K, DY, W2, GU, DGU, lddy, ldw, ldgu, lddgu) &&
         (layout == SSI_GEMM_NT || ssi_gemm_swiglu_bwd_nn_supported(K, lddy, ldw)))
-        return ssi_gemm_swiglu_bwd_mfma(layout, M, inter, K, DY, lddy, W2, ldw, GU, ldgu, DGU, lddgu, stream);
+        return ssi_gemm_swiglu_bwd_mfma(layout, M, inter, K, DY, lddy, W2, ldw, GU, ldgu, DGU, lddgu, stream, workspace, workspace_bytes);
     SSI_CHECK_ARG(dact_ws != nullptr && ldgu == 2 * inter && lddgu == 2 * inter);
     if (int rc = ssi_gemm(layout, M, inter, K, DY, lddy, W2, ldw, dact_ws, inter, nullptr, 1.f, nullptr, 0, dtype, stream)) return rc;
     return ssi_swiglu_bwd(dact_ws, GU, DGU, M, inter, dtype, stream);
diff --git a/speech-integration_amd/csrc/gemm_mfma.hip b/speech-integration_amd/csrc/gemm_mfma.hip
--- a/speech-integration_amd/csrc/gemm_mfma.hip
+++ b/speech-integration_amd/csrc/gemm_mfma.hip
@@ -95,6 +95,22 @@
     const int gm = (tiles_m - group * GM) < GM ? (tiles_m - group * GM) : GM;
     tm = group * GM + in_group % gm;
     tn = in_group / gm;
+}
+
+__host__ __device__ inline int nt4_slice_lo(int nk, int s, int splits) { return (int)(((unsigned)nk * (unsigned)s / (unsigned)splits) & ~1u); }
+__host__ __device__ inline int nt4_slice_hi(int nk, int s, int splits) { return s + 1 == splits ? nk : nt4_slice_lo(nk, s + 1, splits); }
+__host__ __device__ inline int nt4_unit_decode(int t, int n_main, int n_tail, int nk, int splits, int& k_lo, int& k_hi) {
+    if (t < n_main) { k_lo = 0; k_hi = nk; return t; }
+    const unsigned r = (unsigned)(t - n_main), s = r / (unsigned)n_tail;
+    k_lo = nt4_slice_lo(nk, (int)s, splits);
+    k_hi = nt4_slice_hi(nk, (int)s, splits);
+    return n_main + (int)(r - s * (unsigned)n_tail);
+}
+__host__ __device__ inline int nt4_part_len(int n, int x) { return (n >> 3) + (x < (n & 7) ? 1 : 0); }
+__host__ __device__ inline int nt4_part_lo(int n, int x) { const int q = n >> 3, r = n & 7; return x < r ? x * (q + 1) : r * (q + 1) + (x - r) * q; }
+__host__ __device__ inline int nt4_unit_at(int x, int p, int n_main, int n_tail_units) {
+    const int ml = nt4_part_len(n_main, x);
+    return p < ml ? nt4_part_lo(n_main, x) + p : n_main + nt4_part_lo(n_tail_units, x) + (p - ml);
 }
 
 __device__ int g_nt4_sched[16][16];
@@ -441,13 +457,16 @@
                                          int64_t lda, const bf16_t* __restrict__ B, int64_t ldb,
                                          bf16_t* __restrict__ C, int64_t ldc, const bf16_t* __restrict__ R,
                                          float alpha, const float* __restrict__ alpha_dev, EpiArgs ea, int slot,
-                                         int splits, float* __restrict__ slabs) {
+                                         int splits, float* __restrict__ slabs, int n_main_arg) {
+    constexpr bool TAIL = !SPLITK && !BATCHED;
     const int tid = threadIdx.x, lane = tid & 63;
     const int wave = __builtin_amdgcn_readfirstlane(tid >> 6);
     const int wm = wave >> 1, wn = wave & 1;
     const int per_prob = tiles_m * tiles_n;
     const int ntiles_out = BATCHED ? per_prob * ea.batch : per_prob;
-    const int ntiles = SPLITK ? ntiles_out * splits : ntiles_out;
+    const int n_main = TAIL ? n_main_arg : ntiles_out, n_tail = ntiles_out - n_main;
+    const int n_tail1 = n_tail > 0 ? n_tail : 1, n_tail_units = TAIL ? n_tail * splits : 0;
+    const int ntiles = SPLITK ? ntiles_out * splits : n_main + n_tail_units;
     auto locate = [&](int t, int& tm, int& tn) {
         int tt = SPLITK ? t % ntiles_out : t, pb = 0;
         if constexpr (BATCHED) { pb = tt / per_prob; tt -= pb * per_prob; }
@@ -458,12 +477,28 @@
     const int nk_total = (int)(K / BK);
     auto k_lo = [&](int t) { return SPLITK ? (int)(((int64_t)nk_total * (t / ntiles_out) / splits) & ~1LL) : 0; };
     auto k_hi = [&](int t) { return SPLITK ? ((t / ntiles_out) + 1 == splits ? nk_total : (int)(((int64_t)nk_total * (t / ntiles_out + 1) / splits) & ~1LL)) : nk_total; };
+    auto locate_k = [&](int t, int& tm, int& tn, int& lo, int& hi) {
+        if constexpr (TAIL) {
+            tile_from_t(nt4_unit_decode(t, n_main, n_tail1, nk_total, splits, lo, hi), tiles_m, tiles_n, tm, tn);
+            return 0;
+        } else {
+            lo = k_lo(t);
+            hi = k_hi(t);
+            return locate(t, tm, tn);
+        }
+    };
 
     int* sched = g_nt4_sched[slot < 0 ? 0 : slot];
     volatile int* lds_next = reinterpret_cast<volatile int*>(smem + PIPE_BYTES);
     const int xcd = (int)blockIdx.x & 7, span_q = ntiles >> 3, span_r = ntiles & 7;
-    auto span_len = [&](int x) { return span_q + (x < span_r ? 1 : 0); };
-    auto span_lo = [&](int x) { return x < span_r ? x * (span_q + 1) : span_r * (span_q + 1) + (x - span_r) * span_q; };
+    auto span_len = [&](int x) {
+        if constexpr (TAIL) return nt4_part_len(n_main, x) + nt4_part_len(n_tail_units, x);
+        return span_q + (x < span_r ? 1 : 0);
+    };
+    auto unit_at = [&](int x, int p) {
+        if constexpr (TAIL) return nt4_unit_at(x, p, n_main, n_tail_units);
+        return (x < span_r ? x * (span_q + 1) : span_r * (span_q + 1) + (x - span_r) * span_q) + p;
+    };
     auto span_wgs = [&](int x) { return (G - x + 7) >> 3; };
     auto span_fixed = [&](int x) { const int n = 2 * span_wgs(x); return n < span_len(x) ? n : span_len(x); };
     const bool dynamic = slot >= 0;
@@ -475,13 +510,13 @@
     auto receive_tile = [&]() -> int {
         if (!dynamic) {
             my_idx += G >> 3;
-            return ((G & 7) == 0 && my_idx < span_len(xcd)) ? span_lo(xcd) + my_idx : -1;
+            return ((G & 7) == 0 && my_idx < span_len(xcd)) ? unit_at(xcd, my_idx) : -1;
         }
         asm volatile("s_waitcnt lgkmcnt(0)\n\ts_barrier" ::: "memory");
         if (tid == 0) {
             int t = -1;
             const int i = pending + span_fixed(xcd);
-            if (i < span_len(xcd)) t = span_lo(xcd) + i;
+            if (i < span_len(xcd)) t = unit_at(xcd, i);
             if (t < 0) {
                 int seen[8];
 #pragma unroll
@@ -490,7 +525,7 @@
                     const int x = (xcd + k) & 7;
                     if (seen[x] + span_fixed(x) >= span_len(x)) continue;
                     const int j = atomicAdd(&sched[x], 1) + span_fixed(x);
-                    if (j < span_len(x)) t = span_lo(x) + j;
+                    if (j < span_len(x)) t = unit_at(x, j);
                 }
             }
             *lds_next = t;
@@ -498,11 +533,11 @@
         asm volatile("s_waitcnt lgkmcnt(0)\n\ts_barrier" ::: "memory");
         return __builtin_amdgcn_readfirstlane(*lds_next);
     };
-    int cur = ((int)blockIdx.x >> 3) < span_len(xcd) ? span_lo(xcd) + ((int)blockIdx.x >> 3) : -1;
+    int cur = ((int)blockIdx.x >> 3) < span_len(xcd) ? unit_at(xcd, (int)blockIdx.x >> 3) : -1;
     int nxt = -1;
     if (dynamic) {
         const int second = ((int)blockIdx.x >> 3) + span_wgs(xcd);
-        nxt = (cur >= 0 && second < span_len(xcd)) ? span_lo(xcd) + second : -1;
+        nxt = (cur >= 0 && second < span_len(xcd)) ? unit_at(xcd, second) : -1;
     }
 
     f32x4 acc[8][8];
@@ -514,13 +549,13 @@
     const bf16_t* baseB = B;
     const int64_t kstepA_ = A_COL ? BK * lda : BK, kstepB_ = B_COL ? BK * ldb : BK;
     auto set_load_tile = [&](int t) {
-        int tm, tn;
-        const int pb = locate(t, tm, tn);
+        int tm, tn, klo, khi;
+        const int pb = locate_k(t, tm, tn, klo, khi);
         const bf16_t* Ap = BATCHED ? A + pb * ea.bsA : A;
         const bf16_t* Bp = BATCHED ? B + pb * ea.bsB : B;
-        baseA = (A_COL ? Ap + (int64_t)tm * BM : Ap + (int64_t)tm * BM * lda) + k_lo(t) * kstepA_;
-        baseB = (B_COL ? Bp + (int64_t)tn * BN : Bp + (int64_t)tn * (EPI == EPI_SWIGLU_FWD ? BN / 2 : BN) * ldb) + k_lo(t) * kstepB_;
-        lnk = k_hi(t) - k_lo(t);
+        baseA = (A_COL ? Ap + (int64_t)tm * BM : Ap + (int64_t)tm * BM * lda) + klo * kstepA_;
+        baseB = (B_COL ? Bp + (int64_t)tn * BN : Bp + (int64_t)tn * (EPI == EPI_SWIGLU_FWD ? BN / 2 : BN) * ldb) + klo * kstepB_;
+        lnk = khi - klo;
     };
     auto advance = [&]() {
         if (++lkt == lnk) {
@@ -667,9 +702,9 @@
     const float al = alpha * (alpha_dev ? *alpha_dev : 1.f);
     const int g = lane >> 4;
     while (cur >= 0) {
-        int tm, tn;
-        const int pb = locate(cur, tm, tn);
-        const int nk = k_hi(cur) - k_lo(cur);
+        int tm, tn, klo_, khi_;
+        const int pb = locate_k(cur, tm, tn, klo_, khi_);
+        const int nk = khi_ - klo_;
         using B0_ = std::integral_constant<int, 0>;
         using B1_ = std::integral_constant<int, 1>;
         if (nxt >= 0) request_tile();
@@ -705,8 +740,8 @@
                 hi[d] = (unsigned)__builtin_amdgcn_update_dpp((int)ob[d], (int)oa[d], 0x108 , 0xF, 0x3, false);
             }
         };
-        if constexpr (SPLITK) {
-            const __amdgpu_buffer_rsrc_t rsS = make_rsrc(slabs + ((int64_t)cur * 4 + wave) * (64 * 64 * 4));
+        if (SPLITK || (TAIL && cur >= n_main)) {
+            const __amdgpu_buffer_rsrc_t rsS = make_rsrc(slabs + ((int64_t)(cur - n_main * (TAIL ? 1 : 0)) * 4 + wave) * (64 * 64 * 4));
 #pragma unroll
             for (int i = 0; i < 8; ++i)
 #pragma unroll
@@ -721,7 +756,7 @@
                     __builtin_amdgcn_raw_buffer_store_b128(v, rsS, lane * 16, (i * 8 + j) * 1024, 0);
                     __builtin_amdgcn_sched_barrier(0);
                 }
-        } else {
+        } else if constexpr (!SPLITK) {
         const int64_t row0 = (int64_t)tm * BM + wm * NT4_WM;
         const int lane_row = lane & 7, lane_col = ((lane >> 3) & 1) * 32 + (g & 1) * 16 + (g >> 1) * 8;
         auto epilogue = [&](auto scale_c) {
@@ -906,35 +941,25 @@
                                                                      int64_t lda, const bf16_t* __restrict__ B, int64_t ldb,
                                                                      bf16_t* __restrict__ C, int64_t ldc, const bf16_t* __restrict__ R,
                                                                      float alpha, const float* __restrict__ alpha_dev, EpiArgs ea, int slot,
-                                                                     int splits, float* __restrict__ slabs) {
+                                                                     int splits, float* __restrict__ slabs, int n_main) {
     extern __shared__ __attribute__((aligned(16))) char smem[];
-    nt4_body<A_COL, B_COL, EPI, PREV, SPLITK, BATCHED>(smem, tiles_m, tiles_n, K, A, lda, B, ldb, C, ldc, R, alpha, alpha_dev, ea, slot, splits, slabs);
-}
-
-__global__ __launch_bounds__(256) void nt4_splitk_reduce_kernel(const float* __restrict__ slabs, int splits, int tiles_m, int tiles_n,
-                                                                bf16_t* __restrict__ C, int64_t ldc, const bf16_t* __restrict__ R, float alpha,
-                                                                const float* __restrict__ alpha_dev, int accumulate) {
+    nt4_body<A_COL, B_COL, EPI, PREV, SPLITK, BATCHED>(smem, tiles_m, tiles_n, K, A, lda, B, ldb, C, ldc, R, alpha, alpha_dev, ea, slot, splits, slabs, n_main);
+}
+
+template <int EPI>
+__global__ __launch_bounds__(256) void nt4_splitk_reduce_kernel(const float* __restrict__ slabs, int splits, int tiles_m, int tiles_n, int t0,
+                                                                int ntiles, bf16_t* __restrict__ C, int64_t ldc, const bf16_t* __restrict__ R,
+                                                                float alpha, const float* __restrict__ alpha_dev, int accumulate, EpiArgs ea) {
+    constexpr int DUOS = EPI == EPI_SWIGLU_FWD ? 1 : 2;
     const int lane = threadIdx.x & 63;
     const int64_t u = (int64_t)blockIdx.x * 4 + (threadIdx.x >> 6);
-    const int ntiles = tiles_m * tiles_n;
-    if (u >= (int64_t)ntiles * 64) return;
-    const int jd = (int)(u & 1), i = (int)((u >> 1) & 7), wave = (int)((u >> 4) & 3), t = (int)(u >> 6);
+    if (u >= (int64_t)ntiles * 32 * DUOS) return;
+    const int jd = DUOS == 2 ? (int)(u & 1) : 0, ui = (int)(u / DUOS);
+    const int i = ui & 7, wave = (ui >> 3) & 3, t = ui >> 5;
     const int wm = wave >> 1, wn = wave & 1, g = lane >> 4;
     int tm, tn;
-    tile_from_t(t, tiles_m, tiles_n, tm, tn);
+    tile_from_t(t0 + t, tiles_m, tiles_n, tm, tn);
     const float al = alpha * (alpha_dev ? *alpha_dev : 1.f);
-    f32x4 sum[4];
-#pragma unroll
-    for (int j = 0; j < 4; ++j) sum[j] = f32x4{0.f, 0.f, 0.f, 0.f};
-    for (int s = 0; s < splits; ++s) {
-        const float* p = slabs + (((int64_t)s * ntiles + t) * 4 + wave) * (64 * 64 * 4) + (int64_t)(i * 8 + jd * 4) * 256 + lane * 4;
-#pragma unroll
-        for (int j = 0; j < 4; ++j) {
-            const f32x4 v = *reinterpret_cast<const f32x4*>(p + j * 256);
-#pragma unroll
-            for (int r = 0; r < 4; ++r) sum[j][r] += v[r];
-        }
-    }
     auto pair = [&](const f32x4& a, const f32x4& b) {
         bf16x4 x, y;
 #pragma unroll
@@ -946,66 +971,221 @@
         o[0] = s0[0]; o[1] = s1[0]; o[2] = s0[1]; o[3] = s1[1];
         return o;
     };
-    const u32x4 oa = pair(sum[0], sum[1]), ob = pair(sum[2], sum[3]);
+    auto duo = [&](int d, u32x4& lo, u32x4& hi) {
+        f32x4 sum[4];
+#pragma unroll
+        for (int j = 0; j < 4; ++j) sum[j] = f32x4{0.f, 0.f, 0.f, 0.f};
+        for (int s = 0; s < splits; ++s) {
+            const float* p = slabs + (((int64_t)s * ntiles + t) * 4 + wave) * (64 * 64 * 4) + (int64_t)(i * 8 + d * 4) * 256 + lane * 4;
+#pragma unroll
+            for (int j = 0; j < 4; ++j) {
+                const f32x4 v = *reinterpret_cast<const f32x4*>(p + j * 256);
+#pragma unroll
+                for (int r = 0; r < 4; ++r) sum[j][r] += v[r];
+            }
+        }
+        const u32x4 oa = pair(sum[0], sum[1]), ob = pair(sum[2], sum[3]);
+#pragma unroll
+        for (int q = 0; q < 4; ++q) {
+            lo[q] = (unsigned)__builtin_amdgcn_update_dpp((int)oa[q], (int)ob[q], 0x118 , 0xF, 0xC, false);
+            hi[q] = (unsigned)__builtin_amdgcn_update_dpp((int)ob[q], (int)oa[q], 0x108 , 0xF, 0x3, false);
+        }
+    };
+    const int lane_row = lane & 7, lane_col = ((lane >> 3) & 1) * 32 + (g & 1) * 16 + (g >> 1) * 8;
+    const int64_t row = (int64_t)tm * BM + wm * NT4_WM + i * 16 + lane_row;
     u32x4 lo, hi;
-#pragma unroll
-    for (int d = 0; d < 4; ++d) {
-        lo[d] = (unsigned)__builtin_amdgcn_update_dpp((int)oa[d], (int)ob[d], 0x118 , 0xF, 0xC, false);
-        hi[d] = (unsigned)__builtin_amdgcn_update_dpp((int)ob[d], (int)oa[d], 0x108 , 0xF, 0x3, false);
-    }
-    const int lane_row = lane & 7, lane_col = ((lane >> 3) & 1) * 32 + (g & 1) * 16 + (g >> 1) * 8;
-    bf16_t* base = C + ((int64_t)tm * BM + wm * NT4_WM + i * 16 + lane_row) * ldc + (int64_t)tn * BN + wn * NT4_WN + jd * 64 + lane_col;
-    const int64_t r_off = R ? (R - C) : 0;
-    auto finish = [&](u32x4 o, bf16_t* dst) {
-        if (accumulate || R) {
-            bf16x8 ob8 = __builtin_bit_cast(bf16x8, o);
-            const bf16x8 c = *reinterpret_cast<const bf16x8*>(dst + r_off);
-#pragma unroll
-            for (int e = 0; e < 8; ++e) ob8[e] = (bf16_t)((float)ob8[e] + (float)c[e]);
-            o = __builtin_bit_cast(u32x4, ob8);
-        }
-        *reinterpret_cast<u32x4*>(dst) = o;
-    };
-    finish(lo, base);
-    finish(hi, base + 8 * ldc);
-}
-
-template <bool A_COL, bool B_COL, int EPI, int PREV, bool SPLITK = false, bool BATCHED = false>
-int launch_nt4(int tiles_m, int tiles_n, int64_t K, const void* A, int64_t lda, const void* B, int64_t ldb, void* C, int64_t ldc,
-               const void* R, float alpha, const float* alpha_dev, hipStream_t st, EpiArgs ea = EpiArgs{nullptr, 0, nullptr, 0, 0},
-               int splits = 1, float* slabs = nullptr) {
-    static_assert(!BATCHED || (!SPLITK && EPI == EPI_PLAIN), "batched form: plain epilogue, no split-K");
-    auto kern = gemm_nt4dma_kernel<A_COL, B_COL, EPI, PREV, SPLITK, BATCHED>;
-    static const hipError_t attr_rc = hipFuncSetAttribute((const void*)kern, hipFuncAttributeMaxDynamicSharedMemorySize, NT4_LDS_BYTES);
-    if (attr_rc != hipSuccess) { ssi_set_error("gemm_nt4: cannot reserve %d B of LDS: %s", NT4_LDS_BYTES, hipGetErrorString(attr_rc)); return SSI_ERR_HIP + (int)attr_rc; }
+    duo(jd, lo, hi);
+    if constexpr (EPI == EPI_PLAIN) {
+        bf16_t* base = C + row * ldc + (int64_t)tn * BN + wn * NT4_WN + jd * 64 + lane_col;
+        const int64_t r_off = R ? (R - C) : 0;
+        auto finish = [&](u32x4 o, bf16_t* dst) {
+            if (accumulate || R) {
+                bf16x8 ob8 = __builtin_bit_cast(bf16x8, o);
+                const bf16x8 c = *reinterpret_cast<const bf16x8*>(dst + r_off);
+#pragma unroll
+                for (int e = 0; e < 8; ++e) ob8[e] = (bf16_t)((float)ob8[e] + (float)c[e]);
+                o = __builtin_bit_cast(u32x4, ob8);
+            }
+            *reinterpret_cast<u32x4*>(dst) = o;
+        };
+        finish(lo, base);
+        finish(hi, base + 8 * ldc);
+    } else if constexpr (EPI == EPI_ROPE) {
+        bf16_t* base = C + row * ldc + (int64_t)tn * BN + wn * NT4_WN + jd * 64 + lane_col;
+        if ((int64_t)tn * BN < ea.rot_cols) {
+            auto rotate = [&](u32x4& o, int64_t r) {
+                const int prow = ea.pos ? ea.pos[r] : (int)(r % ea.seq);
+                const float* tb = ea.rope + (int64_t)prow * 64 + lane_col;
+                const f32x4 c01 = *reinterpret_cast<const f32x4*>(tb), c23 = *reinterpret_cast<const f32x4*>(tb + 4);
+                bf16x8 v = __builtin_bit_cast(bf16x8, o);
+#pragma unroll
+                for (int p = 0; p < 4; ++p) {
+                    const f32x4& c = p < 2 ? c01 : c23;
+                    float o0, o1;
+                    ssi_rope_pair((float)v[2 * p], (float)v[2 * p + 1], c[(p & 1) * 2], c[(p & 1) * 2 + 1], o0, o1);
+                    v[2 * p] = (bf16_t)o0;
+                    v[2 * p + 1] = (bf16_t)o1;
+                }
+                o = __builtin_bit_cast(u32x4, v);
+            };
+            rotate(lo, row);
+            rotate(hi, row + 8);
+        }
+        *reinterpret_cast<u32x4*>(base) = lo;
+        *reinterpret_cast<u32x4*>(base + 8 * ldc) = hi;
+    } else if constexpr (EPI == EPI_SWIGLU_FWD) {
+        u32x4 ulo, uhi;
+        duo(1, ulo, uhi);
+        const int64_t col = (int64_t)tn * (BN / 2) + wn * 64 + lane_col;
+        auto finish = [&](const u32x4& gq, const u32x4& uq, int64_t r) {
+            const bf16x8 gv = __builtin_bit_cast(bf16x8, gq), uv = __builtin_bit_cast(bf16x8, uq);
+            bf16x8 av;
+#pragma unroll
+            for (int e = 0; e < 8; ++e) {
+                const float sl = (float)(bf16_t)ssi_silu<bf16_t>((float)gv[e]);
+                av[e] = (bf16_t)(sl * (float)uv[e]);
+            }
+            *reinterpret_cast<u32x4*>(C + r * ldc + col) = gq;
+            *reinterpret_cast<u32x4*>(C + r * ldc + ea.inter + col) = uq;
+            *reinterpret_cast<bf16x8*>(ea.out2 + r * ea.ld_out2 + col) = av;
+        };
+        finish(lo, ulo, row);
+        finish(hi, uhi, row + 8);
+    } else {
+        const int64_t col = (int64_t)tn * BN + wn * NT4_WN + jd * 64 + lane_col;
+        auto finish = [&](const u32x4& dq, int64_t r) {
+            const bf16_t* gp = ea.in2 + r * ea.ld_in2 + col;
+            const bf16x8 dv = __builtin_bit_cast(bf16x8, dq), gv = *reinterpret_cast<const bf16x8*>(gp), uv = *reinterpret_cast<const bf16x8*>(gp + ea.inter);
+            bf16x8 og, ou;
+#pragma unroll
+            for (int e = 0; e < 8; ++e) {
+                float dg, du;
+                ssi_swiglu_bwd_elem<bf16_t>((float)gv[e], (float)uv[e], (float)dv[e], dg, du);
+                ou[e] = (bf16_t)du;
+                og[e] = (bf16_t)dg;
+            }
+            bf16_t* op = ea.out2 + r * ea.ld_out2 + col;
+            *reinterpret_cast<bf16x8*>(op) = og;
+            *reinterpret_cast<bf16x8*>(op + ea.inter) = ou;
+        };
+        finish(lo, row);
+        finish(hi, row + 8);
+    }
+}
+
+template <int EPI>
+int launch_nt4_reduce(const float* slabs, int splits, int tiles_m, int tiles_n, int t0, int ntiles, void* C, int64_t ldc, const void* R, float alpha,
+                      const float* alpha_dev, int accumulate, const EpiArgs& ea, hipStream_t st) {
+    const int64_t waves = (int64_t)ntiles * (EPI == EPI_SWIGLU_FWD ? 32 : 64);
+    hipLaunchKernelGGL(nt4_splitk_reduce_kernel<EPI>, dim3((unsigned)ssi_cdiv(waves, 4)), dim3(256), 0, st, slabs, splits, tiles_m, tiles_n, t0, ntiles,
+                       (bf16_t*)C, ldc, (const bf16_t*)R, alpha, alpha_dev, accumulate, ea);
+    SSI_LAUNCH_CHECK();
+    return SSI_OK;
+}
+
+int nt4_num_cu() {
     static const int num_cu = [] {
         int dev = 0, cus = 0;
         if (hipGetDevice(&dev) != hipSuccess || hipDeviceGetAttribute(&cus, hipDeviceAttributeMultiprocessorCount, dev) != hipSuccess || cus <= 0) cus = 256;
         return cus;
     }();
-    const int ntiles = tiles_m * tiles_n * (SPLITK ? splits : 1) * (BATCHED ? ea.batch : 1);
+    return num_cu;
+}
+
+void nt4_tail_rule(int64_t tiles, int64_t nk, int cus, int* n_main, int* splits) {
+    *n_main = (int)tiles;
+    *splits = 1;
+    if (cus <= 0 || (cus & 7) || tiles < cus || tiles >= 16LL * cus || (nk & 1) || nk >= (1 << 24)) return;
+    const int64_t tail = tiles % cus;
+    if (tail == 0 || 2 * tail >= cus) return;
+    const int64_t s = std::min<int64_t>(cus / tail, nk / 8);
+    if (s < 2) return;
+    *n_main = (int)(tiles - tail);
+    *splits = (int)std::min<int64_t>(s, 64);
+}
+
+template <bool A_COL, bool B_COL, int EPI, int PREV, bool SPLITK = false, bool BATCHED = false>
+int launch_nt4(int tiles_m, int tiles_n, int64_t K, const void* A, int64_t lda, const void* B, int64_t ldb, void* C, int64_t ldc,
+               const void* R, float alpha, const float* alpha_dev, hipStream_t st, EpiArgs ea = EpiArgs{nullptr, 0, nullptr, 0, 0},
+               int splits = 1, float* slabs = nullptr, int n_main = -1) {
+    static_assert(!BATCHED || (!SPLITK && EPI == EPI_PLAIN), "batched form: plain epilogue, no split-K");
+    auto kern = gemm_nt4dma_kernel<A_COL, B_COL, EPI, PREV, SPLITK, BATCHED>;
+    static const hipError_t attr_rc = hipFuncSetAttribute((const void*)kern, hipFuncAttributeMaxDynamicSharedMemorySize, NT4_LDS_BYTES);
+    if (attr_rc != hipSuccess) { ssi_set_error("gemm_nt4: cannot reserve %d B of LDS: %s", NT4_LDS_BYTES, hipGetErrorString(attr_rc)); return SSI_ERR_HIP + (int)attr_rc; }
+    const int num_cu = nt4_num_cu();
+    const int ntiles_out = tiles_m * tiles_n * (BATCHED ? ea.batch : 1);
+    if (SPLITK || BATCHED || n_main < 0 || n_main > ntiles_out) n_main = ntiles_out;
+    const int ntiles = SPLITK ? ntiles_out * splits : n_main + (ntiles_out - n_main) * splits;
     int grid = ntiles < num_cu ? ntiles : num_cu;
     const int slot = g_nt4_dynamic.load(std::memory_order_relaxed) ? (int)(nt4_next_slot() & 15) : -1;
     hipLaunchKernelGGL(kern, dim3((unsigned)grid), dim3(NT4_THREADS), NT4_LDS_BYTES, st, tiles_m, tiles_n, K, (const bf16_t*)A, lda,
-                       (const bf16_t*)B, ldb, (bf16_t*)C, ldc, (const bf16_t*)R, alpha, alpha_dev, ea, slot, splits, slabs);
+                       (const bf16_t*)B, ldb, (bf16_t*)C, ldc, (const bf16_t*)R, alpha, alpha_dev, ea, slot, splits, slabs, n_main);
     SSI_LAUNCH_CHECK();
+    if (!SPLITK && n_main < ntiles_out)
+        return launch_nt4_reduce<EPI>(slabs, splits, tiles_m, tiles_n, n_main, ntiles_out - n_main, C, ldc, PREV == 2 ? R : nullptr, alpha, alpha_dev,
+                                      PREV == 1, ea, st);
     return SSI_OK;
 }
 
 bool nt4_ok(int64_t K) { return K % (2 * BK) == 0 && K >= 4 * BK && ssi_get_impl() != SSI_IMPL_MFMA_WG8; }
 bool nt4_ld_ok(int64_t lda, int64_t ldb) { return 256 * lda * 2 < (1LL << 31) && 256 * ldb * 2 < (1LL << 31); }
 
+struct TailPlan { int n_main, splits; };
+int tail_plan(int64_t tiles, int64_t K, const void* ws, int64_t ws_bytes, TailPlan* tp) {
+    tp->n_main = (int)tiles;
+    tp->splits = 1;
+    if (!ws) return SSI_OK;
+    nt4_tail_rule(tiles, K / BK, nt4_num_cu(), &tp->n_main, &tp->splits);
+    if (tp->splits > 1 && (((uintptr_t)ws & 15) || ws_bytes < (tiles - tp->n_main) * tp->splits * (int64_t)(BM * BN * sizeof(float)))) {
+        ssi_set_error("gemm tail split: workspace misaligned or smaller than ssi_gemm_tail_workspace_bytes");
+        return SSI_ERR_WORKSPACE;
+    }
+    return SSI_OK;
+}
+
 template <bool A_COL, bool B_COL>
 int gemm_form(int tm, int tn, int64_t K, const void* A, int64_t lda, const void* B, int64_t ldb, void* C, int64_t ldc, const void* R,
-              float alpha, const float* alpha_dev, int accumulate, hipStream_t st) {
+              float alpha, const float* alpha_dev, int accumulate, hipStream_t st, void* ws, int64_t ws_bytes) {
     if (nt4_ok(K) && nt4_ld_ok(lda, ldb) && !(accumulate && R)) {
-        if (accumulate) return launch_nt4<A_COL, B_COL, EPI_PLAIN, 1>(tm, tn, K, A, lda, B, ldb, C, ldc, R, alpha, alpha_dev, st);
-        if (R) return launch_nt4<A_COL, B_COL, EPI_PLAIN, 2>(tm, tn, K, A, lda, B, ldb, C, ldc, R, alpha, alpha_dev, st);
-        return launch_nt4<A_COL, B_COL, EPI_PLAIN, 0>(tm, tn, K, A, lda, B, ldb, C, ldc, R, alpha, alpha_dev, st);
+        TailPlan tp;
+        if (int rc = tail_plan((int64_t)tm * tn, K, ws, ws_bytes, &tp)) return rc;
+        const EpiArgs none{nullptr, 0, nullptr, 0, 0};
+        if (accumulate) return launch_nt4<A_COL, B_COL, EPI_PLAIN, 1>(tm, tn, K, A, lda, B, ldb, C, ldc, R, alpha, alpha_dev, st, none, tp.splits, (float*)ws, tp.n_main);
+        if (R) return launch_nt4<A_COL, B_COL, EPI_PLAIN, 2>(tm, tn, K, A, lda, B, ldb, C, ldc, R, alpha, alpha_dev, st, none, tp.splits, (float*)ws, tp.n_main);
+        return launch_nt4<A_COL, B_COL, EPI_PLAIN, 0>(tm, tn, K, A, lda, B, ldb, C, ldc, R, alpha, alpha_dev, st, none, tp.splits, (float*)ws, tp.n_main);
     }
     return launch<A_COL, B_COL, false>(tm, tn, K, A, lda, B, ldb, C, ldc, R, alpha, alpha_dev, accumulate, st);
 }
 
+}
+
+int ssi_gemm_mfma_num_cu() { return nt4_num_cu(); }
+
+int ssi_gemm_mfma_tail_plan(int64_t M, int64_t N, int64_t K, int cus, int* n_main, int* splits) {
+    const int64_t tiles = (M > 0 && N > 0 && M % BM == 0 && N % BN == 0) ? (M / BM) * (N / BN) : 0;
+    *n_main = (int)tiles;
+    *splits = 1;
+    if (tiles <= 0 || tiles > (1LL << 30) || K % (2 * BK) || K < 4 * BK) return 1;
+    nt4_tail_rule(tiles, K / BK, cus > 0 ? cus : nt4_num_cu(), n_main, splits);
+    return *splits;
+}
+
+int64_t ssi_gemm_mfma_tail_units(int64_t M, int64_t N, int64_t K, int cus, int32_t* out, int64_t cap) {
+    int n_main, splits;
+    ssi_gemm_mfma_tail_plan(M, N, K, cus, &n_main, &splits);
+    const int tiles = (M % BM || N % BN) ? 0 : (int)((M / BM) * (N / BN)), n_tail = tiles - n_main, nk = (int)(K / BK);
+    int64_t n = 0;
+    for (int x = 0; x < 8; ++x) {
+        const int len = nt4_part_len(n_main, x) + nt4_part_len(n_tail * splits, x);
+        for (int p = 0; p < len; ++p, ++n) {
+            if (n >= cap) continue;
+            int lo, hi;
+            out[3 * n] = nt4_unit_decode(nt4_unit_at(x, p, n_main, n_tail * splits), n_main, n_tail > 0 ? n_tail : 1, nk, splits, lo, hi);
+            out[3 * n + 1] = lo;
+            out[3 * n + 2] = hi;
+        }
+    }
+    return n;
 }
 
 void ssi_gemm_mfma_set_dynamic_tiles(int on) { g_nt4_dynamic.store(on ? 1 : 0, std::memory_order_relaxed); }
@@ -1023,10 +1203,10 @@
 
 int ssi_gemm_mfma_bf16(int layout, int64_t M, int64_t N, int64_t K, const void* A, int64_t lda, const void* B,
                        int64_t ldb, void* C, int64_t ldc, const void* R, float alpha, const float* alpha_dev,
-                       int accumulate, void* stream) {
+                       int accumulate, void* stream, void* tail_ws, int64_t tail_ws_bytes) {
     const int tm = (int)(M / BM), tn = (int)(N / BN);
     auto st = (hipStream_t)stream;
-#define GO(AC, BC) return gemm_form<AC, BC>(tm, tn, K, A, lda, B, ldb, C, ldc, R, alpha, alpha_dev, accumulate, st)
+#define GO(AC, BC) return gemm_form<AC, BC>(tm, tn, K, A, lda, B, ldb, C, ldc, R, alpha, alpha_dev, accumulate, st, tail_ws, tail_ws_bytes)
     switch (layout) {
         case SSI_GEMM_NT: GO(false, false);
         case SSI_GEMM_NN: GO(false, true);
@@ -1062,10 +1242,7 @@
         else if (layout == SSI_GEMM_NT) rc = launch_nt4<false, false, EPI_PLAIN, 0, true>(tm, tn, K, A, lda, B, ldb, C, ldc, nullptr, 1.f, nullptr, st, none, splits, slabs);
         else if (layout == SSI_GEMM_NN) rc = launch_nt4<false, true, EPI_PLAIN, 0, true>(tm, tn, K, A, lda, B, ldb, C, ldc, nullptr, 1.f, nullptr, st, none, splits, slabs);
         if (rc) return rc;
-        hipLaunchKernelGGL(nt4_splitk_reduce_kernel, dim3((unsigned)ssi_cdiv((int64_t)tm * tn * 64, 4)), dim3(256), 0, st, slabs, splits, tm, tn,
-                           (bf16_t*)C, ldc, (const bf16_t*)R, alpha, alpha_dev, accumulate);
-        SSI_LAUNCH_CHECK();
-        return SSI_OK;
+        return launch_nt4_reduce<EPI_PLAIN>(slabs, splits, tm, tn, 0, tm * tn, C, ldc, R, alpha, alpha_dev, accumulate, none, st);
     }
 #define GO(AC, BC) return launch<AC, BC, true>(tm, tn, K, A, lda, B, ldb, C, ldc, R, alpha, alpha_dev, accumulate, st, splits, slabs)
     switch (layout) {
@@ -1078,13 +1255,16 @@
 }
 
 bool ssi_gemm_rope_mfma(int64_t M, int64_t N, int64_t K, const void* A, int64_t lda, const void* B, int64_t ldb, void* C, int64_t ldc,
-                        const float* rope, const int32_t* positions, int64_t seq, int64_t rot_cols, void* stream, int* rc) {
+                        const float* rope, const int32_t* positions, int64_t seq, int64_t rot_cols, void* stream, int* rc, void* tail_ws,
+                        int64_t tail_ws_bytes) {
     if (!nt4_ok(K) || !nt4_ld_ok(lda, ldb) || M % BM || N % BN || rot_cols % BN || rot_cols > N || lda % 8 || ldb % 8 || ldc % 8) return false;
     if (((uintptr_t)A | (uintptr_t)B | (uintptr_t)C) & 15) return false;
     EpiArgs ea{nullptr, 0, nullptr, 0, 0};
     ea.rope = rope; ea.pos = positions; ea.seq = seq; ea.rot_cols = rot_cols;
+    TailPlan tp;
+    if ((*rc = tail_plan((M / BM) * (N / BN), K, tail_ws, tail_ws_bytes, &tp))) return true;
     *rc = launch_nt4<false, false, EPI_ROPE, 0, false>((int)(M / BM), (int)(N / BN), K, A, lda, B, ldb, C, ldc, nullptr, 1.f, nullptr,
-                                                (hipStream_t)stream, ea);
+                                                (hipStream_t)stream, ea, tp.splits, (float*)tail_ws, tp.n_main);
     return true;
 }
 
@@ -1097,26 +1277,34 @@
 }
 
 int ssi_gemm_swiglu_fwd_mfma(int64_t M, int64_t inter, int64_t K, const void* X, int64_t ldx, const void* W13, int64_t ldw,
-                             void* GU, int64_t ldgu, void* ACT, int64_t ldact, void* stream) {
+                             void* GU, int64_t ldgu, void* ACT, int64_t ldact, void* stream, void* tail_ws, int64_t tail_ws_bytes) {
     EpiArgs ea{(bf16_t*)ACT, ldact, nullptr, 0, inter};
-    if (nt4_ok(K))
+    if (nt4_ok(K)) {
+        TailPlan tp;
+        if (int rc = tail_plan((M / BM) * (2 * inter / BN), K, tail_ws, tail_ws_bytes, &tp)) return rc;
         return launch_nt4<false, false, EPI_SWIGLU_FWD, 0, false>((int)(M / BM), (int)(2 * inter / BN), K, X, ldx, W13, ldw, GU, ldgu, nullptr, 1.f, nullptr,
-                                             (hipStream_t)stream, ea);
+                                             (hipStream_t)stream, ea, tp.splits, (float*)tail_ws, tp.n_main);
+    }
     return launch<false, false, false, EPI_SWIGLU_FWD>((int)(M / BM), (int)(2 * inter / BN), K, X, ldx, W13, ldw, GU, ldgu, nullptr, 1.f,
                                                        nullptr, 0, (hipStream_t)stream, 1, nullptr, ea);
 }
 
 int ssi_gemm_swiglu_bwd_mfma(int layout, int64_t M, int64_t inter, int64_t K, const void* DY, int64_t lddy, const void* W2, int64_t ldw,
-                             const void* GU, int64_t ldgu, void* DGU, int64_t lddgu, void* stream) {
+                             const void* GU, int64_t ldgu, void* DGU, int64_t lddgu, void* stream, void* tail_ws, int64_t tail_ws_bytes) {
     EpiArgs ea{(bf16_t*)DGU, lddgu, (const bf16_t*)GU, ldgu, inter};
+    TailPlan tp{0, 1};
+    if (nt4_ok(K) && nt4_ld_ok(lddy, ldw))
+        if (int rc = tail_plan((M / BM) * (inter / BN), K, tail_ws, tail_ws_bytes, &tp)) return rc;
     const int tm = (int)(M / BM), tn = (int)(inter / BN);
     if (layout == SSI_GEMM_NN) {
         if (nt4_ok(K) && nt4_ld_ok(lddy, ldw))
-            return launch_nt4<false, true, EPI_SWIGLU_BWD, 0, false>(tm, tn, K, DY, lddy, W2, ldw, DGU, lddgu, nullptr, 1.f, nullptr, (hipStream_t)stream, ea);
+            return launch_nt4<false, true, EPI_SWIGLU_BWD, 0, false>(tm, tn, K, DY, lddy, W2, ldw, DGU, lddgu, nullptr, 1.f, nullptr, (hipStream_t)stream, ea,
+                                                                     tp.splits, (float*)tail_ws, tp.n_main);
         return SSI_ERR_UNSUPPORTED;
     }
     if (nt4_ok(K) && nt4_ld_ok(lddy, ldw))
-        return launch_nt4<false, false, EPI_SWIGLU_BWD, 0, false>(tm, tn, K, DY, lddy, W2, ldw, DGU, lddgu, nullptr, 1.f, nullptr, (hipStream_t)stream, ea);
+        return launch_nt4<false, false, EPI_SWIGLU_BWD, 0, false>(tm, tn, K, DY, lddy, W2, ldw, DGU, lddgu, nullptr, 1.f, nullptr, (hipStream_t)stream, ea,
+                                                                  tp.splits, (float*)tail_ws, tp.n_main);
     return launch<false, false, false, EPI_SWIGLU_BWD>(tm, tn, K, DY, lddy, W2, ldw, DGU, lddgu, nullptr, 1.f, nullptr, 0, (hipStream_t)stream, 1,
                                                        nullptr, ea);
 }
diff --git a/speech-integration_amd/ssi/_lib.py b/speech-integration_amd/ssi/_lib.py
--- a/speech-integration_amd/ssi/_lib.py
+++ b/speech-integration_amd/ssi/_lib.py
@@ -14,7 +14,7 @@
 GEMM_NT, GEMM_NN, GEMM_TN = 0, 1, 2
 IMPL_AUTO, IMPL_GENERIC, IMPL_MFMA, IMPL_MFMA_WG8 = 0, 1, 2, 3
 TILES_STATIC, TILES_DYNAMIC = 0, 1
-ABI_VERSION = 9
+ABI_VERSION = 10
 ATTN_KERNEL_DQ, ATTN_KERNEL_DKV = 0, 1
 ATTN_MODE_AUTO, ATTN_MODE_OLD, ATTN_MODE_NEW, ATTN_MODE_NO_HEAD_SPLIT = 0, 1, 2, 3
 ATTN_USED_DQ2, ATTN_USED_DKV2, ATTN_USED_HEAD_SPLIT, ATTN_USED_PLAN = 1, 2, 4, 8
@@ -64,6 +64,16 @@
     "ssi_gemm_swiglu_fwd": (c_int, [c_int64, c_int64, c_int64, _P, c_int64, _P, c_int64, _P, c_int64, _P, c_int64, c_int, _P]),
     "ssi_gemm_swiglu_bwd": (c_int, [c_int, c_int64, c_int64, c_int64, _P, c_int64, _P, c_int64, _P, c_int64, _P, c_int64, _P, c_int,
                                     _P]),
+    "ssi_gemm_tail_plan": (c_int, [c_int64, c_int64, c_int64, c_int, _P, _P]),
+    "ssi_gemm_tail_workspace_bytes": (c_int64, [c_int64, c_int64, c_int64, c_int]),
+    "ssi_gemm_tail_units": (c_int64, [c_int64, c_int64, c_int64, c_int, _P, c_int64]),
+    "ssi_gemm_tail": (c_int, [c_int, c_int64, c_int64, c_int64, _P, c_int64, _P, c_int64, _P, c_int64, _P, c_float, _P,
+                              c_int, c_int, _P, c_int64, _P]),
+    "ssi_gemm_rope_tail": (c_int, [c_int64, c_int64, c_int64, _P, c_int64, _P, c_int64, _P, c_int64, c_int64, c_int, c_int, _P, c_int64, _P,
+                                   c_int, _P, c_int64, _P]),
+    "ssi_gemm_swiglu_fwd_tail": (c_int, [c_int64, c_int64, c_int64, _P, c_int64, _P, c_int64, _P, c_int64, _P, c_int64, c_int, _P, c_int64, _P]),
+    "ssi_gemm_swiglu_bwd_tail": (c_int, [c_int, c_int64, c_int64, c_int64, _P, c_int64, _P, c_int64, _P, c_int64, _P, c_int64, _P, c_int,
+                                         _P, c_int64, _P]),
     "ssi_transpose": (c_int, [_P, c_int64, _P, c_int64, c_int64, c_int64, c_int, _P]),
     "ssi_ce_fwd": (c_int, [_P, c_int64, _P, c_int64, c_int64, c_int64, _P, _P, c_int, c_int, _P]),
     "ssi_ce_fwd_weighted": (c_int, [_P, c_int64, _P, _P, c_int64, c_int64, c_int64, _P, _P, c_int, c_int, _P]),
diff --git a/speech-integration_amd/ssi/model.py b/speech-integration_amd/ssi/model.py
--- a/speech-integration_amd/ssi/model.py
+++ b/speech-integration_amd/ssi/model.py
@@ -314,6 +314,12 @@
             ops.gemm_splitk(layout, a, b, c, splits, wsk, residual=residual)
         else:
             ops.gemm(layout, a, b, c, residual=residual)
+
+    def _tail_ws(self, M: int, N: int, K: int) -> Optional[Tensor]:
+        if not (self.split_small_grids and self.dtype == torch.bfloat16 and self._mfma_shapes()):
+            return None
+        nbytes = ops.gemm_tail_workspace_bytes(M, N, K)
+        return self._arena.get("ws.tail", (nbytes,), torch.uint8) if nbytes else None
 
     def build_attn_plan(self, input_pos: Tensor, force: bool = False):
         from . import attn_plan
@@ -355,7 +361,8 @@
             rstd1 = A.get(f"rstd1.{sfx}", (T,), torch.float32)
             ops.rmsnorm_fwd(h, self._view(f"L{l}.sa_norm"), xn1, rstd1, self.norm_eps)
             qkv = A.get(f"qkv.{sfx}", (T, self.qkv_dim), dt)
-            ops.gemm_rope(xn1, self._view(f"L{l}.wqkv"), qkv, S, H + KV, hd, self._rope, positions=pos)
+            ops.gemm_rope(xn1, self._view(f"L{l}.wqkv"), qkv, S, H + KV, hd, self._rope, positions=pos,
+                          tail_ws=self._tail_ws(T, self.qkv_dim, D))
             att = A.get("att.all", (L, T, H * hd), dt)[l] if save else A.get("att.x", (T, H * hd), dt)
             lse = A.get(f"lse.{sfx}", (B * H * S,), torch.float32)
             ops.attn_fwd(qkv, att, lse, B, S, H, KV, hd, ds, de)
@@ -366,7 +373,7 @@
             ops.rmsnorm_fwd(hmid, self._view(f"L{l}.mlp_norm"), xn2, rstd2, self.norm_eps)
             gu = A.get(f"gu.{sfx}", (T, 2 * I), dt)
             act = A.get(f"act.{sfx}", (T, I), dt)
-            ops.gemm_swiglu_fwd(xn2, self._view(f"L{l}.w13"), gu, act)
+            ops.gemm_swiglu_fwd(xn2, self._view(f"L{l}.w13"), gu, act, tail_ws=self._tail_ws(T, 2 * I, D))
             hn_name = f"h{l + 1}" if save else f"hx{l & 1}"
             hnext = A.get(hn_name, (T, D), dt)
             self._gemm(GEMM_NT, act, self._view(f"L{l}.w2"), hnext, residual=hmid)
@@ -448,7 +455,7 @@
             h_in = A.get(f"h{l}", (T, D), dt)
             wgrad(dh, act, f"L{l}.w2")
             dgu = A.get("dgu", (T, 2 * I), dt)
-            ops.gemm_swiglu_bwd(GEMM_NN, dh, self._view(f"L{l}.w2"), gu, dgu, A.get("dact", (T, I), dt))
+            ops.gemm_swiglu_bwd(GEMM_NN, dh, self._view(f"L{l}.w2"), gu, dgu, A.get("dact", (T, I), dt), tail_ws=self._tail_ws(T, I, D))
             dxn = A.get("dxn", (T, D), dt)
             dgrad(dgu, f"L{l}.w13", dxn)
             wgrad(dgu, xn2, f"L{l}.w13")
diff --git a/speech-integration_amd/ssi/ops.py b/speech-integration_amd/ssi/ops.py
--- a/speech-integration_amd/ssi/ops.py
+++ b/speech-integration_amd/ssi/ops.py
@@ -1,5 +1,7 @@
 
 from __future__ import annotations
+
+import ctypes
 
 import torch
 from typing import Optional
@@ -9,7 +11,7 @@
 from ._lib import GEMM_NN, GEMM_NT, GEMM_TN, check, dtype_code, ptr, stream_ptr
 
 __all__ = ["lmhead_ce_fwd", "lmhead_ce_bwd", "doc_ranges", "embed_fwd", "embed_bwd", "rmsnorm_fwd", "rmsnorm_bwd", "rope_", "attn_fwd", "attn_bwd", "attn_bwd_workspace_bytes", "swiglu_fwd",
-           "swiglu_bwd", "gemm", "gemm_splitk", "splitk_choice", "gemm_swiglu_fwd", "gemm_swiglu_bwd", "transpose", "ce_fwd", "ce_reduce", "count_tokens", "scale_", "sumsq", "adamw_step", "set_impl", "set_attn_impl", "attn_last_dispatch",
+           "swiglu_bwd", "gemm", "gemm_splitk", "splitk_choice", "gemm_tail_plan", "gemm_tail_workspace_bytes", "gemm_tail_units", "gemm_swiglu_fwd", "gemm_swiglu_bwd", "transpose", "ce_fwd", "ce_reduce", "count_tokens", "scale_", "sumsq", "adamw_step", "set_impl", "set_attn_impl", "attn_last_dispatch",
            "GEMM_NT", "GEMM_NN", "GEMM_TN"]
 
 
@@ -85,16 +87,45 @@
           "ssi_rope_inplace")
 
 
+def _tail_ws(workspace: Tensor | None):
+    if workspace is None:
+        return None, 0
+    assert workspace.is_contiguous() and workspace.is_cuda
+    return ptr(workspace), workspace.numel() * workspace.element_size()
+
+
+def gemm_tail_plan(M: int, N: int, K: int, n_cu: int = 0) -> tuple[int, int]:
+    n_main, splits = ctypes.c_int(0), ctypes.c_int(1)
+    _lib.load().ssi_gemm_tail_plan(M, N, K, n_cu, ctypes.byref(n_main), ctypes.byref(splits))
+    return n_main.value, splits.value
+
+
+def gemm_tail_workspace_bytes(M: int, N: int, K: int, n_cu: int = 0) -> int:
+    return int(_lib.load().ssi_gemm_tail_workspace_bytes(M, N, K, n_cu))
+
+
+def gemm_tail_units(M: int, N: int, K: int, n_cu: int = 0) -> list[tuple[int, int, int]]:
+    lib = _lib.load()
+    n_main, splits = gemm_tail_plan(M, N, K, n_cu)
+    cap = n_main + ((M // 256) * (N // 256) - n_main) * splits
+    buf = (ctypes.c_int32 * (3 * max(cap, 1)))()
+    n = int(lib.ssi_gemm_tail_units(M, N, K, n_cu, buf, cap))
+    assert n == cap, (n, cap)
+    return [(buf[3 * i], buf[3 * i + 1], buf[3 * i + 2]) for i in range(n)]
+
+
 def gemm_rope(a: Tensor, b: Tensor, c: Tensor, seq_len: int, n_heads_rot: int, head_dim: int, table: Tensor,
-              positions: Tensor | None = None) -> None:
+              positions: Tensor | None = None, tail_ws: Tensor | None = None) -> None:
     assert a.dim() == 2 and b.dim() == 2 and c.dim() == 2 and a.stride(1) == 1 and b.stride(1) == 1 and c.stride(1) == 1
     M, K = a.shape
     N = b.shape[0]
     assert b.shape[1] == K and c.shape == (M, N) and a.dtype == b.dtype == c.dtype
     assert table.dtype == torch.float32 and table.is_contiguous() and table.shape[1] * 2 == head_dim
     assert positions is None or (positions.dtype == torch.int32 and positions.numel() == M)
-    check(_lib.load().ssi_gemm_rope(M, N, K, ptr(a), a.stride(0), ptr(b), b.stride(0), ptr(c), c.stride(0), seq_len, n_heads_rot, head_dim,
-                                    ptr(table), table.shape[0], ptr(positions), dtype_code(a.dtype), stream_ptr()), "ssi_gemm_rope")
+    ws, ws_bytes = _tail_ws(tail_ws)
+    check(_lib.load().ssi_gemm_rope_tail(M, N, K, ptr(a), a.stride(0), ptr(b), b.stride(0), ptr(c), c.stride(0), seq_len, n_heads_rot, head_dim,
+                                         ptr(table), table.shape[0], ptr(positions), dtype_code(a.dtype), ws, ws_bytes, stream_ptr()),
+          "ssi_gemm_rope_tail")
 
 
 def _doc_ptrs(doc_start: Optional[Tensor], doc_end: Optional[Tensor], rows: int):
@@ -176,7 +207,7 @@
 
 
 def gemm(layout: int, a: Tensor, b: Tensor, c: Tensor, *, residual: Tensor | None = None, alpha: float = 1.0,
-         alpha_dev: Tensor | None = None, accumulate: bool = False) -> None:
+         alpha_dev: Tensor | None = None, accumulate: bool = False, tail_ws: Tensor | None = None) -> None:
     assert a.dim() == 2 and b.dim() == 2 and c.dim() == 2 and a.stride(1) == 1 and b.stride(1) == 1 and c.stride(1) == 1
     assert a.dtype == b.dtype == c.dtype
     M, N = c.shape
@@ -193,9 +224,10 @@
         assert residual.shape == c.shape and residual.stride() == c.stride() and residual.dtype == c.dtype
     if alpha_dev is not None:
         assert alpha_dev.dtype == torch.float32 and alpha_dev.numel() == 1
-    check(_lib.load().ssi_gemm(layout, M, N, K, ptr(a), a.stride(0), ptr(b), b.stride(0), ptr(c), c.stride(0),
-                               ptr(residual), alpha, ptr(alpha_dev), int(accumulate), dtype_code(c.dtype), stream_ptr()),
-          "ssi_gemm")
+    ws, ws_bytes = _tail_ws(tail_ws)
+    check(_lib.load().ssi_gemm_tail(layout, M, N, K, ptr(a), a.stride(0), ptr(b), b.stride(0), ptr(c), c.stride(0),
+                                    ptr(residual), alpha, ptr(alpha_dev), int(accumulate), dtype_code(c.dtype), ws, ws_bytes, stream_ptr()),
+          "ssi_gemm_tail")
 
 
 def splitk_choice(M: int, N: int, K: int, n_cu: int = 256) -> int:
@@ -250,23 +282,26 @@
           "ssi_gemm_batched")
 
 
-def gemm_swiglu_fwd(x: Tensor, w13: Tensor, gu: Tensor, act: Tensor) -> None:
+def gemm_swiglu_fwd(x: Tensor, w13: Tensor, gu: Tensor, act: Tensor, tail_ws: Tensor | None = None) -> None:
     M, K = x.shape
     inter = act.shape[1]
     assert w13.shape == (2 * inter, K) and gu.shape == (M, 2 * inter) and act.shape[0] == M
     assert x.stride(1) == 1 and w13.stride(1) == 1 and gu.is_contiguous() and act.is_contiguous()
-    check(_lib.load().ssi_gemm_swiglu_fwd(M, inter, K, ptr(x), x.stride(0), ptr(w13), w13.stride(0), ptr(gu), gu.stride(0), ptr(act),
-                                          act.stride(0), dtype_code(x.dtype), stream_ptr()), "ssi_gemm_swiglu_fwd")
-
-
-def gemm_swiglu_bwd(layout: int, dy: Tensor, w2: Tensor, gu: Tensor, dgu: Tensor, dact_ws: Tensor | None) -> None:
+    ws, ws_bytes = _tail_ws(tail_ws)
+    check(_lib.load().ssi_gemm_swiglu_fwd_tail(M, inter, K, ptr(x), x.stride(0), ptr(w13), w13.stride(0), ptr(gu), gu.stride(0), ptr(act),
+                                               act.stride(0), dtype_code(x.dtype), ws, ws_bytes, stream_ptr()), "ssi_gemm_swiglu_fwd_tail")
+
+
+def gemm_swiglu_bwd(layout: int, dy: Tensor, w2: Tensor, gu: Tensor, dgu: Tensor, dact_ws: Tensor | None,
+                    tail_ws: Tensor | None = None) -> None:
     M, K = dy.shape
     inter = gu.shape[1] // 2
     assert w2.shape == ((inter, K) if layout == GEMM_NT else (K, inter)) and dgu.shape == gu.shape and gu.shape[0] == M
     assert dy.stride(1) == 1 and w2.stride(1) == 1 and gu.is_contiguous() and dgu.is_contiguous()
-    check(_lib.load().ssi_gemm_swiglu_bwd(layout, M, inter, K, ptr(dy), dy.stride(0), ptr(w2), w2.stride(0), ptr(gu), gu.stride(0),
-                                          ptr(dgu), dgu.stride(0), ptr(dact_ws), dtype_code(dy.dtype), stream_ptr()),
-          "ssi_gemm_swiglu_bwd")
+    ws, ws_bytes = _tail_ws(tail_ws)
+    check(_lib.load().ssi_gemm_swiglu_bwd_tail(layout, M, inter, K, ptr(dy), dy.stride(0), ptr(w2), w2.stride(0), ptr(gu), gu.stride(0),
+                                               ptr(dgu), dgu.stride(0), ptr(dact_ws), dtype_code(dy.dtype), ws, ws_bytes, stream_ptr()),
+          "ssi_gemm_swiglu_bwd_tail")
 
 
 def transpose(src: Tensor, dst: Tensor) -> None:
```

Result: no change. 156,700 tokens/s (-0.1%).
